# mmigas/LiverRenderer

Hardware: AMD Instinct MI355X
Metric: Msamples/s (higher is better)
Workload: dtype f32; 1 GPU; C3 Liver-SingleMesh volpath 1920x1080 512 spp max_depth 12 (homogeneous medium, isotropic phase, envmap); width=1920, height=1080, spp=512, parallelism=1 GPU

## Files before the change

liverrenderer_amd/csrc/device.hip:

```cpp
#include "host_scene.h"
#include "device_scene.h"
#include "kernels_prb.h"
#include "kernels_vae.h"
#include "kernels_aov.h"
#include "kernels_denoise.h"
#include "kernels_moment.h"
#include <functional>
#include "scene_prep.h"
#include <cmath>
#include <array>
#include <cstring>
#include <algorithm>
#include <stdexcept>
#include <string>
#include <cstdio>
#include <cstdlib>
#include <thread>
#include <chrono>
#include <exception>
#include <dlfcn.h>
#include <rccl/rccl.h>

namespace lrt {

// ... 85 lines not shown
        for (auto e : ev_pool) (void) hipEventDestroy(e);
        if (h_counters) (void) hipHostFree(h_counters);
        if (h_launch) (void) hipHostFree(h_launch);
        if (stream) (void) hipStreamDestroy(stream);
    }
};

void device_scene_destroy(DeviceScene *d) { delete d; }

static_assert(PREP_F_DELTA == F_DELTA && PREP_F_SMOOTH == F_SMOOTH && PREP_F_NULL == F_NULL, "scene_prep.h restates the BSDF leaf flags of dshade.h");

__global__ void k_bio_prepare(DBioMedium *bio, uint32_t n) {
    const uint32_t i = blockIdx.x * blockDim.x + threadIdx.x;
    if (i < n) bio[i].log10_hep = m_log2(bio[i].hepatocity + 1.f) / m_log2(10.f);
}

__global__ void k_medium_prepare(DMedium *media, uint32_t n) {
    const uint32_t i = blockIdx.x * blockDim.x + threadIdx.x;
    if (i >= n) return;
    DMedium &M = media[i];
    const V3 st(M.sigma_t[0], M.sigma_t[1], M.sigma_t[2]), ss = st * V3(M.albedo[0], M.albedo[1], M.albedo[2]);
    const V3 ws = ss / mean3(st / st), wp = ss / st;
    M.w_spec[0] = ws.x; M.w_spec[1] = ws.y; M.w_spec[2] = ws.z; M.w_plain[0] = wp.x; M.w_plain[1] = wp.y; M.w_plain[2] = wp.z;
}

static void upload_media(DeviceScene *D, const lrt_scene_desc &d) {
    prepare_media(d, D->sc.env.bsphere_r, D->h_media, D->h_bio, D->h_het);
    for (size_t i = 0; i < D->h_het.size(); ++i) D->h_het[i].data = D->het_data[i];
    HIP_CHECK(hipMemcpyAsync(D->d_bio, D->h_bio.data(), D->h_bio.size() * sizeof(DBioMedium), hipMemcpyHostToDevice, D->stream));
    k_bio_prepare<<<1, 64, 0, D->stream>>>(D->d_bio, (uint32_t) std::min<size_t>(D->h_bio.size(), 64));
    HIP_CHECK(hipGetLastError());
    HIP_CHECK(hipMemcpyAsync(D->d_het, D->h_het.data(), D->h_het.size() * sizeof(DHetMedium), hipMemcpyHostToDevice, D->stream));
    HIP_CHECK(hipMemcpyAsync(D->d_media, D->h_media.data(), D->h_media.size() * sizeof(DMedium), hipMemcpyHostToDevice, D->stream));
    k_medium_prepare<<<1, 64, 0, D->stream>>>(D->d_media, (uint32_t) std::min<size_t>(D->h_media.size(), 64));
    HIP_CHECK(hipGetLastError());
}

typedef void (*RenderFn)(ScenePtr, LaunchPtr);
struct RenderRow { int mode; bool lds, ld, compact, ext; uint32_t block, record_bytes; RenderFn fn; };

template <int MODE, int BLOCK, bool LDS, bool LD, bool COMPACT = false, bool EXT = false> static void add_row(std::vector<RenderRow> &t) {
    static_assert(record_form_exists(record_layout(MODE), COMPACT), "this layout has no such form (record_layout.h, kRecordForms)");
    t.push_back({ MODE, LDS, LD, COMPACT, EXT, BLOCK, record_bytes(record_layout(MODE), COMPACT), k_render<MODE, BLOCK, LDS, LD, COMPACT, EXT> });
}
template <int MODE, int LDS_BLOCK> static void add_mode(std::vector<RenderRow> &t) {
    add_row<MODE, LDS_BLOCK, true, false>(t); add_row<MODE, LDS_BLOCK, true, true>(t);
    add_row<MODE, LDS_BLOCK, true, false, false, true>(t); add_row<MODE, LDS_BLOCK, true, true, false, true>(t);
    add_row<MODE, LRT_BLOCK, false, false>(t); add_row<MODE, LRT_BLOCK, false, true>(t);
    add_row<MODE, LRT_BLOCK, false, false, false, true>(t); add_row<MODE, LRT_BLOCK, false, true, false, true>(t);
}
template <int MODE> static void add_compact(std::vector<RenderRow> &t) { add_row<MODE, 1024, true, false, true>(t); add_row<MODE, 1024, true, true, true>(t); }

struct KernelTable { std::vector<RenderRow> render; RenderFn prb[2][2][2][2] = {}, prb_grid[2][2] = {}; };
template <bool LDS, bool LD> static void add_prb(KernelTable &t) {
    constexpr int BLOCK = LDS ? 1024 : LRT_BLOCK;
    t.prb[0][LDS][LD][0] = k_render_prb<false, BLOCK, LDS, LD, false>; t.prb[0][LDS][LD][1] = k_render_prb<false, BLOCK, LDS, LD, true>;
    t.prb[1][LDS][LD][0] = k_render_prb<true, BLOCK, LDS, LD, false>; t.prb[1][LDS][LD][1] = k_render_prb<true, BLOCK, LDS, LD, true>;
    t.prb_grid[LDS][LD] = k_render_prb_grid<BLOCK, LDS, LD>;
}
static const KernelTable &kernels() {
    static const KernelTable table = [] {
        KernelTable t; std::vector<RenderRow> &r = t.render;
#ifdef LRT_DEV_VOLPATH_ONLY
#ifndef LRT_DEV_INTEGRATOR
#define LRT_DEV_INTEGRATOR LRT_INTEGRATOR_VOLPATH
#endif
#ifndef LRT_DEV_LD
#define LRT_DEV_LD false
#endif
#ifndef LRT_DEV_BLOCK
#define LRT_DEV_BLOCK 1024
#endif
#define LRT_DEV_CLOSED (LRT_DEV_INTEGRATOR == LRT_INTEGRATOR_VOLPATH ? LRT_INTEGRATOR_VOLPATH_CLOSED : LRT_DEV_INTEGRATOR)
        add_row<LRT_DEV_INTEGRATOR, LRT_DEV_BLOCK, true, LRT_DEV_LD>(r);
        if constexpr (record_form_exists(record_layout(LRT_DEV_INTEGRATOR), true)) {
            add_row<LRT_DEV_INTEGRATOR, LRT_DEV_BLOCK, true, LRT_DEV_LD, true>(r); add_row<LRT_DEV_CLOSED, LRT_DEV_BLOCK, true, LRT_DEV_LD, true>(r);
        }
#else
        add_mode<LRT_INTEGRATOR_PATH, 1024>(r); add_mode<LRT_INTEGRATOR_VOLPATH, 1024>(r); add_mode<LRT_INTEGRATOR_BIOVOLPATH, 1024>(r); add_mode<LRT_INTEGRATOR_BIOVOLPATH06, 1024>(r);
        add_mode<LRT_INTEGRATOR_VOLPATH_HET, LRT_WIDE_BLOCK>(r); add_mode<LRT_INTEGRATOR_VOLPATHMIS, LRT_WIDE_BLOCK>(r); add_mode<LRT_INTEGRATOR_VOLPATHMIS_PLAIN, LRT_WIDE_BLOCK>(r);
        add_compact<LRT_INTEGRATOR_PATH>(r); add_compact<LRT_INTEGRATOR_VOLPATH>(r); add_compact<LRT_INTEGRATOR_BIOVOLPATH>(r); add_compact<LRT_INTEGRATOR_BIOVOLPATH06>(r);
        add_compact<LRT_INTEGRATOR_VOLPATH_CLOSED>(r);
        add_prb<false, false>(t); add_prb<false, true>(t); add_prb<true, false>(t); add_prb<true, true>(t);
#endif
        return t;
    }();
    return table;
}

typedef void (*AovFn)(ScenePtr, LaunchPtr, AovSpecPtr);
static AovFn aov_kernel(bool lds, bool ld, bool ext) {
    static const AovFn t[2][2][2] = { { { k_aov<false, false, false>, k_aov<false, false, true> }, { k_aov<false, true, false>, k_aov<false, true, true> } },
                                      { { k_aov<true, false, false>, k_aov<true, false, true> }, { k_aov<true, true, false>, k_aov<true, true, true> } } };
    return t[lds][ld][ext];
}
typedef decltype(&k_trace<false, false>) TraceFn;
typedef decltype(&k_trace_lds<false, false>) TraceLdsFn;
static TraceFn trace_kernel(bool any_hit, bool ext) {
    static const TraceFn t[2][2] = { { k_trace<false, false>, k_trace<false, true> }, { k_trace<true, false>, k_trace<true, true> } };
    return t[any_hit][ext];
}
static TraceLdsFn trace_lds_kernel(bool any_hit, bool ext) {
    static const TraceLdsFn t[2][2] = { { k_trace_lds<false, false>, k_trace_lds<false, true> }, { k_trace_lds<true, false>, k_trace_lds<true, true> } };
    return t[any_hit][ext];
}
static RenderFn moment_splat_kernel(bool wide, bool alpha) {
    static const RenderFn t[2][2] = { { k_moment_splat<false, false>, k_moment_splat<false, true> }, { k_moment_splat<true, false>, k_moment_splat<true, true> } };
    return t[wide][alpha];
}

DeviceScene *device_scene_create(const lrt_scene_desc &d, int device) {
    select_device(device);
    std::unique_ptr<DeviceScene> D(new DeviceScene());
    D->device = device;
    HIP_CHECK(hipStreamCreateWithFlags(&D->stream, hipStreamNonBlocking));
    hipStream_t st = D->stream;
    PrepOptions opt = PrepOptions::from_env();
    hipDeviceProp_t prop; HIP_CHECK(hipGetDeviceProperties(&prop, device)); opt.n_cus = prop.multiProcessorCount > 0 ? prop.multiProcessorCount : 256;
    int optin = 0; if (hipDeviceGetAttribute(&optin, hipDeviceAttributeSharedMemPerBlockOptin, device) != hipSuccess || optin <= 0) optin = (int) prop.sharedMemPerBlock;
    (void) hipGetLastError();
    opt.lds_limit = std::min<size_t>((size_t) std::max(optin, 0), 160 * 1024) - 512;
    PreparedScene P; DScene &sc = P.sc;
    prepare_geometry(d, opt, P);
    D->n_cus = opt.n_cus; D->bvh_leaf = P.bvh_leaf; D->ext = P.ext;
    auto up = [&](const auto &v) { return D->track(dev_upload(v.data(), v.size(), st)); };
    sc.spheres = P.spheres.empty() ? nullptr : up(P.spheres);
    sc.nodes = (const float4 *) up(P.bvh.nodes);
    sc.tris = (const float4 *) up(P.bvh.tris);
    if (P.use_lds) {
        D->lds = P.lds; D->lds.blob = (const uint4 *) up(P.lds_blob);
        const size_t lds_limit = opt.lds_limit;
        auto raise_lds = [&](const void *k) { if (k) HIP_CHECK(hipFuncSetAttribute(k, hipFuncAttributeMaxDynamicSharedMemorySize, (int) lds_limit)); };
        const KernelTable &K = kernels();
        for (const RenderRow &r : K.render) if (r.lds && (!r.ext || D->ext)) raise_lds((const void *) r.fn);
        for (const auto &adjoint : K.prb) for (const auto &ld : adjoint[1]) for (RenderFn fn : ld) raise_lds((const void *) fn);
        for (RenderFn fn : K.prb_grid[1]) raise_lds((const void *) fn);
        for (int i = 0; i < 2; ++i) for (int ext = 0; ext <= (D->ext ? 1 : 0); ++ext) {
            raise_lds((const void *) aov_kernel(true, i, ext)); raise_lds((const void *) trace_lds_kernel(i, ext));
        }
        D->use_lds = true;
    }
    if (sc.grid.enabled) {
        const size_t n_cells = (size_t) sc.grid.n[0] * sc.grid.n[1] * sc.grid.n[2];
        uint16_t *buf = nullptr; HIP_CHECK(hipMalloc((void **) &buf, n_cells * sizeof(uint16_t))); D->track(buf);
        k_build_dist_grid<<<(uint32_t) ((n_cells + LRT_BLOCK - 1) / LRT_BLOCK), LRT_BLOCK, 0, st>>>(sc.tris, d.n_faces ? (uint32_t) (P.bvh.tris.size() / 12) : 0u, sc.grid, buf, P.grid_abs_margin,
                                                                                             sc.spheres, sc.n_spheres);
        HIP_CHECK(hipGetLastError());
        sc.grid.d = buf;
    }
    prepare_shading(d, opt, P);
    D->has_area_emitter = P.has_area_emitter; D->has_het = P.has_het; D->has_non_bio = P.has_non_bio; D->prb_null = P.prb_null;
    sc.positions = D->track(dev_upload(d.positions, 3 * (size_t) d.n_vertices, st));
    sc.vattr = (const float4 *) up(P.vattr);
    sc.faces = D->track(dev_upload(d.faces, 3 * (size_t) d.n_faces, st));
    sc.face_shape = D->track(dev_upload(d.face_shape, d.n_faces, st));
    sc.shapes = up(P.shapes);
    sc.textures = up(P.textures);
    sc.tex_data = up(P.tex_data);
    sc.bsdfs = up(P.bsdfs);
    HIP_CHECK(hipMalloc((void **) &D->d_media, std::max<uint32_t>(d.n_media, 1) * sizeof(DMedium))); D->track(D->d_media);
    HIP_CHECK(hipMalloc((void **) &D->d_bio, std::max<uint32_t>(d.n_media, 1) * sizeof(DBioMedium))); D->track(D->d_bio);
    HIP_CHECK(hipMalloc((void **) &D->d_het, std::max<uint32_t>(d.n_media, 1) * sizeof(DHetMedium))); D->track(D->d_het);
    D->het_data.assign(std::max<uint32_t>(d.n_media, 1), nullptr);
    for (uint32_t i = 0; i < d.n_media; ++i) {
        const lrt_medium_desc &M = d.media[i];
        if (M.type == LRT_MEDIUM_HETEROGENEOUS) D->het_data[i] = D->track(dev_upload(M.grid_data, (size_t) M.grid_res[0] * M.grid_res[1] * M.grid_res[2], st));
    }
    D->sc = sc;
    upload_media(D.get(), d); sc.media = D->d_media; sc.bio = D->d_bio; sc.het = D->d_het;
    sc.emitters = up(P.emitters);
    sc.mesh_emitters = up(P.mesh_emitters);
    sc.mesh_emitter_tab = up(P.mesh_emitter_tab);
    sc.env_data = (const float4 *) up(P.env_data);
    sc.env_hier = up(P.env_hier);
    HIP_CHECK(hipMalloc((void **) &D->d_sc, sizeof(DScene))); D->track(D->d_sc);
    D->sc = sc;
    HIP_CHECK(hipMemcpyAsync(D->d_sc, &D->sc, sizeof(DScene), hipMemcpyHostToDevice, st));
    HIP_CHECK(hipMalloc((void **) &D->d_launch, LRT_LAUNCH_SLOTS * sizeof(DLaunch))); D->track(D->d_launch);
    HIP_CHECK(hipHostMalloc((void **) &D->h_launch, LRT_LAUNCH_SLOTS * sizeof(DLaunch)));
    HIP_CHECK(hipMalloc((void **) &D->counters, sizeof(DCounters))); D->track(D->counters);
    HIP_CHECK(hipHostMalloc((void **) &D->h_counters, sizeof(DCounters)));
    HIP_CHECK(hipStreamSynchronize(st));
    return D.release();
}

void device_scene_update_params(DeviceScene *D, const lrt_scene_desc &d, bool grids) {
    HIP_CHECK(hipSetDevice(D->device));
    if (grids) for (uint32_t i = 0; i < d.n_media; ++i) {
        const lrt_medium_desc &M = d.media[i];
        if (M.type == LRT_MEDIUM_HETEROGENEOUS && D->het_data[i])
            HIP_CHECK(hipMemcpyAsync(D->het_data[i], M.grid_data, (size_t) M.grid_res[0] * M.grid_res[1] * M.grid_res[2] * sizeof(float), hipMemcpyHostToDevice, D->stream));
    }
    upload_media(D, d);
    HIP_CHECK(hipStreamSynchronize(D->stream));
}

static void ensure_workspace(DeviceScene *D, uint32_t capacity) {
    const uint32_t layouts = workspace_layouts(D->has_het, D->need_mis);
    if (D->capacity >= capacity && D->ws_layouts == layouts) return;
    HIP_CHECK(hipStreamSynchronize(D->stream));
    D->capacity = 0;
    auto get = [](const DPathStreams *q, const RecordStream &r) { void *p; memcpy(&p, (const char *) q + r.member, sizeof p); return p; };
    auto set = [](DPathStreams *q, const RecordStream &r, void *p) { memcpy((char *) q + r.member, &p, sizeof p); };
    for (DPathStreams *q : { &D->q[0], &D->q[1] })
        for (const RecordStream &r : kRecordStreams) if (r.member != kNoMember) { D->release(get(q, r)); set(q, r, nullptr); }
    for (DPathStreams *q : { &D->q[0], &D->q[1] })
        for (size_t k = 0; k < std::size(kRecordStreams); ++k) if (const uint32_t bytes = workspace_stream_bytes(k, layouts)) {
            void *p = nullptr; HIP_CHECK(hipMalloc(&p, (size_t) capacity * bytes)); D->track(p); set(q, kRecordStreams[k], p);
        }
    D->capacity = capacity; D->ws_layouts = layouts;
}

static hipEvent_t get_event(DeviceScene *D, size_t i) {
    while (D->ev_pool.size() <= i) { hipEvent_t e; HIP_CHECK(hipEventCreate(&e)); D->ev_pool.push_back(e); }
    return D->ev_pool[i];
}

static void ensure_pixel_list(DeviceScene *D, const ResolvedOpts &O) {
    const DFilm &F = D->sc.film;
    if (O.tile_count == 1) { D->n_owned_pixels = (uint32_t) F.width * F.height; return; }
    if (D->pixel_list && D->pixel_list_rank == O.tile_rank && D->pixel_list_count == O.tile_count) return;
    const TilePixels T = tile_pixel_list(F, O.tile_rank, O.tile_count);
    D->release(D->pixel_list); D->release(D->pixel_slot); D->pixel_list = nullptr; D->pixel_slot = nullptr;
    D->pixel_list = D->track(dev_upload(T.list.data(), T.list.size(), D->stream));
    D->pixel_slot = D->track(dev_upload(T.slot.data(), T.slot.size(), D->stream));
    D->pixel_list_rank = O.tile_rank; D->pixel_list_count = O.tile_count; D->n_owned_pixels = (uint32_t) T.list.size();
}

static void ensure_halo_list(DeviceScene *D, const ResolvedOpts &O, uint32_t halo) {
    const DFilm &F = D->sc.film;
    if (D->halo_list && D->halo_rank == O.tile_rank && D->halo_count == O.tile_count && D->halo_width == halo) return;
    const std::vector<uint32_t> px = halo_pixel_list(F, O.tile_rank, O.tile_count, halo);
    D->release(D->halo_list); D->halo_list = nullptr;
    D->halo_list = D->track(dev_upload(px.data(), px.size(), D->stream));
    D->halo_rank = O.tile_rank; D->halo_count = O.tile_count; D->halo_width = halo; D->n_halo_pixels = (uint32_t) px.size();
}

static void ensure_prb_workspace(DeviceScene *D, uint32_t records, uint64_t l_buf_lanes) {
    for (int k = 0; k < 2; ++k) D->grow(D->dl[k], D->dl_records[k], records);
    D->grow(D->L_buf, D->l_buf_lanes, l_buf_lanes);
    if (!D->d_grads) { HIP_CHECK(hipMalloc((void **) &D->d_grads, 7 * sizeof(double))); D->track(D->d_grads); }
}

static DRenderParams make_params(const lrt_scene_desc &d, const ResolvedOpts &O, uint64_t n_lanes) {
    DRenderParams rp{};
    rp.integrator = O.integrator; rp.max_depth = O.max_depth; rp.rr_depth = O.rr_depth; rp.hide_emitters = O.hide_emitters;
    rp.spp = O.spp; rp.log2_spp = ((O.spp & (O.spp - 1)) == 0) ? (uint32_t) __builtin_ctz(O.spp) : 0xffffffffu;
    rp.profile = getenv("LRT_DEBUG_LAUNCH") ? 1u : 0u;
#ifdef LRT_EXPERIMENT
    if (getenv("LRT_EXP")) rp.profile |= (uint32_t) atoi(getenv("LRT_EXP"));
    if (getenv("LRT_PRB_DEBUG_LANE")) rp.pad1 = (uint32_t) atoi(getenv("LRT_PRB_DEBUG_LANE")) + 1u;
#endif
    rp.seed_value = d.sampler_seed + O.seed; rp.base_seed = d.sampler_seed; rp.seed = O.seed;
    rp.ld_count = d.sampler_type == LRT_SAMPLER_LD ? O.spp_total : 0u; rp.pass_index = O.pass; rp.spp_total = O.spp_total; rp.tile_rank = O.tile_rank; rp.tile_count = O.tile_count; rp.n_lanes = n_lanes;
    return rp;
}

struct LaunchLog { std::vector<std::pair<hipEvent_t, hipEvent_t>> launches; std::vector<uint32_t> sizes; unsigned long long n_records = 0; size_t ev = 0; uint64_t n_iter = 0; };

static void finish_stats(DeviceScene *D, LaunchLog &log, hipEvent_t e_begin, hipEvent_t e_end, uint64_t n_lanes, lrt_render_stats &stats) {
    hipStream_t st = D->stream;
    HIP_CHECK(hipEventRecord(e_end, st));
    HIP_CHECK(hipMemcpyAsync(D->h_counters, D->counters, sizeof(DCounters), hipMemcpyDeviceToHost, st));
    HIP_CHECK(hipStreamSynchronize(st));
    HIP_CHECK(hipGetLastError());
    stats.n_samples = n_lanes; stats.n_iter = log.n_iter; stats.n_shadow = D->h_counters->n_shadow; stats.n_launches = log.launches.size();
    stats.n_records = log.n_records; if (!log.n_records) for (uint32_t n : log.sizes) stats.n_records += n;
    float ms = 0.f; double ksum = 0.0;
    for (size_t i = 0; i < log.launches.size(); ++i) {
        HIP_CHECK(hipEventElapsedTime(&ms, log.launches[i].first, log.launches[i].second)); ksum += ms;
        if (getenv("LRT_DEBUG_LAUNCH") && i < 40) {
            fprintf(stderr, "[lrt] launch %zu: %.3f ms\n", i, ms);
        }
    }
    stats.kernel_ms = ksum; stats.lds_resident = D->use_lds ? 1 : 0;
    if (getenv("LRT_DEBUG_LAUNCH")) for (int r = 0; r < 4; ++r) {
        fprintf(stderr, "[lrt] tile kind %d (0 proven-free, 1 query, 2 surface, 3 fresh): %llu tiles, %.1f ticks/tile (100 MHz wall clock)\n", r, D->h_counters->prof_tiles[r], D->h_counters->prof_tiles[r] ? (double) D->h_counters->prof_cycles[r] / D->h_counters->prof_tiles[r] : 0.0);
    }
    if (getenv("LRT_DEBUG_LAUNCH") && D->h_counters->prof_wg[1]) {
        const unsigned long long *w = D->h_counters->prof_wg; const double n_wg = D->use_lds ? D->n_cus : 4.0 * D->n_cus, first = (double) ~w[2];
        fprintf(stderr, "[lrt] workgroups (last launch; us): first start 0, last start %.1f, last end %.1f, mean run time %.1f, mean LDS-image copy %.1f, mean barrier wait per wave %.1f\n",
                ((double) w[5] - first) / 100.0, ((double) w[1] - first) / 100.0, (double) w[3] / n_wg / 100.0, (double) w[0] / n_wg / 100.0, (double) w[4] / (n_wg * (D->use_lds ? 16.0 : 4.0)) / 100.0);
    }
    HIP_CHECK(hipEventElapsedTime(&ms, e_begin, e_end)); stats.total_ms = ms;
}

struct PoolGeometry { uint32_t n_wg, P; size_t smem; };
static PoolGeometry pool_geometry(DeviceScene *D, uint64_t n_lanes) {
    PoolGeometry g;
    g.n_wg = D->use_lds ? (uint32_t) D->n_cus : 4u * (uint32_t) D->n_cus;
    const uint32_t pool_max = getenv("LRT_POOL") ? std::max(64, atoi(getenv("LRT_POOL"))) : (D->use_lds ? 32768u : 8192u);
    g.P = (uint32_t) std::min<uint64_t>(pool_max, std::max<uint64_t>(64, ((n_lanes + g.n_wg - 1) / g.n_wg + 63) / 64 * 64));
    if (!getenv("LRT_POOL") && D->use_lds) {
        const uint64_t per_wg = (n_lanes + g.n_wg - 1) / g.n_wg, want = (per_wg / 48 + 63) / 64 * 64;
        if (want < g.P) g.P = (uint32_t) std::max<uint64_t>(want, std::min<uint64_t>(g.P, 8192));
    }
    g.smem = D->use_lds ? D->lds.total_bytes : (size_t) LRT_STACK * LRT_BLOCK * sizeof(int);
    return g;
}

static LaunchPtr push_launch(DeviceScene *D, const DLaunch &a) {
    const uint32_t slot = D->launch_next++ % LRT_LAUNCH_SLOTS;
    if (slot == 0 && D->launch_next > 1) HIP_CHECK(hipStreamSynchronize(D->stream));
    D->h_launch[slot] = a;
    HIP_CHECK(hipMemcpyAsync(&D->d_launch[slot], &D->h_launch[slot], sizeof(DLaunch), hipMemcpyHostToDevice, D->stream));
    return (LaunchPtr) &D->d_launch[slot];
}

template <bool ADJOINT>
static void launch_prb(DeviceScene *D, const DRenderParams &rp, const PoolGeometry &g, const uint32_t *pixel_list, uint64_t lane_begin,
                       float4 *L_buf, const float *grad_image, double *grads, float *film, float *sample_out, float *dgrid = nullptr) {
    hipStream_t st = D->stream;
    HIP_CHECK(hipMemsetAsync(&D->counters->next_lane, 0, sizeof(unsigned long long), st));
    DLaunch a{}; a.rp = rp; a.li = D->lds; a.q0 = D->q[0]; a.q1 = D->q[1]; a.dl0 = D->dl[0]; a.dl1 = D->dl[1]; a.P = g.P; a.cnt = D->counters;
    a.pixel_list = pixel_list; a.lane_begin = lane_begin; a.n = rp.n_lanes; a.L_buf = L_buf; a.grad_image = grad_image; a.wfilm = D->wfilm; a.grads = grads;
    a.film = film; a.sample_out = sample_out; a.sample_base = lane_begin; a.dgrid = dgrid;
    const LaunchPtr lp = push_launch(D, a);
    const bool ld = rp.ld_count != 0;
    const RenderFn fn = (ADJOINT && dgrid) ? kernels().prb_grid[D->use_lds][ld] : kernels().prb[ADJOINT][D->use_lds][ld][D->prb_null];
    if (!fn) throw std::runtime_error("developer build: volpath only");
    fn<<<g.n_wg, D->use_lds ? 1024 : LRT_BLOCK, g.smem, st>>>((ScenePtr) D->d_sc, lp);
    HIP_CHECK(hipGetLastError());
}

static void check_integrator_media(DeviceScene *D, int integrator) {
    if ((integrator == LRT_INTEGRATOR_BIOVOLPATH || integrator == LRT_INTEGRATOR_BIOVOLPATH06) && D->has_non_bio)
        throw std::runtime_error("NotImplementedError: sample_interaction (the bio integrators need liver / parenchyma / glissonCapsule media)");
    if (integrator == LRT_INTEGRATOR_PRBVOLPATH && D->ext)
        throw std::runtime_error("unsupported: prbvolpath on a scene with sphere shapes, point emitters or area emitters on meshes (its adjoint is built for triangles and rectangle / infinite emitters)");
    if (integrator == LRT_INTEGRATOR_VOLPATHMIS) D->need_mis = true;
}

static const RenderRow &select_render_kernel(int integrator, bool has_het, bool spectral_mis, bool lds, bool ld, bool ext, bool compact, bool closed) {
    int mode;
    switch (integrator) {
        case LRT_INTEGRATOR_PATH: case LRT_INTEGRATOR_BIOVOLPATH: case LRT_INTEGRATOR_BIOVOLPATH06: mode = integrator; break;
        case LRT_INTEGRATOR_VOLPATHMIS: mode = spectral_mis ? LRT_INTEGRATOR_VOLPATHMIS : LRT_INTEGRATOR_VOLPATHMIS_PLAIN; break;
        default: mode = closed ? LRT_INTEGRATOR_VOLPATH_CLOSED : (has_het ? LRT_INTEGRATOR_VOLPATH_HET : LRT_INTEGRATOR_VOLPATH);
    }
    for (const RenderRow &r : kernels().render) if (r.mode == mode && r.lds == lds && r.ld == ld && r.compact == compact && r.ext == ext) return r;
    throw std::runtime_error("no render-kernel instance for mode " + std::to_string(mode) + (lds ? ", LDS BVH" : ", global BVH") + (ld ? ", ld sampler" : ", independent sampler") +
                             (compact ? ", compact records" : ", wide records") + (ext ? ", EXT" : ""));
}

static void run_wavefront(DeviceScene *D, const lrt_scene_desc &d, const ResolvedOpts &O, uint64_t lane_begin, uint64_t n_lanes,
                          const uint32_t *pixel_list, float *film, float *sample_out, lrt_render_stats &stats) {
    hipStream_t st = D->stream;
    DRenderParams rp = make_params(d, O, n_lanes);
    rp.pixel_slot = pixel_list ? D->pixel_slot : nullptr;
    rp.pass_in = D->cur_pass_in; rp.pass_out = D->cur_pass_out;
    const bool prb = O.integrator == LRT_INTEGRATOR_PRBVOLPATH;
    check_integrator_media(D, O.integrator);
    PoolGeometry g = pool_geometry(D, n_lanes);
    const uint32_t records = (uint32_t) std::min<uint64_t>((uint64_t) g.n_wg * 2u * g.P, 0xffffffffull);
    ensure_workspace(D, records);
    if (prb) ensure_prb_workspace(D, records, 0);
    HIP_CHECK(hipMemsetAsync(D->counters, 0, sizeof(DCounters), st));
    LaunchLog log;
    hipEvent_t e_begin = get_event(D, log.ev++), e_end = get_event(D, log.ev++);
    HIP_CHECK(hipEventRecord(e_begin, st));
    const bool count_iter = !(O.integrator == LRT_INTEGRATOR_PATH && O.max_depth == 0);
    hipEvent_t a = get_event(D, log.ev++), b = get_event(D, log.ev++);
    HIP_CHECK(hipEventRecord(a, st));
    if (prb) { stats.record_bytes = 0; launch_prb<false>(D, rp, g, pixel_list, lane_begin, nullptr, nullptr, nullptr, film, sample_out); }
    else {
        DLaunch a{}; a.rp = rp; a.li = D->lds; a.q0 = D->q[0]; a.q1 = D->q[1]; a.P = g.P; a.cnt = D->counters; a.pixel_list = pixel_list;
        a.lane_begin = lane_begin; a.n = n_lanes; a.film = film; a.sample_out = sample_out; a.sample_base = lane_begin;
        const bool compact = D->use_lds && !D->has_area_emitter && !D->ext && !getenv("LRT_WIDE_RECORDS") && O.integrator != LRT_INTEGRATOR_VOLPATHMIS && !(O.integrator == LRT_INTEGRATOR_VOLPATH && D->has_het);
        const bool closed = compact && O.integrator == LRT_INTEGRATOR_VOLPATH && closed_records(d, D->sc.cam.medium) && !getenv("LRT_NO_CLOSED_RECORDS");
#ifdef LRT_DEV_VOLPATH_ONLY
        if (D->ext) throw std::runtime_error("developer build: no EXT instances (spheres / point emitters)");
        if (!(D->use_lds && (O.integrator == LRT_DEV_INTEGRATOR || (LRT_DEV_INTEGRATOR == LRT_INTEGRATOR_VOLPATH_HET && D->has_het)) && (rp.ld_count != 0) == LRT_DEV_LD)) throw std::runtime_error("developer build: one integrator / sampler / LDS BVH only");
#endif
        const RenderRow &row = select_render_kernel(O.integrator, D->has_het, d.use_spectral_mis != 0, D->use_lds, rp.ld_count != 0, D->ext, compact, closed);
        stats.record_bytes = row.record_bytes;
        const LaunchPtr lp = push_launch(D, a);
        row.fn<<<g.n_wg, row.block, g.smem, st>>>((ScenePtr) D->d_sc, lp);
        HIP_CHECK(hipGetLastError());
    }
    HIP_CHECK(hipEventRecord(b, st));
    log.launches.emplace_back(a, b); log.sizes.push_back(0);
    HIP_CHECK(hipMemcpyAsync(D->h_counters, D->counters, sizeof(DCounters), hipMemcpyDeviceToHost, st));
    HIP_CHECK(hipStreamSynchronize(st));
    log.n_iter = count_iter ? D->h_counters->n_iter : 0;
    log.n_records = D->h_counters->n_records;
    finish_stats(D, log, e_begin, e_end, n_lanes, stats);
    stats.n_closed_guard = D->h_counters->n_closed_guard;
    if (stats.n_closed_guard)
        throw std::runtime_error("64-byte path records: " + std::to_string(stats.n_closed_guard) + " trips broke the premise of the layout (radiance before a path's last trip, "
                                 "or an emitter hit that needs its MIS weight); the scene test in closed_records() is wrong for this scene: LRT_NO_CLOSED_RECORDS=1 renders it with 80-byte records");
}

static void render_passes(DeviceScene *D, const lrt_scene_desc &d, const lrt_render_opts *opts, float *film_raw, float *image, lrt_render_stats &stats,
                          const std::function<void(const ResolvedOpts &)> &after_pass, bool moment = false);

void device_render(DeviceScene *D, const lrt_scene_desc &d, const lrt_render_opts *opts, float *film_raw, float *image, lrt_render_stats &stats) {
    render_passes(D, d, opts, film_raw, image, stats, nullptr);
}

static void develop_and_download(DeviceScene *D, const float *film, float *film_raw, float *image, size_t film_floats, size_t image_floats, bool on_device, bool moment = false) {
    const DFilm &F = D->sc.film; const size_t np = (size_t) F.width * F.height;
// ... 614 lines not shown
```

liverrenderer_amd/csrc/device_types.h:

```cpp
#pragma once
#include <stdint.h>
#include <hip/hip_vector_types.h>

namespace lrt {

struct DShape {
    int32_t bsdf, emitter, interior_medium, exterior_medium;
    int32_t has_normals, has_texcoords, flip_normals, kind;
};

struct DBsdf {
    int32_t type, reflectance, nested, texture;
    float eta, scale; int32_t flags, pad;
};

struct DTexture {
    int32_t type, width, height, channels;
    float color0[3]; float color1[3];
    float to_uv[6];
    uint32_t data_offset;
    uint32_t pad;
};

struct DMedium {
    float sigma_t[3]; float albedo[3];
    int32_t has_spectral_extinction, sample_emitters, phase; float g;
    float scale; int32_t het;
    float w_spec[3], w_plain[3];
    float nee_vmin[3];
    float pad2[3];
};

struct DBioMedium {
    int32_t type, has_spectral_extinction;
    float layer_limit[4];
    float collagen[4][3], elastin[4][3];
    float blood[3], bile[3], lipid_water[3];
    float hepatocity, log10_hep;
    float sigmat[3];
    float pad;
};

struct DHetMedium {
    const float *data;
    int32_t res[3]; float max_density;
    float to_local[12];
    float bbox_min[3], bbox_max[3];
    float scale, pad;
};

struct DEmitter {
    int32_t type, shape; float radiance[3]; float scale;
    float n[3]; float inv_area;
    float to_world[12];
};

struct DSphere {
    float center[3], radius;
    float to_world[9];
    float to_object[12];
    uint32_t shape; int32_t flip_normals;
    float pad[2];
};

struct DMeshEmitter {
    uint32_t first_face, n_faces, pmf_offset, cdf_offset;
    float sum, normalization;
    int32_t has_normals, flip_normals;
    int32_t mesh, pad[3];
};

#define LRT_MAX_HIER_LEVELS 16

struct DCamera {
    float s2c[16];
    float to_world[12];
    float near_clip, far_clip;
    int32_t medium, pad;
    float ppo_x, ppo_y;
};

struct DFilm {
    int32_t width, height;
    int32_t crop_offset_x, crop_offset_y;
    float scale_x, scale_y, offset_x, offset_y;
    int32_t channels, has_alpha, rfilter, fcount;
    float rf_radius, rf_inv_radius; int32_t fn, pad;
    float rf_coeff[10];
    int32_t pad2[2];
};

struct DEnv {
    int32_t type;
    int32_t emitter;
    uint32_t w, h;
    float scale;
    float bsphere_c[3]; float bsphere_r;
    float to_world[9];
    float to_local[9];
    float patch_size[2], inv_patch_size[2];
    uint32_t max_patch[2];
    int32_t n_levels;
    uint32_t level_offset[LRT_MAX_HIER_LEVELS];
    uint32_t level_width[LRT_MAX_HIER_LEVELS];
    float radiance[3];
};

struct DDistGrid {
    const uint16_t *d;
    float lo[3]; float cell, inv_cell;
    int32_t n[3]; int32_t enabled;
};

struct DScene {
    const float4 *nodes;
    const float4 *tris;
    const float *positions;
    const float4 *vattr;
    const uint32_t *faces, *face_shape;
    const DShape *shapes; const DBsdf *bsdfs; const DTexture *textures; const DMedium *media; const DBioMedium *bio; const DHetMedium *het; const DEmitter *emitters;
    const float *tex_data;
    const float4 *env_data;
    const float *env_hier;
    uint32_t n_faces, n_emitters;
    int32_t root_is_leaf, has_null_bsdf;
    int32_t nee_fast_reject;
    int32_t one_shape;
    uint32_t root_leaf_first, root_leaf_count;
    DCamera cam; DFilm film; DEnv env;
    DDistGrid grid;
    const DSphere *spheres;
    uint32_t n_spheres, pad_sph;
    const DMeshEmitter *mesh_emitters;
    const float *mesh_emitter_tab;
};

#define LRT_CONST __attribute__((address_space(4)))
typedef const LRT_CONST DScene &SceneRef;
typedef const LRT_CONST DFilm &FilmRef;
typedef const LRT_CONST DEnv &EnvRef;
typedef const LRT_CONST DDistGrid &GridRef;
typedef const LRT_CONST DScene *ScenePtr;

struct DRenderParams {
    int32_t integrator, max_depth, rr_depth, hide_emitters;
    uint32_t spp, log2_spp;
    uint32_t seed_value;
    uint32_t base_seed, seed;
    uint32_t ld_count, pad1;
    uint32_t tile_rank, tile_count;
    int32_t grad_medium;
    uint32_t tiles_x, tiles_y, profile;
    uint32_t pad2;
    uint64_t n_lanes;
    const uint32_t *pixel_slot;
    uint32_t pass_index, spp_total;
    const unsigned long long *pass_in;
    unsigned long long *pass_out;
};

struct DPathStreams {
    float4 *o_maxt;
    float4 *d_eta;
    float4 *tp_pdf;
    float4 *res_flags;
    float4 *lp_lane;
    uint2  *rng;
    float2 *tdepth;
    float4 *hit;
    float4 *w1, *w2, *w3, *w4;
};

#define LRT_INTEGRATOR_VOLPATHMIS_PLAIN 102
#define LRT_INTEGRATOR_VOLPATH_HET 101
#define LRT_INTEGRATOR_VOLPATH_CLOSED 103

#define PF_DEPTH_MASK   0x0000ffffu
#define PF_MEDIUM_SHIFT 16
#define PF_MEDIUM_MASK  0x00ff0000u
#define PF_CHANNEL_SHIFT 24
#define PF_SPECULAR     (1u << 26)
#define PF_VALID        (1u << 27)
#define PF_NOHIT        (1u << 28)
#define PF_BIO_SCATTERED (1u << 29)
#define PF_LONG_QUERY   (1u << 29)
#define PF_HAVE_SI      (1u << 29)
#define PF_LAST_NULL    (1u << 30)
#define PF_BIO_EMIT     (1u << 30)
#define PF_BIO_FULL     (1u << 31)

struct DCounters {
    uint32_t pad[4];
    unsigned long long n_shadow;
    unsigned long long n_iter;
    unsigned long long next_lane;
    unsigned long long n_records;
    unsigned long long prof_cycles[4], prof_tiles[4];
    unsigned long long prof_wg[6];
    unsigned long long n_closed_guard;
};

struct DLdsInfo {
    const uint4 *blob;
    uint32_t blob_bytes, nodes_off, verts_off, tris_off, stack_off, total_bytes;
};

struct DLaunch {
    DRenderParams rp; DLdsInfo li; DPathStreams q0, q1;
    float4 *dl0, *dl1;
    uint32_t P, pad; DCounters *cnt; const uint32_t *pixel_list; uint64_t lane_begin, n;
    float4 *L_buf; const float *grad_image; const float *wfilm; double *grads;
    float *film; float *sample_out; uint64_t sample_base;
    float *dgrid;
};
typedef const LRT_CONST DRenderParams &RpRef;
typedef const LRT_CONST DLaunch *LaunchPtr;

}
```

liverrenderer_amd/csrc/dshade.h:

```cpp
#pragma once
#include "device_types.h"
#include "dmath.h"
#include "../../include/liverrt.h"

namespace lrt {

#define LRT_BLOCK 256
#define LRT_STACK 32

template <class T> DEV T tab(const T *table, uint32_t i, bool worth_a_look = true) {
    if (!worth_a_look) return table[i];
    const uint32_t i0 = (uint32_t) __builtin_amdgcn_readfirstlane((int) i);
    if (__builtin_amdgcn_ballot_w64(true) != 0ull && __builtin_amdgcn_ballot_w64(i != i0) == 0ull)
    { T out; __builtin_memcpy(&out, reinterpret_cast<const LRT_CONST T *>((uintptr_t) table) + i0, sizeof(T)); return out; }
    return table[i];
}

struct Ray { V3 o, d; float maxt; };
struct Hit { float t, u, v; uint32_t prim; uint32_t slot = 0xffffffffu; };
struct SI { bool valid; float t; V3 p, n; Frame sh; V2 uv; V3 dp_du, dp_dv, wi; uint32_t prim, shape; };

DEV float slab_rcp(float x) { return fmin_(fmax_(__builtin_amdgcn_rcpf(x), -1e20f), 1e20f); }
DEV void test_tri(const float4 *__restrict__ tris, uint32_t slot, V3 o, V3 d, float maxt, Hit &best) {
    float4 a = tris[3 * slot], b = tris[3 * slot + 1], c = tris[3 * slot + 2];
    V3 p0(a.x, a.y, a.z), e1(b.x, b.y, b.z), e2(c.x, c.y, c.z);
    uint32_t f = f2u(a.w);
    V3 pvec = cross(d, e2);
    float inv_det = rcp(dot(e1, pvec));
    V3 tvec = o - p0;
    float u = dot(tvec, pvec) * inv_det;
    if (!(u >= 0.f && u <= 1.f)) return;
    V3 qvec = cross(tvec, e1);
    float v = dot(d, qvec) * inv_det;
    if (!(v >= 0.f && u + v <= 1.f)) return;
    float t = dot(e2, qvec) * inv_det;
    if (!(t >= 0.f && t <= maxt)) return;
    if (t < best.t || (t == best.t && f < best.prim)) { best.t = t; best.u = u; best.v = v; best.prim = f; }
}

template <bool ANY_HIT>
DEV Hit trace(SceneRef sc, const Ray &r, int *__restrict__ stack ) {
    Hit best; best.t = kInf; best.u = best.v = 0.f; best.prim = 0xffffffffu;
    if (sc.n_faces == 0) return best;
    const V3 o = r.o, d = r.d;
    if (sc.root_is_leaf) {
        for (uint32_t i = 0; i < sc.root_leaf_count; ++i) test_tri(sc.tris, sc.root_leaf_first + i, o, d, r.maxt, best);
        return best;
    }
    const float ix = slab_rcp(d.x), iy = slab_rcp(d.y), iz = slab_rcp(d.z);
    const float ox = -o.x * ix, oy = -o.y * iy, oz = -o.z * iz;
    const f32x2 vix = { ix, ix }, viy = { iy, iy }, viz = { iz, iz }, vox = { ox, ox }, voy = { oy, oy }, voz = { oz, oz };
    const uint32_t DONE = 0x7fffffffu;
    int sp = 0; uint32_t cur = 0;
    for (;;) {
        while (cur < DONE) {
            const float4 *nd = sc.nodes + 4 * (size_t) cur;
            float4 n0 = nd[0], n1 = nd[1], n2 = nd[2], n3 = nd[3];
            float limit = fmin_(best.t, r.maxt);
            const f32x2 vax = pk_fma(f32x2{ n0.x, n0.y }, vix, vox), vay = pk_fma(f32x2{ n0.z, n0.w }, viy, voy), vaz = pk_fma(f32x2{ n2.x, n2.y }, viz, voz);
            const f32x2 vbx = pk_fma(f32x2{ n1.x, n1.y }, vix, vox), vby = pk_fma(f32x2{ n1.z, n1.w }, viy, voy), vbz = pk_fma(f32x2{ n2.z, n2.w }, viz, voz);
            const float ax0 = vax.x, ax1 = vax.y, ay0 = vay.x, ay1 = vay.y, az0 = vaz.x, az1 = vaz.y;
            const float bx0 = vbx.x, bx1 = vbx.y, by0 = vby.x, by1 = vby.y, bz0 = vbz.x, bz1 = vbz.y;
            float tmin0 = fmax_(fmax_(fmin_(ax0, ax1), fmin_(ay0, ay1)), fmax_(fmin_(az0, az1), 0.f));
            float tmax0 = fmin_(fmin_(fmax_(ax0, ax1), fmax_(ay0, ay1)), fmin_(fmax_(az0, az1), limit));
            float tmin1 = fmax_(fmax_(fmin_(bx0, bx1), fmin_(by0, by1)), fmax_(fmin_(bz0, bz1), 0.f));
            float tmax1 = fmin_(fmin_(fmax_(bx0, bx1), fmax_(by0, by1)), fmin_(fmax_(bz0, bz1), limit));
            bool h0 = tmin0 <= tmax0 * 1.000002f, h1 = tmin1 <= tmax1 * 1.000002f;
            int r0 = (int) f2u(n3.x), r1 = (int) f2u(n3.y);
            uint32_t c0 = r0 < 0 ? (0x80000000u | (uint32_t) ~r0) : (uint32_t) r0;
            uint32_t c1 = r1 < 0 ? (0x80000000u | (uint32_t) ~r1) : (uint32_t) r1;
            if (h0 && h1) {
                bool swap = tmin1 < tmin0;
                stack[sp * LRT_BLOCK] = (int) (swap ? c0 : c1); ++sp;
                cur = swap ? c1 : c0;
            } else if (h0 || h1) cur = h0 ? c0 : c1;
            else if (sp == 0) cur = DONE;
            else { --sp; cur = (uint32_t) stack[sp * LRT_BLOCK]; }
        }
        if (cur == DONE) break;
        uint32_t slot = cur & 0x7fffffffu; bool last;
        do { last = sc.tris[3 * slot + 1].w != 0.f; test_tri(sc.tris, slot, o, d, r.maxt, best); ++slot; } while (!last);
        if (ANY_HIT && best.prim != 0xffffffffu) return best;
        if (sp == 0) break;
        --sp; cur = (uint32_t) stack[sp * LRT_BLOCK];
    }
    return best;
}

struct GlobalTracer {
    static constexpr bool kExt = false;
    SceneRef sc; int *stack;
    DEV Hit closest(const Ray &r) const { return trace<false>(sc, r, stack); }
    DEV Hit any(const Ray &r) const { return trace<true>(sc, r, stack); }
    DEV SI surface(SceneRef s, const Ray &r, const Hit &h) const;
};

struct LdsScene {
    const float4 *nodes; const float4 *verts; const uint2 *tris;
    uint32_t n_faces, root_is_leaf, root_first, root_count;
};
#define LRT_LDS_BLOCK_MAX 1024

DEV void test_tri_lds(const LdsScene &L, uint2 ix, uint32_t slot, V3 o, V3 d, float maxt, Hit &best) {
    float4 a = L.verts[ix.x & 0xffffu], b = L.verts[ix.x >> 16], c = L.verts[ix.y & 0xffffu];
    V3 p0(a.x, a.y, a.z), e1(b.x - a.x, b.y - a.y, b.z - a.z), e2(c.x - a.x, c.y - a.y, c.z - a.z);
    V3 pvec = cross(d, e2);
    float inv_det = rcp(dot(e1, pvec));
    V3 tvec = o - p0;
    float u = dot(tvec, pvec) * inv_det;
    if (!(u >= 0.f && u <= 1.f)) return;
    V3 qvec = cross(tvec, e1);
    float v = dot(d, qvec) * inv_det;
    if (!(v >= 0.f && u + v <= 1.f)) return;
    float t = dot(e2, qvec) * inv_det;
    if (!(t >= 0.f && t <= maxt)) return;
    if (t > best.t) return;
    uint32_t f = ix.y >> 17;
    if (t < best.t || f < (best.prim & 0x7fffu)) { best.t = t; best.u = u; best.v = v; best.prim = f | (slot << 16); }
}

#ifdef LRT_TRAV_STATS
__device__ unsigned long long g_trav[8];
#define LRT_TRAV_COUNT(k) { const unsigned long long m_ = __ballot(true); if ((threadIdx.x & 63u) == (uint32_t) (__ffsll((long long) m_) - 1)) { atomicAdd(&g_trav[(ANY_HIT ? 4 : 0) + k], 1ull); atomicAdd(&g_trav[(ANY_HIT ? 4 : 0) + k + 1], (unsigned long long) __popcll(m_)); } }
#else
#define LRT_TRAV_COUNT(k)
#endif
template <bool ANY_HIT, int STRIDE>
DEV Hit trace_lds(const LdsScene &L, const Ray &r, uint16_t *__restrict__ stack ) {
    Hit best; best.t = kInf; best.u = best.v = 0.f; best.prim = 0xffffffffu;
    if (L.n_faces == 0) return best;
    const V3 o = r.o, d = r.d;
    if (L.root_is_leaf) {
        for (uint32_t i = 0; i < L.root_count; ++i) test_tri_lds(L, L.tris[L.root_first + i], L.root_first + i, o, d, r.maxt, best);
        if (best.prim != 0xffffffffu) { best.slot = best.prim >> 16; best.prim &= 0x7fffu; }
        return best;
    }
    const float ix = slab_rcp(d.x), iy = slab_rcp(d.y), iz = slab_rcp(d.z);
    const float ox = -o.x * ix, oy = -o.y * iy, oz = -o.z * iz;
    const f32x2 vix = { ix, ix }, viy = { iy, iy }, viz = { iz, iz }, vox = { ox, ox }, voy = { oy, oy }, voz = { oz, oz };
    const uint32_t DONE = 0x10000u;
    int sp = 0; uint32_t cur = 0;
    for (;;) {
        while (cur < 0x8000u) {
            LRT_TRAV_COUNT(0)
            const float4 *nd = L.nodes + 4 * cur;
            float4 n0 = nd[0], n1 = nd[1], n2 = nd[2], n3 = nd[3];
            float limit = fmin_(best.t, r.maxt);
            const f32x2 vax = pk_fma(f32x2{ n0.x, n0.y }, vix, vox), vay = pk_fma(f32x2{ n0.z, n0.w }, viy, voy), vaz = pk_fma(f32x2{ n2.x, n2.y }, viz, voz);
            const f32x2 vbx = pk_fma(f32x2{ n1.x, n1.y }, vix, vox), vby = pk_fma(f32x2{ n1.z, n1.w }, viy, voy), vbz = pk_fma(f32x2{ n2.z, n2.w }, viz, voz);
            const float ax0 = vax.x, ax1 = vax.y, ay0 = vay.x, ay1 = vay.y, az0 = vaz.x, az1 = vaz.y;
            const float bx0 = vbx.x, bx1 = vbx.y, by0 = vby.x, by1 = vby.y, bz0 = vbz.x, bz1 = vbz.y;
            float tmin0 = fmax_(fmax_(fmin_(ax0, ax1), fmin_(ay0, ay1)), fmax_(fmin_(az0, az1), 0.f));
            float tmax0 = fmin_(fmin_(fmax_(ax0, ax1), fmax_(ay0, ay1)), fmin_(fmax_(az0, az1), limit));
            float tmin1 = fmax_(fmax_(fmin_(bx0, bx1), fmin_(by0, by1)), fmax_(fmin_(bz0, bz1), 0.f));
            float tmax1 = fmin_(fmin_(fmax_(bx0, bx1), fmax_(by0, by1)), fmin_(fmax_(bz0, bz1), limit));
            bool h0 = tmin0 <= tmax0 * 1.000002f, h1 = tmin1 <= tmax1 * 1.000002f;
            const uint32_t c0 = f2u(n3.x), c1 = f2u(n3.y);
            if (h0 && h1) {
                bool swap = tmin1 < tmin0;
                stack[sp * STRIDE] = (uint16_t) (swap ? c0 : c1); ++sp;
                cur = swap ? c1 : c0;
            } else if (h0 || h1) cur = h0 ? c0 : c1;
            else if (sp == 0) cur = DONE;
            else { --sp; cur = stack[sp * STRIDE]; }
        }
        if (cur == DONE) break;
        uint32_t slot = cur & 0x7fffu, last;
        do {
            LRT_TRAV_COUNT(2)
            const uint2 ix = L.tris[slot];
            last = (ix.y >> 16) & 1u;
            test_tri_lds(L, ix, slot, o, d, r.maxt, best);
            ++slot;
        } while (!last);
        if (ANY_HIT && best.prim != 0xffffffffu) return best;
        if (sp == 0) break;
        --sp; cur = stack[sp * STRIDE];
    }
    if (best.prim != 0xffffffffu) { best.slot = best.prim >> 16; best.prim &= 0x7fffu; }
    return best;
}

template <int STRIDE>
struct LdsTracer {
    static constexpr bool kExt = false;
    const LdsScene &L; uint16_t *stack;
    DEV Hit closest(const Ray &r) const { return trace_lds<false, STRIDE>(L, r, stack); }
    DEV Hit any(const Ray &r) const { return trace_lds<true, STRIDE>(L, r, stack); }
    DEV SI surface(SceneRef s, const Ray &r, const Hit &h) const;
};

DEV float dist_grid_lower_bound(GridRef g, V3 p) {
    float fx = (p.x - g.lo[0]) * g.inv_cell, fy = (p.y - g.lo[1]) * g.inv_cell, fz = (p.z - g.lo[2]) * g.inv_cell;
    int ix = min(max((int) fx, 0), g.n[0] - 1), iy = min(max((int) fy, 0), g.n[1] - 1), iz = min(max((int) fz, 0), g.n[2] - 1);
    union { uint16_t u; _Float16 h; } cv; cv.u = g.d[(uint32_t) ((iz * g.n[1] + iy) * g.n[0] + ix)];
    float D = (float) cv.h;
    float cx = fx - ((float) ix + .5f), cy = fy - ((float) iy + .5f), cz = fz - ((float) iz + .5f);
    return D - __builtin_amdgcn_sqrtf(cx * cx + cy * cy + cz * cz) * (g.cell * 1.001f);
}

#ifndef LRT_GRID_STEPS
#define LRT_GRID_STEPS 3
#endif
template <int STEPS = LRT_GRID_STEPS>
DEV bool segment_proven_empty(GridRef g, V3 o, V3 d, float maxt) {
    if (!g.enabled || !(maxt < 1e30f)) return false;
    float len = __builtin_amdgcn_sqrtf(dot(d, d));
    float remaining = maxt * len * 1.01f, inv_len = __builtin_amdgcn_rcpf(len);
    V3 p = o;
    for (int k = 0; k < STEPS; ++k) {
        float lb = dist_grid_lower_bound(g, p);
        if (remaining < lb) return true;
        if (!(lb > .5f * g.cell)) return false;
        float adv = lb * .99f;
        p = p + d * (adv * inv_len);
        remaining -= adv * .995f;
    }
    return false;
}

template <int K>
DEV bool segment_covered_by_balls(GridRef g, V3 o, V3 d, float maxt) {
    if (!g.enabled || !(maxt < 1e30f)) return false;
    const float len = __builtin_amdgcn_sqrtf(dot(d, d));
    const float L = maxt * len * 1.01f;
#define LRT_FRAC(k) (((float) (k) + .5f) / (float) K)
    float lb[K];
#pragma unroll
    for (int k = 0; k < K; ++k) lb[k] = dist_grid_lower_bound(g, fma3(d, maxt * LRT_FRAC(k), o)) * .995f;
    float covered = 0.f; bool ok = true;
#pragma unroll
    for (int k = 0; k < K; ++k) {
        const float c = L * LRT_FRAC(k);
        ok = ok && (lb[k] > 0.f) && (c - lb[k] <= covered);
        covered = fmax_(covered, c + lb[k]);
    }
    return ok && covered >= L;
#undef LRT_FRAC
}

DEV bool segment_free_of_surfaces(GridRef g, V3 o, V3 d, float maxt) {
#ifdef LRT_SPHERE_TRACE
    return segment_proven_empty(g, o, d, maxt);
#else
    return segment_covered_by_balls<2>(g, o, d, maxt);
#endif
}

DEV SI compute_si(SceneRef sc, const Ray &r, const Hit &h, const LdsScene *L = nullptr) {
    const bool valid = h.prim != 0xffffffffu;
    float t = kInf; V3 p(0.f), n(0.f), shn(0.f), shs(0.f), sht(0.f), dp_du(0.f), dp_dv(0.f), wi = -r.d;
    V2 uv = { 0.f, 0.f }; uint32_t f = 0xffffffffu, shp = 0xffffffffu;
    if (valid) {
        f = h.prim; shp = 0u; if (!sc.one_shape) shp = sc.face_shape[f];
        const DShape sd = tab(sc.shapes, shp, sc.one_shape);
        uint32_t i0, i1, i2; V3 p0, p1, p2;
        if (L && h.slot != 0xffffffffu) {
            const uint2 ix = L->tris[h.slot];
            i0 = ix.x & 0xffffu; i1 = ix.x >> 16; i2 = ix.y & 0xffffu;
            const float4 a = L->verts[i0], b = L->verts[i1], c = L->verts[i2];
            p0 = V3(a.x, a.y, a.z); p1 = V3(b.x, b.y, b.z); p2 = V3(c.x, c.y, c.z);
        } else {
            i0 = sc.faces[3 * f]; i1 = sc.faces[3 * f + 1]; i2 = sc.faces[3 * f + 2];
            p0 = V3(sc.positions[3 * i0], sc.positions[3 * i0 + 1], sc.positions[3 * i0 + 2]);
            p1 = V3(sc.positions[3 * i1], sc.positions[3 * i1 + 1], sc.positions[3 * i1 + 2]);
            p2 = V3(sc.positions[3 * i2], sc.positions[3 * i2 + 1], sc.positions[3 * i2 + 2]);
        }
        float b1 = h.u, b2 = h.v, b0 = 1.f - b1 - b2;
        t = h.t;
        p = V3(fma_(p0.x, b0, fma_(p1.x, b1, p2.x * b2)), fma_(p0.y, b0, fma_(p1.y, b1, p2.y * b2)), fma_(p0.z, b0, fma_(p1.z, b1, p2.z * b2)));
        V3 dp0 = p1 - p0, dp1 = p2 - p0;
        n = normalize(cross(dp0, dp1));
        uv = { b1, b2 };
        Basis bs = coordinate_system(n);
        dp_du = bs.s; dp_dv = bs.t;
        if (sd.has_texcoords) {
            const float2 t0 = *reinterpret_cast<const float2 *>(sc.vattr + 2 * (size_t) i0 + 1), t1 = *reinterpret_cast<const float2 *>(sc.vattr + 2 * (size_t) i1 + 1),
                         t2 = *reinterpret_cast<const float2 *>(sc.vattr + 2 * (size_t) i2 + 1);
            V2 uv0 = { t0.x, t0.y }, uv1 = { t1.x, t1.y }, uv2 = { t2.x, t2.y };
            uv = { fma_(uv2.x, b2, fma_(uv1.x, b1, uv0.x * b0)), fma_(uv2.y, b2, fma_(uv1.y, b1, uv0.y * b0)) };
            V2 duv0 = { uv1.x - uv0.x, uv1.y - uv0.y }, duv1 = { uv2.x - uv0.x, uv2.y - uv0.y };
            float det = fma_(duv0.x, duv1.y, -(duv0.y * duv1.x)), inv_det = rcp(det);
            if (det != 0.f) {
                dp_du = V3(fma_(duv1.y, dp0.x, -(duv0.y * dp1.x)), fma_(duv1.y, dp0.y, -(duv0.y * dp1.y)), fma_(duv1.y, dp0.z, -(duv0.y * dp1.z))) * inv_det;
                dp_dv = V3(fma_(-duv1.x, dp0.x, duv0.x * dp1.x), fma_(-duv1.x, dp0.y, duv0.x * dp1.y), fma_(-duv1.x, dp0.z, duv0.x * dp1.z)) * inv_det;
            }
        }
        if (sd.has_normals) {
            const float4 a0 = sc.vattr[2 * (size_t) i0], a1 = sc.vattr[2 * (size_t) i1], a2 = sc.vattr[2 * (size_t) i2];
            V3 n0(a0.x, a0.y, a0.z), n1(a1.x, a1.y, a1.z), n2(a2.x, a2.y, a2.z);
            V3 ni(fma_(n2.x, b2, fma_(n1.x, b1, n0.x * b0)), fma_(n2.y, b2, fma_(n1.y, b1, n0.y * b0)), fma_(n2.z, b2, fma_(n1.z, b1, n0.z * b0)));
            float il = rsqrt_(squared_norm(ni));
            shn = ni * il;
        } else shn = n;
        if (sd.flip_normals) { n = V3(-n.x, -n.y, -n.z); shn = V3(-shn.x, -shn.y, -shn.z); }
        shs = normalize(fma3(shn, -dot(shn, dp_du), dp_du));
        if (dp_du.x == 0.f && dp_du.y == 0.f && dp_du.z == 0.f) shs = coordinate_system(shn).s;
        sht = cross(shn, shs);
        V3 md(-r.d.x, -r.d.y, -r.d.z);
        wi = V3(dot(md, shs), dot(md, sht), dot(md, shn));
    }
    SI si;
    si.valid = valid; si.t = t; si.p = p; si.n = n; si.sh.s = shs; si.sh.t = sht; si.sh.n = shn; si.uv = uv;
    si.dp_du = dp_du; si.dp_dv = dp_dv; si.wi = wi; si.prim = f; si.shape = shp;
    return si;
}

DEV SI GlobalTracer::surface(SceneRef s, const Ray &r, const Hit &h) const { return compute_si(s, r, h); }
template <int STRIDE> DEV SI LdsTracer<STRIDE>::surface(SceneRef s, const Ray &r, const Hit &h) const { return compute_si(s, r, h, &L); }


DEV bool solve_quadratic(float a, float b, float c, float &x0, float &x1) {
    const bool linear_case = a == 0.f, valid_linear = linear_case && b != 0.f;
    x0 = x1 = -c / b;
    const float discrim = fma_(b, b, -(4.f * a * c));
    const bool valid_quadratic = !linear_case && discrim >= 0.f;
    const float sqrt_discrim = __builtin_sqrtf(discrim);
    const float temp = -0.5f * (b + __builtin_copysignf(sqrt_discrim, b));
    const float x0p = temp / a, x1p = c / temp;
    const float x0m = fmin_(x0p, x1p), x1m = fmax_(x0p, x1p);
    if (!linear_case) { x0 = x0m; x1 = x1m; }
    return valid_linear || valid_quadratic;
}
DEV float sphere_intersect(V3 center, float radius, const Ray &r) {
    const V3 l = r.o - center, d = r.d;
    const float plane_t = dot(-l, d) / norm(d);
    const V3 o = fma3(d, plane_t, r.o) - center;
    const float A = squared_norm(d), B = 2.f * dot(o, d), C = squared_norm(o) - sqr(radius);
    float near_t, far_t;
    const bool found = solve_quadratic(A, B, C, near_t, far_t);
    near_t += plane_t; far_t += plane_t;
    const bool out_bounds = !(near_t <= r.maxt && far_t >= 0.f);
    const bool in_bounds = near_t < 0.f && far_t > r.maxt;
    const float t = near_t < 0.f ? far_t : near_t;
    return (found && !out_bounds && !in_bounds) ? t : kInf;
}
DEV bool sphere_test(V3 center, float radius, const Ray &r) {
    const V3 o = r.o - center, d = r.d;
    const float A = squared_norm(d), B = 2.f * dot(o, d), C = squared_norm(o) - sqr(radius);
    float near_t, far_t;
    const bool found = solve_quadratic(A, B, C, near_t, far_t);
    const bool out_bounds = !(near_t <= r.maxt && far_t >= 0.f);
    const bool in_bounds = near_t < 0.f && far_t > r.maxt;
    return found && !out_bounds && !in_bounds;
}
DEV const LRT_CONST DSphere &sphere_ref(SceneRef sc, uint32_t k) { return reinterpret_cast<const LRT_CONST DSphere *>((uintptr_t) sc.spheres)[k]; }
DEV Hit spheres_closest(SceneRef sc, const Ray &r) {
    Hit best; best.t = kInf; best.u = best.v = 0.f; best.prim = 0xffffffffu;
    const uint32_t ns = sc.n_spheres;
    for (uint32_t k = 0; k < ns; ++k) {
        const LRT_CONST DSphere &S = sphere_ref(sc, k);
        const float t = sphere_intersect(V3(S.center[0], S.center[1], S.center[2]), S.radius, r);
        if (t < best.t) { best.t = t; best.prim = sc.n_faces + k; }
    }
    return best;
}
DEV bool spheres_any(SceneRef sc, const Ray &r) {
    const uint32_t ns = sc.n_spheres;
    bool hit = false;
    for (uint32_t k = 0; k < ns; ++k) {
        const LRT_CONST DSphere &S = sphere_ref(sc, k);
        hit = hit || sphere_test(V3(S.center[0], S.center[1], S.center[2]), S.radius, r);
    }
    return hit;
}
template <bool ANY_HIT, class WALK> DEV Hit trace_ext(SceneRef sc, const Ray &r, const WALK &walk) {
    if (ANY_HIT) {
        if (spheres_any(sc, r)) { Hit h; h.t = 0.f; h.u = h.v = 0.f; h.prim = sc.n_faces; return h; }
        return walk(r);
    }
    const Hit s = spheres_closest(sc, r);
    Ray r2 = r; r2.maxt = fmin_(r.maxt, s.t);
    const Hit h = walk(r2);
    return h.prim != 0xffffffffu ? h : s;
}

DEV float unit_angle_z(V3 v) {
    const float temp = 2.f * m_asin(.5f * norm(V3(v.x, v.y, v.z - signf_(v.z))));
    return v.z >= 0.f ? temp : kPi - temp;
}
DEV SI compute_si_sphere(SceneRef sc, const Ray &r, const Hit &h) {
    const uint32_t k = h.prim - sc.n_faces;
    const DSphere S = tab(reinterpret_cast<const DSphere *>(sc.spheres), k);
    const V3 c(S.center[0], S.center[1], S.center[2]);
    SI si;
    si.valid = true; si.t = h.t;
    si.p = fma3(r.d, h.t, r.o);
    V3 n = normalize(si.p - c);
    const V3 local = xform_point12(S.to_object, si.p);
    const float theta = unit_angle_z(local);
    float phi = m_atan2(local.y, local.x);
    if (phi < 0.f) phi += 2.f * kPi;
    si.uv = { phi * kInvTwoPi, theta * kInvPi };
    V3 dp_du(-local.y, local.x, 0.f);
    const float rd = __builtin_sqrtf(sqr(local.x) + sqr(local.y)), inv_rd = rcp(rd);
    const float cos_phi = local.x * inv_rd, sin_phi = local.y * inv_rd;
    V3 dp_dv(local.z * cos_phi, local.z * sin_phi, -rd);
    if (rd == 0.f) dp_dv = V3(1.f, 0.f, 0.f);
    si.dp_du = xform_vec9(S.to_world, dp_du) * (2.f * kPi);
    si.dp_dv = xform_vec9(S.to_world, dp_dv) * kPi;
    if (S.flip_normals) n = V3(-n.x, -n.y, -n.z);
    si.n = n; si.sh.n = n;
    V3 shs = normalize(fma3(n, -dot(n, si.dp_du), si.dp_du));
    if (si.dp_du.x == 0.f && si.dp_du.y == 0.f && si.dp_du.z == 0.f) shs = coordinate_system(n).s;
    si.sh.s = shs; si.sh.t = cross(n, shs);
    const V3 md(-r.d.x, -r.d.y, -r.d.z);
    si.wi = V3(dot(md, si.sh.s), dot(md, si.sh.t), dot(md, si.sh.n));
    si.prim = h.prim; si.shape = S.shape;
    return si;
}

template <class BASE> struct ExtTracer {
    static constexpr bool kExt = true;
    const BASE &base; SceneRef sc;
    DEV Hit closest(const Ray &r) const { return trace_ext<false>(sc, r, [&](const Ray &rr) { return base.closest(rr); }); }
    DEV Hit any(const Ray &r) const { return trace_ext<true>(sc, r, [&](const Ray &rr) { return base.any(rr); }); }
    DEV SI surface(SceneRef s, const Ray &r, const Hit &h) const {
        if (h.prim != 0xffffffffu && h.prim >= s.n_faces) return compute_si_sphere(s, r, h);
        return base.surface(s, r, h);
    }
};
template <bool SECOND, class A, class B> DEV const auto &pick(const A &a, const B &b) { if constexpr (SECOND) return b; else return a; }
template <class TR> DEV SI surface_of(const TR &, SceneRef sc, const Ray &r, const Hit &h) { return compute_si(sc, r, h); }
template <class B> DEV SI surface_of(const ExtTracer<B> &tr, SceneRef sc, const Ray &r, const Hit &h) { return tr.surface(sc, r, h); }
template <class TR> DEV bool hit_on_emitter(const TR &, SceneRef sc, const Hit &h) {
    return h.prim != 0xffffffffu && tab(sc.shapes, sc.face_shape[h.prim], sc.one_shape).emitter >= 0;
}
template <class B> DEV bool hit_on_emitter(const ExtTracer<B> &, SceneRef sc, const Hit &h) {
    return h.prim != 0xffffffffu && h.prim < sc.n_faces && tab(sc.shapes, sc.face_shape[h.prim], sc.one_shape).emitter >= 0;
}

DEV V3 offset_p(V3 p, V3 n, V3 d) {
    float mag = (1.f + max3(abs3(p))) * kRayEpsilon;
    mag = mulsign(mag, dot(n, d));
    return fma3(n, mag, p);
}
DEV Ray spawn_ray(V3 p, V3 n, V3 d) { Ray r; r.o = offset_p(p, n, d); r.d = d; r.maxt = kLargest; return r; }
DEV Ray spawn_ray_to(V3 p, V3 n, V3 t) {
    Ray r; r.o = offset_p(p, n, t - p);
    V3 d = t - r.o; float dist = norm(d);
    r.d = d / dist; r.maxt = dist * (1.f - kShadowEpsilon);
    return r;
}

DEV V2 square_to_uniform_disk_concentric(float sx, float sy) {
    float x = fma_(2.f, sx, -1.f), y = fma_(2.f, sy, -1.f);
    bool is_zero = (x == 0.f) && (y == 0.f), q13 = __builtin_fabsf(x) < __builtin_fabsf(y);
    float r = q13 ? y : x, rp = q13 ? x : y;
    float phi = 0.25f * kPi * rp / r;
    if (q13) phi = 0.5f * kPi - phi;
    if (is_zero) phi = 0.f;
    float s, c; m_sincos(phi, &s, &c);
    return { r * c, r * s };
}
DEV V3 square_to_cosine_hemisphere(float sx, float sy) {
    V2 p = square_to_uniform_disk_concentric(sx, sy);
    float z = safe_sqrt(1.f - fma_(p.x, p.x, p.y * p.y));
    return V3(p.x, p.y, z);
}
DEV V3 square_to_uniform_sphere(float sx, float sy) {
    float z = fma_(-2.f, sy, 1.f), r = safe_sqrt(fma_(-z, z, 1.f));
    float s, c; m_sincos(2.f * kPi * sx, &s, &c);
    return V3(r * c, r * s, z);
}

DEV V3 tex_eval(SceneRef sc, int tex, const SI &si) {
    const DTexture &T = sc.textures[tex];
    if (T.type == LRT_TEX_CHECKERBOARD) {
        float u = fma_(T.to_uv[1], si.uv.y, fma_(T.to_uv[0], si.uv.x, T.to_uv[2]));
        float v = fma_(T.to_uv[4], si.uv.y, fma_(T.to_uv[3], si.uv.x, T.to_uv[5]));
        bool mx = u - __builtin_floorf(u) > .5f, my = v - __builtin_floorf(v) > .5f;
        return (mx == my) ? V3(T.color0[0], T.color0[1], T.color0[2]) : V3(T.color1[0], T.color1[1], T.color1[2]);
    }
    if (T.type == LRT_TEX_RGB) return V3(T.color0[0], T.color0[1], T.color0[2]);
    return V3(0.f);
}

DEV V2 tex_eval_1_grad(SceneRef sc, int tex, const SI &si) {
    const DTexture &T = sc.textures[tex];
    if (T.type != LRT_TEX_BITMAP) return { 0.f, 0.f };
    float u = fma_(T.to_uv[1], si.uv.y, fma_(T.to_uv[0], si.uv.x, T.to_uv[2]));
    float v = fma_(T.to_uv[4], si.uv.y, fma_(T.to_uv[3], si.uv.x, T.to_uv[5]));
    int w = T.width, h = T.height;
    float fx = fma_(u, (float) w, -0.5f), fy = fma_(v, (float) h, -0.5f);
    int ix = (int) __builtin_floorf(fx), iy = (int) __builtin_floorf(fy);
    float w1x = fx - (float) ix, w1y = fy - (float) iy, w0x = 1.f - w1x, w0y = 1.f - w1y;
    int x0 = ix % w; if (x0 < 0) x0 += w; int x1 = (ix + 1) % w; if (x1 < 0) x1 += w;
    int y0 = iy % h; if (y0 < 0) y0 += h; int y1 = (iy + 1) % h; if (y1 < 0) y1 += h;
    const float *d = sc.tex_data + T.data_offset;
    float f00 = d[y0 * w + x0], f10 = d[y0 * w + x1], f01 = d[y1 * w + x0], f11 = d[y1 * w + x1];
    float dx = fma_(w0y, f10 - f00, w1y * (f11 - f01)), dy = fma_(w0x, f01 - f00, w1x * (f11 - f10));
    float du = T.to_uv[0] * dx + T.to_uv[3] * dy, dv = T.to_uv[1] * dx + T.to_uv[4] * dy;
    return { (float) w * du, (float) h * dv };
}

enum { F_DELTA = 1, F_SMOOTH = 2, F_NULL = 4 };
struct BSDFSample { V3 wo; float pdf, eta; int type; V3 weight; };

DEV void fresnel(float cos_theta_i, float eta, float *r, float *cos_theta_t, float *eta_it, float *eta_ti) {
    bool outside = cos_theta_i >= 0.f;
    float rcp_eta = rcp(eta);
    *eta_it = outside ? eta : rcp_eta; *eta_ti = outside ? rcp_eta : eta;
    float cos_theta_t_sqr = fma_(-fma_(-cos_theta_i, cos_theta_i, 1.f), *eta_ti * *eta_ti, 1.f);
    float cti = __builtin_fabsf(cos_theta_i), ctt = safe_sqrt(cos_theta_t_sqr);
    bool index_matched = eta == 1.f, special = index_matched || cti == 0.f;
    float r_sc = index_matched ? 0.f : 1.f;
    float a_s = fma_(-*eta_it, ctt, cti) / fma_(*eta_it, ctt, cti);
    float a_p = fma_(-*eta_it, cti, ctt) / fma_(*eta_it, cti, ctt);
    float rr = 0.5f * (sqr(a_s) + sqr(a_p));
    if (special) rr = r_sc;
    *r = rr; *cos_theta_t = mulsign_neg(ctt, cos_theta_i);
}

DEV Frame bump_frame(SceneRef sc, const DBsdf &B, const SI &si) {
    V2 g = tex_eval_1_grad(sc, B.texture, si);
    float gx = B.scale * g.x, gy = B.scale * g.y;
    V3 dp_du = fma3(si.sh.n, gx - dot(si.sh.n, si.dp_du), si.dp_du);
    V3 dp_dv = fma3(si.sh.n, gy - dot(si.sh.n, si.dp_dv), si.dp_dv);
    Frame r;
    r.n = normalize(cross(dp_du, dp_dv));
    if (dot(si.n, r.n) < 0.f) r.n = r.n * -1.f;
    r.n = si.sh.to_local(r.n);
    if (si.wi.z * dot(si.wi, r.n) <= 0.f) r.n = V3(-r.n.x, -r.n.y, r.n.z);
    r.s = normalize(fma3(r.n, -dot(r.n, si.dp_du), si.dp_du));
    r.t = cross(r.n, r.s);
    return r;
}
DEV float tan_theta_2(V3 v) { float t = fma_(-v.z, v.z, 1.f); return fmax_(t, 0.f) / sqr(v.z); }
DEV float shadow_terminator(V3 pn, V3 wo) {
    float alpha2 = fmin_(0.125f * tan_theta_2(pn), 1.f);
    return 2.f / (1.f + __builtin_sqrtf(1.f + alpha2 * tan_theta_2(wo)));
}

template <bool DIELECTRIC = false>
DEV BSDFSample leaf_sample(SceneRef sc, const DBsdf &B, const SI &si, V3 wi, float s1, float s2x, float s2y) {
    BSDFSample bs;
    bs.wo = V3(0.f); bs.pdf = 0.f; bs.eta = 0.f; bs.type = 0; bs.weight = V3(0.f);
    if (!DIELECTRIC && B.type == LRT_BSDF_DIFFUSE) {
        if (wi.z > 0.f) {
            bs.wo = square_to_cosine_hemisphere(s2x, s2y);
            bs.pdf = kInvPi * bs.wo.z; bs.eta = 1.f; bs.type = F_SMOOTH;
            if (bs.pdf > 0.f) bs.weight = tex_eval(sc, B.reflectance, si);
        }
    } else if (DIELECTRIC || B.type == LRT_BSDF_DIELECTRIC) {
        float r_i, ctt, eta_it, eta_ti;
        fresnel(wi.z, B.eta, &r_i, &ctt, &eta_it, &eta_ti);
        float t_i = 1.f - r_i;
        bool sel_r = s1 <= r_i;
        bs.pdf = sel_r ? r_i : t_i;
        bs.type = F_DELTA;
        bs.wo = sel_r ? V3(-wi.x, -wi.y, wi.z) : V3(-eta_ti * wi.x, -eta_ti * wi.y, ctt);
        bs.eta = sel_r ? 1.f : eta_it;
        bs.weight = V3(1.f);
        if (!sel_r) bs.weight = bs.weight * sqr(eta_ti);
    } else {
        float nx = -wi.x, ny = -wi.y, nz = -wi.z;
        asm volatile("" : "+v"(nx), "+v"(ny), "+v"(nz));
        bs.wo = V3(nx, ny, nz); bs.type = F_NULL; bs.eta = 1.f; bs.pdf = 1.f; bs.weight = V3(1.f);
    }
    return bs;
}
DEV V3 leaf_eval(SceneRef sc, const DBsdf &B, const SI &si, V3 wi, V3 wo) {
    if (B.type == LRT_BSDF_DIFFUSE) {
        if (!(wi.z > 0.f && wo.z > 0.f)) return V3(0.f);
        return tex_eval(sc, B.reflectance, si) * kInvPi * wo.z;
    }
    return V3(0.f);
}
DEV float leaf_pdf(const DBsdf &B, V3 wi, V3 wo) {
    if (B.type == LRT_BSDF_DIFFUSE) return (wi.z > 0.f && wo.z > 0.f) ? kInvPi * wo.z : 0.f;
    return 0.f;
}

template <bool DIELECTRIC = false>
DEV BSDFSample bsdf_sample(SceneRef sc, int b, const SI &si, float s1, float s2x, float s2y) {
    const DBsdf B = tab(sc.bsdfs, b, sc.one_shape);
    if (B.type == LRT_BSDF_BUMPMAP) {
        Frame pf = bump_frame(sc, B, si);
        V3 pwi = pf.to_local(si.wi);
        BSDFSample bs = leaf_sample<DIELECTRIC>(sc, tab(sc.bsdfs, B.nested, sc.one_shape), si, pwi, s1, s2x, s2y);
        bool active = any_nonzero(bs.weight);
        V3 pwo = pf.to_world(bs.wo);
        active = active && (bs.wo.z * pwo.z > 0.f);
        bs.wo = pwo;
        V3 w = bs.weight * shadow_terminator(pf.n, bs.wo);
        bs.weight = active ? w : V3(0.f);
        return bs;
    }
    return leaf_sample<DIELECTRIC>(sc, B, si, si.wi, s1, s2x, s2y);
}
DEV V3 bsdf_eval(SceneRef sc, int b, const SI &si, V3 wo) {
    const DBsdf B = tab(sc.bsdfs, b, sc.one_shape);
    if (B.type == LRT_BSDF_BUMPMAP) {
        Frame pf = bump_frame(sc, B, si);
        V3 pwi = pf.to_local(si.wi), pwo = pf.to_local(wo);
        if (!(wo.z * pwo.z > 0.f)) return V3(0.f);
        return leaf_eval(sc, tab(sc.bsdfs, B.nested, sc.one_shape), si, pwi, pwo) * shadow_terminator(pf.n, wo);
    }
    return leaf_eval(sc, B, si, si.wi, wo);
}
DEV float bsdf_pdf(SceneRef sc, int b, const SI &si, V3 wo) {
    const DBsdf B = tab(sc.bsdfs, b, sc.one_shape);
    if (B.type == LRT_BSDF_BUMPMAP) {
        Frame pf = bump_frame(sc, B, si);
        V3 pwi = pf.to_local(si.wi), pwo = pf.to_local(wo);
        if (!(wo.z * pwo.z > 0.f)) return 0.f;
        return leaf_pdf(tab(sc.bsdfs, B.nested, sc.one_shape), pwi, pwo);
    }
    return leaf_pdf(B, si.wi, wo);
}
DEV float bsdf_null_transmission(SceneRef sc, int b) { return tab(sc.bsdfs, b, sc.one_shape).type == LRT_BSDF_NULL ? 1.f : 0.f; }

struct DirSample { V3 p, n, d; float pdf, dist; bool delta; int emitter; };

DEV float interval_to_linear(float v0, float v1, float sample) {
    if (__builtin_fabsf(v0 - v1) > 1e-4f * (v0 + v1))
        return (v0 - safe_sqrt(lerpf(sqr(v0), sqr(v1), sample))) / (v0 - v1);
    return sample;
}
DEV void hier_sample(SceneRef sc, float sx, float sy, float *ox, float *oy, float *pdf) {
    EnvRef E = sc.env;
    sx = clampf(sx, 0.f, 1.f); sy = clampf(sy, 0.f, 1.f);
    uint32_t offx = 0, offy = 0;
    for (int l = E.n_levels - 2; l > 0; --l) {
        offx <<= 1; offy <<= 1;
        uint32_t width = E.level_width[l];
        uint32_t oi = ((offx & 1u) | (((offx & ~1u) | (offy & 1u)) << 1)) + ((offy & ~1u) * width);
        const float4 q = *reinterpret_cast<const float4 *>(sc.env_hier + E.level_offset[l] + oi);
        float v00 = q.x, v10 = q.y, v01 = q.z, v11 = q.w;
        sx = clampf(sx, 0.f, 1.f); sy = clampf(sy, 0.f, 1.f);
        float r0 = v00 + v10, r1 = v01 + v11;
        sy *= r0 + r1;
        bool mask = sy > r0;
        if (mask) { offy += 1; sy -= r0; }
        sy /= mask ? r1 : r0;
        float c0 = mask ? v01 : v00, c1 = mask ? v11 : v10;
        sx *= c0 + c1;
        mask = sx > c0;
        if (mask) sx -= c0;
        sx /= mask ? c1 : c0;
        if (mask) offx += 1;
    }
    uint32_t w0 = E.level_width[0];
    const float *l0 = sc.env_hier + E.level_offset[0];
    uint32_t oi = offx + offy * w0;
    float v00 = l0[oi], v10 = l0[oi + 1], v01 = l0[oi + w0], v11 = l0[oi + w0 + 1];
    float r0 = v00 + v10, r1 = v01 + v11;
    sy = interval_to_linear(r0, r1, sy);
    float c0 = lerpf(v00, v01, sy), c1 = lerpf(v10, v11, sy);
    sx = interval_to_linear(c0, c1, sx);
    *pdf = lerpf(c0, c1, sx);
    *ox = ((float) (int) offx + sx) * E.patch_size[0];
    *oy = ((float) (int) offy + sy) * E.patch_size[1];
}
DEV float hier_eval(SceneRef sc, float px, float py) {
    EnvRef E = sc.env;
    px = clampf(px, 0.f, 1.f); py = clampf(py, 0.f, 1.f);
    px *= E.inv_patch_size[0]; py *= E.inv_patch_size[1];
    uint32_t ox = min((uint32_t) (int) px, E.max_patch[0]), oy = min((uint32_t) (int) py, E.max_patch[1]);
    px -= (float) (int) ox; py -= (float) (int) oy;
    uint32_t w0 = E.level_width[0];
    const float *l0 = sc.env_hier + E.level_offset[0];
    uint32_t oi = ox + oy * w0;
    float v00 = l0[oi], v10 = l0[oi + 1], v01 = l0[oi + w0], v11 = l0[oi + w0 + 1];
    return lerpf(lerpf(v00, v10, px), lerpf(v01, v11, px), py);
}

DEV V3 env_eval_uv(SceneRef sc, float u, float v) {
    EnvRef E = sc.env;
    uint32_t rx = E.w, ry = E.h;
    u -= .5f / (float) (rx - 1u);
    u -= __builtin_floorf(u); v -= __builtin_floorf(v);
    u *= (float) (rx - 1u); v *= (float) (ry - 1u);
    uint32_t px = min((uint32_t) u, rx - 2u), py = min((uint32_t) v, ry - 2u);
    float w1x = u - (float) px, w1y = v - (float) py, w0x = 1.f - w1x, w0y = 1.f - w1y;
    uint32_t idx = py * rx + px;
    float4 a = sc.env_data[idx], b = sc.env_data[idx + 1], c = sc.env_data[idx + rx], d = sc.env_data[idx + rx + 1];
    V3 v00(a.x, a.y, a.z), v10(b.x, b.y, b.z), v01(c.x, c.y, c.z), v11(d.x, d.y, d.z);
    V3 t0 = v10 * w1x, t1 = v11 * w1x;
    V3 v0(fma_(w0x, v00.x, t0.x), fma_(w0x, v00.y, t0.y), fma_(w0x, v00.z, t0.z));
    V3 v1(fma_(w0x, v01.x, t1.x), fma_(w0x, v01.y, t1.y), fma_(w0x, v01.z, t1.z));
    V3 t2 = v1 * w1y;
    V3 vv(fma_(w0y, v0.x, t2.x), fma_(w0y, v0.y, t2.y), fma_(w0y, v0.z, t2.z));
    return vv * E.scale;
}
DEV V3 emitter_eval_env(SceneRef sc, V3 dir_world) {
    EnvRef E = sc.env;
    if (E.type == LRT_EMITTER_CONSTANT) return V3(E.radiance[0], E.radiance[1], E.radiance[2]);
    V3 v = xform_vec9(E.to_local, dir_world);
    float uu = m_atan2(v.x, -v.z) * kInvTwoPi, vv = safe_acos(v.y) * kInvPi;
    return env_eval_uv(sc, uu, vv);
}

DEV uint32_t mesh_emitter_search(const float *__restrict__ cdf, uint32_t n, float sum, float value) {
    const float s = value * sum;
    uint32_t start = 0u, end = n - 1u;
    const uint32_t trips = n > 1u ? 32u - (uint32_t) __builtin_clz(n - 1u) : 0u;
    for (uint32_t i = 0; i < trips; ++i) {
        const uint32_t middle = (start + end) >> 1;
        const float c = cdf[middle];
        const bool pred = (c < s || c == 0.f) && c != sum;
        start = pred ? min(middle + 1u, end) : start;
        end = pred ? end : middle;
    }
    return start;
}
DEV void mesh_emitter_position(SceneRef sc, const DMeshEmitter &M, float sx, float sy, V3 *p_out, V3 *n_out) {
    const float *tab_f = sc.mesh_emitter_tab;
    const uint32_t idx = mesh_emitter_search(tab_f + M.cdf_offset, M.n_faces, M.sum, sy);
    const float pmf = tab_f[M.pmf_offset + idx] * M.normalization;
    const float cdf = idx > 0u ? tab_f[M.cdf_offset + idx - 1u] * M.normalization : 0.f;
    sy = (sy - cdf) / pmf;
    const uint32_t f = M.first_face + idx;
    const uint32_t i0 = sc.faces[3 * f], i1 = sc.faces[3 * f + 1], i2 = sc.faces[3 * f + 2];
    const V3 p0(sc.positions[3 * i0], sc.positions[3 * i0 + 1], sc.positions[3 * i0 + 2]);
    const V3 p1(sc.positions[3 * i1], sc.positions[3 * i1 + 1], sc.positions[3 * i1 + 2]);
    const V3 p2(sc.positions[3 * i2], sc.positions[3 * i2 + 1], sc.positions[3 * i2 + 2]);
    const V3 e0 = p1 - p0, e1 = p2 - p0;
    const float t = safe_sqrt(1.f - sx), bx = 1.f - t, by = t * sy;
    *p_out = V3(fma_(e0.x, bx, fma_(e1.x, by, p0.x)), fma_(e0.y, bx, fma_(e1.y, by, p0.y)), fma_(e0.z, bx, fma_(e1.z, by, p0.z)));
    V3 n;
    if (M.has_normals) {
        const float4 a0 = sc.vattr[2 * (size_t) i0], a1 = sc.vattr[2 * (size_t) i1], a2 = sc.vattr[2 * (size_t) i2];
        const float b0 = 1.f - bx - by;
        n = V3(fma_(a0.x, b0, fma_(a1.x, bx, a2.x * by)), fma_(a0.y, b0, fma_(a1.y, bx, a2.y * by)), fma_(a0.z, b0, fma_(a1.z, bx, a2.z * by)));
    } else n = cross(e0, e1);
    n = normalize(n);
    *n_out = M.flip_normals ? -n : n;
}

template <bool EXT = false>
DEV V3 sample_emitter_direction(SceneRef sc, V3 ref_p, float sx, float sy, DirSample *ds) {
    uint32_t ne = sc.n_emitters;
    ds->p = V3(0.f); ds->n = V3(0.f); ds->d = V3(0.f); ds->pdf = 0.f; ds->dist = 0.f; ds->delta = false; ds->emitter = -1;
    if (ne == 0) return V3(0.f);
    uint32_t index = 0; float emitter_weight = 1.f, pmf = 1.f;
    if (ne > 1) {
        float scaled = sx * (float) ne;
        index = min((uint32_t) scaled, ne - 1u);
        emitter_weight = (float) ne; sx = scaled - (float) index; pmf = 1.f / (float) ne;
    }
    const DEmitter &E = sc.emitters[index];
    ds->emitter = (int) index;
    V3 spec(0.f);
    if (E.type == LRT_EMITTER_AREA) {
        const DMeshEmitter M = EXT ? tab(sc.mesh_emitters, index) : DMeshEmitter{};
        if (EXT && M.mesh) {
            mesh_emitter_position(sc, M, sx, sy, &ds->p, &ds->n);
            ds->pdf = M.normalization;
        } else {
            ds->p = xform_point12(E.to_world, V3(fma_(sx, 2.f, -1.f), fma_(sy, 2.f, -1.f), 0.f));
            ds->n = V3(E.n[0], E.n[1], E.n[2]);
            ds->pdf = E.inv_area;
        }
        ds->d = ds->p - ref_p;
        float dist2 = squared_norm(ds->d);
        ds->dist = __builtin_sqrtf(dist2);
// ... 215 lines not shown
```

liverrenderer_amd/csrc/film.h:

```cpp

template <typename FP> DEV float estrin10(float x, FP c) {
    float x2 = x * x, x4 = x2 * x2, x8 = x4 * x4;
    float a0 = fma_(x, c[1], c[0]), a1 = fma_(x, c[3], c[2]), a2 = fma_(x, c[5], c[4]), a3 = fma_(x, c[7], c[6]), a4 = fma_(x, c[9], c[8]);
    float b0 = fma_(x2, a1, a0), b1 = fma_(x2, a3, a2);
    float c0 = fma_(x4, b1, b0);
    return fma_(x8, a4, c0);
}
DEV float rfilter_eval(FilmRef F, float x) {
    if (F.rfilter == LRT_RFILTER_GAUSSIAN) return fmax_(estrin10(sqr(x), F.rf_coeff), 0.f);
    if (F.rfilter == LRT_RFILTER_TENT) return fmax_(0.f, 1.f - __builtin_fabsf(x * F.rf_inv_radius));
    return (__builtin_fabsf(x) <= 0.5f) ? 1.f : 0.f;
}

DEV size_t film_pixel_index(FilmRef F, int px, int py) {
    return (size_t) (py - F.crop_offset_y) * F.width + (px - F.crop_offset_x);
}

struct FilmFootprint {
    int pix, piy; float relx, rely;
    DEV uint32_t key() const { return (uint32_t) (piy + 0x4000) << 16 | (uint32_t) (pix + 0x4000); }
};
DEV FilmFootprint film_footprint(FilmRef F, int px, int py, float jx, float jy) {
    const float spx = (float) px + jx, spy = (float) py + jy;
    FilmFootprint f;
    f.pix = (int) __builtin_floorf(spx) - F.fn; f.piy = (int) __builtin_floorf(spy) - F.fn;
    f.relx = (float) f.pix + .5f - spx; f.rely = (float) f.piy + .5f - spy;
    return f;
}

DEV void finish_path(SceneRef sc, RpRef rp, float *__restrict__ film, float *__restrict__ sample_out,
                     uint64_t sample_base, uint32_t lane, V3 L, bool valid) {
    if (rp.integrator == LRT_INTEGRATOR_PATH && !valid) L = V3(0.f);
    if (sample_out) {
        const uint64_t j = lane_local_index(rp, lane);
        float4 *o = reinterpret_cast<float4 *>(sample_out) + (j - sample_base);
        *o = make_float4(L.x, L.y, L.z, valid ? 1.f : 0.f);
        return;
    }
    FilmRef F = sc.film;
    int px, py; lane_to_pixel(sc, rp, lane, &px, &py);
    const int C = F.channels;
    const float alpha = valid ? 1.f : 0.f;
    auto splat = [&](float *p, float w) {
        atomicAdd(p + 0, L.x * w); atomicAdd(p + 1, L.y * w); atomicAdd(p + 2, L.z * w);
        if (F.has_alpha) { atomicAdd(p + 3, alpha * w); atomicAdd(p + 4, 1.f * w); } else atomicAdd(p + 3, 1.f * w);
    };
    if (F.rfilter == LRT_RFILTER_BOX) {
        int x = px - F.crop_offset_x, y = py - F.crop_offset_y;
        float *p = film + ((size_t) y * F.width + x) * C;
        atomicAdd(p + 0, L.x); atomicAdd(p + 1, L.y); atomicAdd(p + 2, L.z);
        if (F.has_alpha) { atomicAdd(p + 3, alpha); atomicAdd(p + 4, 1.f); } else atomicAdd(p + 3, 1.f);
        return;
    }
    float jx, jy; lane_jitter(rp, lane, lane_local_index(rp, lane), jx, jy);
    const FilmFootprint fp = film_footprint(F, px, py, jx, jy);
    int count = F.fcount;
    for (int ys = 0; ys < count; ++ys) {
        int y = fp.piy - F.crop_offset_y + ys;
        float wy = rfilter_eval(F, fp.rely + (float) ys);
        if (y < 0 || y >= F.height || (wy == 0.f && finite3(L))) continue;
        for (int xs = 0; xs < count; ++xs) {
            int x = fp.pix - F.crop_offset_x + xs;
            if (x < 0 || x >= F.width) continue;
            float w = wy * rfilter_eval(F, fp.relx + (float) xs);
            if (w == 0.f && finite3(L)) continue;
            splat(film + ((size_t) y * F.width + x) * C, w);
        }
    }
}

struct FilmRun { uint32_t pixel; bool head, tail; };
DEV FilmRun film_run(FilmRef F, bool have, int px, int py) {
    FilmRun r;
    r.pixel = have ? (uint32_t) film_pixel_index(F, px, py) : 0xffffffffu;
    const uint32_t prev = wave_prev(r.pixel, 0xfffffffeu), next = wave_next(r.pixel, 0xfffffffeu);
    r.head = r.pixel != prev || !have; r.tail = have && r.pixel != next;
    return r;
}

DEV void finish_paths_wave(SceneRef sc, RpRef rp, float *__restrict__ film, float *__restrict__ sample_out,
                           uint64_t sample_base, bool finishing, uint32_t lane, V3 L, bool valid) {
    FilmRef F = sc.film;
    if (sample_out || F.rfilter != LRT_RFILTER_BOX) {
        if (finishing) finish_path(sc, rp, film, sample_out, sample_base, lane, L, valid);
        return;
    }
    if (rp.integrator == LRT_INTEGRATOR_PATH && !valid) L = V3(0.f);
    uint32_t pixel = 0xffffffffu;
    if (finishing) { int px, py; lane_to_pixel(sc, rp, lane, &px, &py); pixel = (uint32_t) (py - F.crop_offset_y) * (uint32_t) F.width + (uint32_t) (px - F.crop_offset_x); }
    if (__ballot(finishing) == 0ull) return;
    const uint32_t prev = wave_prev(pixel, 0xfffffffeu), next = wave_next(pixel, 0xfffffffeu);
    float v[5] = { finishing ? L.x : 0.f, finishing ? L.y : 0.f, finishing ? L.z : 0.f, finishing ? 1.f : 0.f, (finishing && valid) ? 1.f : 0.f };
    wave_segmented_sums(v, pixel != prev || !finishing);
    if (finishing && pixel != next) {
        float *p = film + (size_t) pixel * F.channels;
        atomicAdd(p + 0, v[0]); atomicAdd(p + 1, v[1]); atomicAdd(p + 2, v[2]);
        if (F.has_alpha) { atomicAdd(p + 3, v[4]); atomicAdd(p + 4, v[3]); } else atomicAdd(p + 3, v[3]);
    }
}

template <int NC, int WI, typename Live, typename Flush>
DEV void film_walk(FilmRef F, bool have, const FilmFootprint &fp, const float (&v)[NC], Live live, Flush flush) {
    const uint32_t me = threadIdx.x & 63u, key = fp.key();
    const int count = F.fcount, n_cells = count * count;
    unsigned long long todo = __ballot(have);
    while (todo) {
        const int leader = __ffsll((long long) todo) - 1;
        const bool mine = have && key == (uint32_t) __shfl((int) key, leader);
        const int gx = __shfl(fp.pix, leader), gy = __shfl(fp.piy, leader);
        float t[NC];
#pragma unroll
        for (int k = 0; k < NC; ++k) t[k] = 0.f;
        for (int ys = 0, ci = 0; ys < count; ++ys) {
            const float wy = mine ? rfilter_eval(F, fp.rely + (float) ys) : 0.f;
            for (int xs = 0; xs < count; ++xs, ++ci) {
                const float w = mine ? wy * rfilter_eval(F, fp.relx + (float) xs) : 0.f;
                const bool keep = (int) me == (ci & 63);
#pragma unroll
                for (int k = 0; k < NC; ++k) {
                    if (!live(k)) continue;
                    const float s = wave_sum(mine ? v[k] * w : 0.f);
                    if (keep) t[k] = s;
                }
                if ((ci & 63) != 63 && ci != n_cells - 1) continue;
                const int cell = (ci & ~63) + (int) me;
                bool add = false;
#pragma unroll
                for (int k = 0; k < NC; ++k) add = add || ((WI < 0 || k == WI) ? t[k] != 0.f : t[k] != t[k]);
                if (cell <= ci && add) {
                    const int cy = cell / count, cx = cell - cy * count;
                    const int x = gx - F.crop_offset_x + cx, y = gy - F.crop_offset_y + cy;
                    if (x >= 0 && x < F.width && y >= 0 && y < F.height) flush(x, y, t);
                }
#pragma unroll
                for (int k = 0; k < NC; ++k) t[k] = 0.f;
            }
        }
        todo &= ~__ballot(mine);
    }
}
```

liverrenderer_amd/csrc/kernels.h:

```cpp
#pragma once
#include "dshade.h"
#include "record.h"

namespace lrt {

#ifndef LRT_STAMP_KIND
#define LRT_STAMP_KIND 0
#endif
struct StampClock {
    unsigned long long *acc; unsigned long long t; bool on;
    DEV void start(unsigned long long *a, bool enable) { acc = a; on = enable; t = on ? __builtin_amdgcn_s_memtime() : 0ull; }
    DEV void at(int k) { if (on) { const unsigned long long now = __builtin_amdgcn_s_memtime(); if ((threadIdx.x & 63u) == 0) atomicAdd(&acc[k], now - t); t = now; } }
};

template <bool LD>
DEV uint64_t lane_rng_inc(RpRef rp, uint32_t lane) {
    if (LD) {
        const uint32_t pixel = (rp.log2_spp != 0xffffffffu) ? (lane >> rp.log2_spp) : (lane / rp.spp);
        uint32_t v0, v1; tea32(rp.base_seed, rp.spp * pixel + rp.seed, &v0, &v1);
        return (uint64_t) v0 | ((uint64_t) (rp.pass_index * rp.spp + (lane - pixel * rp.spp)) << 32);
    }
    uint32_t v0, v1; tea32(rp.seed_value, lane, &v0, &v1);
    return ((uint64_t) v1 << 1) | 1u;
}
// ... 54 lines not shown
    for (int i = 0; i < 4; ++i) r[i] = fma_(m[4 * i + 2], p.z, fma_(m[4 * i + 1], p.y, fma_(m[4 * i + 0], p.x, m[4 * i + 3])));
    V3 near_p(r[0] / r[3], r[1] / r[3], r[2] / r[3]);
    V3 d = normalize(near_p);
    Ray ray;
    ray.o = V3(sc.cam.to_world[3], sc.cam.to_world[7], sc.cam.to_world[11]);
    ray.d = xform_vec12(sc.cam.to_world, d);
    float inv_z = rcp(d.z), near_t = sc.cam.near_clip * inv_z, far_t = sc.cam.far_clip * inv_z;
    ray.o = ray.o + ray.d * near_t;
    ray.maxt = far_t - near_t;
    return ray;
}

template <bool LD>
DEV PathState generate_camera_path(SceneRef sc, RpRef rp, const uint32_t *__restrict__ pixel_list, uint64_t j) {
    uint32_t lane;
    if (pixel_list) { uint32_t pj = (rp.log2_spp != 0xffffffffu) ? (uint32_t) (j >> rp.log2_spp) : (uint32_t) (j / rp.spp); lane = pixel_list[pj] * rp.spp + (uint32_t) (j - (uint64_t) pj * rp.spp); }
    else lane = (uint32_t) j;
    SamplerT<LD> rng = lane_rng_pass_start<LD>(rp, lane, j);
    int px, py; lane_to_pixel(sc, rp, lane, &px, &py);
    float jx, jy; rng.next2(jx, jy);
    float spx = (float) px + jx, spy = (float) py + jy;
    Ray ray = camera_ray(sc, fma_(spx, sc.film.scale_x, sc.film.offset_x), fma_(spy, sc.film.scale_y, sc.film.offset_y));
    PathState s;
    s.o = ray.o; s.d = ray.d; s.maxt = ray.maxt; s.eta = 1.f; s.tp = V3(1.f); s.res = V3(0.f); s.lp = V3(0.f); s.last_pdf = 1.f; s.lane = lane;
    s.tdepth = 0.f; s.si_t = kInf; s.ff_t = u2f(0x7fc00000u); s.bio_dist = u2f(0x7fc00000u); s.bio_hep = false; s.hit = make_float4(0.f, 0.f, 0.f, 0.f);
    for (int a = 0; a < 2; ++a) for (int i = 0; i < 3; ++i) for (int j = 0; j < 3; ++j) s.W[a][i][j] = 1.f;
    bool env_visible = !rp.hide_emitters && sc.env.type >= 0;
    uint32_t flags = env_visible ? PF_VALID : 0u;
    if (rp.integrator == LRT_INTEGRATOR_PATH) flags |= PF_SPECULAR;
    else {
        if (!rp.hide_emitters) flags |= PF_SPECULAR;
        uint32_t channel = min((uint32_t) (rng.next() * 3.f), 2u);
        flags |= channel << PF_CHANNEL_SHIFT;
        flags |= (uint32_t) (sc.cam.medium + 1) << PF_MEDIUM_SHIFT;
        if (rp.integrator == LRT_INTEGRATOR_BIOVOLPATH06) flags |= PF_BIO_EMIT | PF_BIO_FULL;
    }
    s.flags = flags; s.rng_state = rng.state; s.rng_word = lane_rng_word<LD>(rng);
    return s;
}

#include "film.h"

template <bool HET, typename SMP, typename TR, typename CNT>
DEV V3 volpath_sample_emitter(SceneRef sc, SMP &rng, V3 ref_p, V3 ref_n, bool ref_is_surface, uint32_t ref_shape, V3 ref_geo_n,
                              int medium, uint32_t channel, DirSample *ds_out, const TR &tr, CNT &n_shadow) {
    V3 transmittance(1.f);
    float sx, sy; rng.next2(sx, sy);
    DirSample ds; V3 emitter_val = sample_emitter_direction<TR::kExt>(sc, ref_p, sx, sy, &ds);
    *ds_out = ds;
    if (ds.pdf == 0.f) return V3(0.f);
    Ray ray = spawn_ray_to(ref_p, ref_n, ds.p);
    float max_dist = ray.maxt;
    if (ref_is_surface) { const DShape sd = tab(sc.shapes, ref_shape, sc.one_shape); if (is_medium_transition(sd)) medium = target_medium(sd, ray.d, ref_geo_n); }
    float total_dist = 0.f;
    SI si; si.valid = false; si.t = 0.f; si.shape = 0; si.p = V3(0.f); si.n = V3(0.f);
    bool needs_intersection = true, active = true;
    while (active) {
        float remaining_dist = max_dist - total_dist;
        ray.maxt = remaining_dist;
        if (!(remaining_dist > 0.f)) { rng.skip(1); break; }
        bool escaped_medium = false, active_medium = medium >= 0, active_surface = !active_medium;
        if (!active_medium) rng.skip(1);
        if (active_medium) {
            const DMedium M = tab(sc.media, medium);
            const bool het = HET && M.het;
            MI mei = het ? het_sample_interaction(M, tab(sc.het, medium), ray, rng.next()) : medium_sample_interaction(M, ray, rng.next(), channel);
            if (mei.valid() && !het) ray.maxt = fmin_(mei.t, remaining_dist);
            if (needs_intersection) {
                bool elide = mei.valid() && !sc.has_null_bsdf && !het;
                if (!elide) { n_shadow++; Hit h = tr.closest(ray); si = tr.surface(sc, ray, h); }
                else { si.valid = false; si.t = kInf; }
            }
            if (si.t < mei.t) mei.t = kInf;
            needs_intersection = false;
            bool spectral = M.has_spectral_extinction;
            if (spectral) {
                float t = fmin_(remaining_dist, fmin_(mei.t, si.t)) - mei.mint;
                V3 tr = exp_neg(t, mei.combined);
                V3 ffp = (si.t < mei.t || mei.t > remaining_dist) ? tr : tr * mei.combined;
                float tr_pdf = idx3(ffp, channel);
                transmittance = transmittance * ((tr_pdf > 0.f) ? div_uniform(tr, tr_pdf) : V3(0.f));
            }
            if ((mei.t > remaining_dist) && mei.valid()) total_dist = ds.dist;
            if (mei.t > remaining_dist) mei.t = kInf;
            escaped_medium = !mei.valid();
            active_medium = mei.valid();
            if (active_medium) {
                total_dist += mei.t;
                ray.o = mei.p;
                si.t = si.t - mei.t;
                if (spectral) transmittance = transmittance * mei.sigma_n;
                else transmittance = transmittance * (mei.sigma_n / mei.combined);
            }
        }
        bool intersect = active_surface && needs_intersection;
        if (intersect) { n_shadow++; Hit h = tr.closest(ray); si = tr.surface(sc, ray, h); needs_intersection = false; }
        active_surface = active_surface || escaped_medium;
        if (active_surface) total_dist += si.t;
        active_surface = active_surface && si.valid && !active_medium;
        if (active_surface) {
            transmittance = transmittance * bsdf_null_transmission(sc, tab(sc.shapes, si.shape, sc.one_shape).bsdf);
            ray = spawn_ray(si.p, si.n, ray.d);
        }
        ray.maxt = remaining_dist;
        needs_intersection = needs_intersection || active_surface;
        active = (active_medium || active_surface) && any_nonzero(transmittance);
        if (active_surface) { const DShape sd = tab(sc.shapes, si.shape, sc.one_shape); if (is_medium_transition(sd)) medium = target_medium(sd, ray.d, si.n); }
    }
    return transmittance * emitter_val;
}

struct WaveCount {
    unsigned long long *c;
    DEV void operator++(int) {
        const unsigned long long m = __ballot(true);
        if ((threadIdx.x & 63u) == (uint32_t) (__ffsll((long long) m) - 1)) atomicAdd(c, (unsigned long long) __popcll(m));
    }
};

template <bool HET, bool CLOSED = false, typename SMP, typename TR, typename CNT>
DEV bool volpath_iteration(SceneRef sc, RpRef rp, PathState &s, SMP &rng, const TR &tr, CNT &n_shadow, CNT &n_extra, bool fresh = false, StampClock *clk = nullptr,
                           unsigned long long *guard = nullptr) {
    constexpr bool PRE = !HET;
    uint32_t depth = s.flags & PF_DEPTH_MASK;
    bool proven_empty = (s.flags & PF_NOHIT) != 0;
    float ff_t = s.ff_t;
    const bool needs_intersection = !(HET && (s.flags & PF_HAVE_SI));
    bool act_null_scatter = false;
    Hit hkeep; hkeep.t = s.hit.x; hkeep.u = s.hit.y; hkeep.v = s.hit.z; hkeep.prim = f2u(s.hit.w);
    if (PRE) { hkeep.t = kInf; hkeep.u = hkeep.v = 0.f; hkeep.prim = 0xffffffffu; }
    int medium = (int) ((s.flags & PF_MEDIUM_MASK) >> PF_MEDIUM_SHIFT) - 1;
    const uint32_t channel = (s.flags >> PF_CHANNEL_SHIFT) & 3u;
    bool specular_chain = (s.flags & PF_SPECULAR) != 0, valid_ray = (s.flags & PF_VALID) != 0;
    const uint32_t max_depth = (uint32_t) rp.max_depth;
    V3 throughput = s.tp, result = CLOSED ? V3(0.f) : s.res;
    bool broken = false;
    float eta = s.eta;
    Ray ray; ray.o = s.o; ray.d = s.d; ray.maxt = s.maxt;
    auto commit = [&]() {
        s.tp = throughput; s.res = result; s.eta = eta; s.o = ray.o; s.d = ray.d; s.maxt = ray.maxt;
        s.flags = (depth & PF_DEPTH_MASK) | ((uint32_t) (medium + 1) << PF_MEDIUM_SHIFT) | (channel << PF_CHANNEL_SHIFT) |
                  (specular_chain ? PF_SPECULAR : 0u) | (valid_ray ? PF_VALID : 0u);
    };
    auto termination_stage = [&]() -> bool {
        bool a = any_nonzero(throughput);
        const float q = fmin_(max3(throughput) * sqr(eta), .95f);
        const bool perform_rr = depth > (uint32_t) rp.rr_depth;
        if (a) { const float u = rng.next(); a = (u < q) || !perform_rr; }
        if (perform_rr) throughput = throughput * rcp(q);
        return a && depth < max_depth;
    };
    uint32_t nohit = 0;
    float cache_t = u2f(0x7fc00000u);
    auto free_flight_stage = [&]() {
        if (medium < 0) return;
        const DMedium M = tab(sc.media, medium);
        cache_t = medium_sampled_t(M, rng.next(), channel);
        if (sc.grid.enabled) { const MI m2 = medium_interaction_at(M, ray, cache_t); if (m2.valid() && segment_free_of_surfaces(sc.grid, ray.o, ray.d, m2.t)) nohit = PF_NOHIT; }
    };
    bool active = true;
    if (!PRE) active = termination_stage();
    else if (fresh) { active = termination_stage(); if (active) { free_flight_stage(); ff_t = cache_t; proven_empty = nohit != 0; nohit = 0; cache_t = u2f(0x7fc00000u); } }
    if (!active) { commit(); return false; }

    bool active_medium = medium >= 0, active_surface = !active_medium;
    bool act_medium_scatter = false, escaped_medium = false;
    MI mei; mei.t = kInf;
    SI si; si.valid = false; si.t = kInf;
    if (!active_medium) rng.skip(2);
    if (active_medium) {
        const DMedium M = tab(sc.media, medium);
        const bool het = HET && M.het;
        if (PRE) mei = medium_interaction_at(M, ray, ff_t);
        else { const float sample = rng.next(); mei = het ? het_sample_interaction(M, tab(sc.het, medium), ray, sample) : medium_sample_interaction(M, ray, sample, channel); }
        if (mei.valid() && !het) ray.maxt = mei.t;
        if (!needs_intersection) si = surface_of(tr, sc, ray, hkeep);
        else if (!proven_empty) {
            hkeep = tr.closest(ray);
            if (PRE) { si.valid = hkeep.prim != 0xffffffffu; si.t = si.valid ? hkeep.t : kInf; }
            else si = tr.surface(sc, ray, hkeep);
        }
        if (si.t < mei.t) mei.t = kInf;
        if (M.has_spectral_extinction) {
            float t = fmin_(mei.t, si.t) - mei.mint;
            V3 tr = exp_neg(t, mei.combined);
            V3 pdf = (si.t < mei.t) ? tr : tr * mei.combined;
            float tr_pdf = idx3(pdf, channel);
            throughput = throughput * ((tr_pdf > 0.f) ? div_uniform(tr, tr_pdf) : V3(0.f));
        }
        escaped_medium = !mei.valid();
        active_medium = mei.valid();
        if (!active_medium) rng.skip(1);
        if (active_medium) {
            const float u_null = rng.next();
            if (HET) {
                const float null_scatter_prob = mean3(mei.sigma_n / mei.combined);
                act_null_scatter = u_null < null_scatter_prob;
                if (M.has_spectral_extinction && act_null_scatter) throughput = throughput * (mei.sigma_n / null_scatter_prob);
            }
            act_medium_scatter = !act_null_scatter;
            if (act_medium_scatter) { depth += 1; s.lp = mei.p; }
        }
    }
    active = active && depth < max_depth;
    act_medium_scatter = act_medium_scatter && active;
    if (HET && act_null_scatter) { ray.o = mei.p; hkeep.t = si.t - mei.t; }
    if (clk) clk->at(2);
    if (!act_medium_scatter) rng.skip(3);
    if (act_medium_scatter) {
        const DMedium M = tab(sc.media, medium);
        if (HET && M.het) {
            if (M.has_spectral_extinction) throughput = throughput * (mei.sigma_s / mean3(mei.sigma_t / mei.combined));
            else throughput = throughput * (mei.sigma_s / mei.sigma_t);
        } else if (M.has_spectral_extinction) throughput = throughput * V3(M.w_spec[0], M.w_spec[1], M.w_spec[2]);
        else throughput = throughput * V3(M.w_plain[0], M.w_plain[1], M.w_plain[2]);
        bool sample_emitters = M.sample_emitters != 0;
        valid_ray = true;
        specular_chain = !sample_emitters;
        if (!sample_emitters) rng.skip(1);
        if (sample_emitters) {
            bool rejected = false;
            if (sc.nee_fast_reject) {
                SMP saved = rng;
                float sx, sy; rng.next2(sx, sy);
                float u3 = rng.next();
                const float lo = 9.5367431640625e-7f, hi = 1.f - 9.5367431640625e-7f;
                bool interior = sc.env.type == LRT_EMITTER_CONSTANT || (sx > lo && sx < hi && sy > lo && sy < hi);
                rejected = interior;
                if (!(1.f - u3 >= idx3(V3(M.nee_vmin[0], M.nee_vmin[1], M.nee_vmin[2]), channel))) {
                    float sampled_t = 0.f + (-m_log(1.f - u3) / idx3(V3(M.sigma_t[0], M.sigma_t[1], M.sigma_t[2]), channel));
                    V3 cc(sc.env.bsphere_c[0], sc.env.bsphere_c[1], sc.env.bsphere_c[2]);
                    float dist = 2.f * fmax_(sc.env.bsphere_r, norm(mei.p - cc));
                    rejected = interior && sampled_t <= dist * 0.998f - 1e-3f;
                }
                if (!rejected) rng = saved;
            }
            if (!rejected && CLOSED) {
                float sx, sy; rng.next2(sx, sy);
                DirSample ds; (void) sample_emitter_direction<TR::kExt>(sc, mei.p, sx, sy, &ds);
                if (ds.pdf != 0.f) {
                    const Ray r2 = spawn_ray_to(mei.p, V3(0.f), ds.p);
                    if (!(r2.maxt > 0.f)) rng.skip(1);
                    else { const MI m2 = medium_sample_interaction(M, r2, rng.next(), channel); if (!m2.valid()) n_shadow++; }
                }
            } else if (!rejected) {
                DirSample ds;
                V3 emitted = volpath_sample_emitter<HET>(sc, rng, mei.p, V3(0.f), false, 0, V3(0.f), medium, channel, &ds, tr, n_shadow);
                float phase_val = phase_eval(M, mei.wi, ds.d);
                V3 c = throughput * phase_val * emitted * mis_weight(ds.pdf, ds.delta ? 0.f : phase_val);
                result = result + c;
            }
        }
        (void) rng.next();
        float s2x, s2y; rng.next2(s2x, s2y);
        V3 wo; float phase_pdf; phase_sample(M, mei.wi, s2x, s2y, &wo, &phase_pdf);
        if (phase_pdf > 0.f) {
            ray = spawn_ray(mei.p, V3(0.f), wo);
            s.last_pdf = phase_pdf;
        }
    }
    active_surface = active_surface || escaped_medium;
    bool intersect = active_surface && !escaped_medium;
    if (PRE) {
        Hit h = hkeep;
        if (intersect) h = tr.closest(ray);
        if (active_surface) si = tr.surface(sc, ray, h);
    } else if (intersect) { Hit h = tr.closest(ray); si = tr.surface(sc, ray, h); }
    if (active_surface) {
        if (!CLOSED && rp.hide_emitters && depth == 0 && intersect) {
            bool skip = si.valid && tab(sc.shapes, si.shape, sc.one_shape).emitter >= 0;
            if (skip) {
                Ray r2 = spawn_ray(si.p, si.n, ray.d);
                bool a = true; Hit h; h.prim = 0xffffffffu; h.t = kInf; h.u = h.v = 0.f;
                while (a) {
                    h = tr.closest(r2);
                    a = hit_on_emitter(tr, sc, h);
                    if (a) { SI s2 = surface_of(tr, sc, r2, h); r2 = spawn_ray(s2.p, s2.n, r2.d); }
                }
                si = surface_of(tr, sc, r2, h);
            }
        }
        bool count_direct = (depth == 0) || specular_chain;
        int emitter = CLOSED ? (si.valid ? -1 : sc.env.emitter) : si_emitter(sc, si);
        bool active_e = emitter >= 0 && !(depth == 0 && rp.hide_emitters);
        if (active_e) {
            if (CLOSED) { broken = broken || !count_direct; result = result + throughput * emitter_eval_env(sc, -si.wi); }
            else {
                float emitter_pdf = 1.f;
                if (!count_direct) emitter_pdf = pdf_emitter_direction<TR::kExt>(sc, s.lp, si, emitter);
                V3 emitted = emitter_eval(sc, emitter, si);
                V3 contrib = count_direct ? throughput * emitted : throughput * mis_weight(s.last_pdf, emitter_pdf) * emitted;
                result = result + contrib;
            }
        }
    }
    active_surface = active_surface && si.valid;
    if (!active_surface) rng.skip(3);
    if (active_surface) {
        const DShape sd = tab(sc.shapes, si.shape, sc.one_shape);
        int b = sd.bsdf;
        int flags = tab(sc.bsdfs, b, sc.one_shape).flags;
        bool active_e = !CLOSED && (flags & F_SMOOTH) && (depth + 1 < max_depth);
        if (!active_e) rng.skip(1);
        if (active_e) {
            DirSample ds;
            V3 emitted = volpath_sample_emitter<HET>(sc, rng, si.p, si.n, true, si.shape, si.n, medium, channel, &ds, tr, n_shadow);
            V3 wo = si.sh.to_local(ds.d);
            V3 bsdf_val = bsdf_eval(sc, b, si, wo);
            float bpdf = bsdf_pdf(sc, b, si, wo);
            V3 c = throughput * bsdf_val * mis_weight(ds.pdf, ds.delta ? 0.f : bpdf) * emitted;
            result = result + c;
        }
        float s1 = rng.next(), s2x, s2y; rng.next2(s2x, s2y);
        const BSDFSample bs = bsdf_sample<CLOSED>(sc, b, si, s1, s2x, s2y);
        throughput = throughput * bs.weight;
        eta *= bs.eta;
        ray = spawn_ray(si.p, si.n, si.sh.to_world(bs.wo));
        bool non_null = !(bs.type & F_NULL);
        if (non_null) { depth += 1; s.lp = si.p; s.last_pdf = bs.pdf; valid_ray = true; }
        specular_chain = specular_chain || (non_null && (bs.type & F_DELTA));
        specular_chain = specular_chain && !(bs.type & F_SMOOTH);
        if (is_medium_transition(sd)) medium = target_medium(sd, ray.d, si.n);
    }
    active = active && (active_surface || active_medium);
    if (clk) clk->at(3);
    if (PRE) {
        if (active) { if (!termination_stage()) { active = false; n_extra++; } else free_flight_stage(); }
        if (clk) clk->at(4);
    } else if (active) {
        SMP pk = rng;
        bool a2 = any_nonzero(throughput);
        float q2 = fmin_(max3(throughput) * sqr(eta), .95f);
        if (a2) { float u = pk.next(); a2 = (u < q2) || !(depth > (uint32_t) rp.rr_depth); }
        a2 = a2 && depth < max_depth;
        if (!a2) { active = false; n_extra++; rng = pk; }
        else if (medium >= 0 && sc.grid.enabled && !(HET && act_null_scatter)) {
            const DMedium M = tab(sc.media, medium);
            if (!(HET && M.het)) {
                const float t2 = medium_sampled_t(M, pk.next(), channel);
                const MI m2 = medium_interaction_at(M, ray, t2);
                if (m2.valid() && segment_free_of_surfaces(sc.grid, ray.o, ray.d, m2.t)) nohit = PF_NOHIT;
            }
        }
    }
    commit();
    s.flags |= nohit; s.ff_t = cache_t;
#ifndef LRT_CLOSED_NO_GUARD
    if (CLOSED && (broken || (active && !(result.x == 0.f && result.y == 0.f && result.z == 0.f)))) atomicAdd(guard, 1ull);
#endif
    if (HET && act_null_scatter && active) { s.flags |= PF_HAVE_SI; s.hit = make_float4(hkeep.t, hkeep.u, hkeep.v, u2f(hkeep.prim)); }
    return active;
}

template <typename SMP, typename TR>
DEV bool path_iteration(SceneRef sc, RpRef rp, PathState &s, SMP &rng, const TR &tr, uint32_t &n_shadow) {
    uint32_t depth = s.flags & PF_DEPTH_MASK;
    bool prev_bsdf_delta = (s.flags & PF_SPECULAR) != 0, valid_ray = (s.flags & PF_VALID) != 0;
    const uint32_t max_depth = (uint32_t) rp.max_depth;
    V3 throughput = s.tp, result = s.res;
    float eta = s.eta;
    Ray ray; ray.o = s.o; ray.d = s.d; ray.maxt = s.maxt;
    auto commit = [&]() {
        s.tp = throughput; s.res = result; s.eta = eta; s.o = ray.o; s.d = ray.d; s.maxt = ray.maxt;
        s.flags = (depth & PF_DEPTH_MASK) | (prev_bsdf_delta ? PF_SPECULAR : 0u) | (valid_ray ? PF_VALID : 0u);
    };
    if (max_depth == 0) { commit(); return false; }
    Hit pi = tr.closest(ray);
    if (rp.hide_emitters && depth == 0) {
        bool skip = hit_on_emitter(tr, sc, pi);
        if (skip) {
            SI s0 = surface_of(tr, sc, ray, pi);
            Ray r2 = spawn_ray(s0.p, s0.n, ray.d);
            bool a = true; Hit h; h.prim = 0xffffffffu; h.t = kInf; h.u = h.v = 0.f;
            while (a) {
                h = tr.closest(r2);
                a = hit_on_emitter(tr, sc, h);
                if (a) { SI s2 = surface_of(tr, sc, r2, h); r2 = spawn_ray(s2.p, s2.n, r2.d); }
            }
            pi = h; ray = r2;
        }
    }
    SI si = surface_of(tr, sc, ray, pi);
    int emitter = si_emitter(sc, si);
    if (emitter >= 0) {
        float em_pdf = 0.f;
        if (!prev_bsdf_delta) em_pdf = pdf_emitter_direction<TR::kExt>(sc, s.lp, si, emitter);
        float mis_bsdf = mis_weight(s.last_pdf, em_pdf);
        V3 em = (s.last_pdf > 0.f) ? emitter_eval(sc, emitter, si) : V3(0.f);
        em = em * mis_bsdf;
        result = V3(fma_(throughput.x, em.x, result.x), fma_(throughput.y, em.y, result.y), fma_(throughput.z, em.z, result.z));
    }
    bool active_next = (depth + 1 < max_depth) && si.valid;
    if (!active_next) {
        float a0, a1; rng.next2(a0, a1); (void) rng.next(); rng.next2(a0, a1); (void) rng.next();
        if (si.valid && !(tab(sc.bsdfs, tab(sc.shapes, si.shape, sc.one_shape).bsdf, sc.one_shape).flags & F_NULL)) valid_ray = true;
        commit(); return false;
    }
    const DShape sd = tab(sc.shapes, si.shape, sc.one_shape);
    int b = sd.bsdf;
    bool active_em = (tab(sc.bsdfs, b, sc.one_shape).flags & F_SMOOTH) != 0;
    DirSample ds; ds.pdf = 0.f; ds.delta = false; ds.d = V3(0.f);
    V3 em_weight(0.f), wo(0.f);
    float sx, sy; rng.next2(sx, sy);
    if (active_em) {
        em_weight = sample_emitter_direction<TR::kExt>(sc, si.p, sx, sy, &ds);
        if (ds.pdf != 0.f) {
            Ray sr = spawn_ray_to(si.p, si.n, ds.p);
            n_shadow++;
            Hit h = tr.any(sr);
            if (h.prim != 0xffffffffu) { em_weight = V3(0.f); ds.pdf = 0.f; }
        }
        active_em = ds.pdf != 0.f;
        wo = si.sh.to_local(ds.d);
    }
    float s1 = rng.next(), s2x, s2y; rng.next2(s2x, s2y);
    V3 bsdf_val = bsdf_eval(sc, b, si, wo);
    float bpdf = bsdf_pdf(sc, b, si, wo);
    const BSDFSample bs = bsdf_sample(sc, b, si, s1, s2x, s2y);
    const V3 bsdf_weight = bs.weight;
    if (active_em) {
        float mis_em = ds.delta ? 1.f : mis_weight(ds.pdf, bpdf);
        V3 c = bsdf_val * em_weight * mis_em;
        result = V3(fma_(throughput.x, c.x, result.x), fma_(throughput.y, c.y, result.y), fma_(throughput.z, c.z, result.z));
    }
    ray = spawn_ray(si.p, si.n, si.sh.to_world(bs.wo));
    throughput = throughput * bsdf_weight;
    eta *= bs.eta;
    valid_ray = valid_ray || !(bs.type & F_NULL);
    s.lp = si.p; s.last_pdf = bs.pdf; prev_bsdf_delta = (bs.type & F_DELTA) != 0;
    depth += 1;
    float tmax = max3(throughput);
    float rr_prob = fmin_(tmax * sqr(eta), .95f);
    bool rr_active = depth >= (uint32_t) rp.rr_depth, rr_continue = rng.next() < rr_prob;
    if (rr_active) throughput = throughput * rcp(rr_prob);
    bool active = active_next && (!rr_active || rr_continue) && (tmax != 0.f);
    commit();
    return active;
}

}
#include "kernels_bio.h"
#include "kernels_mis.h"
namespace lrt {

template <RecordLayout LAYOUT = RecordLayout::Wide, bool READLANE = true, bool COMPACT = false, bool LONGQ = false>
DEV void retire_and_compact_wave(SceneRef sc, RpRef rp, bool had_path, bool alive, const PathState &s,
                                 float *__restrict__ film, float *__restrict__ sample_out, uint64_t sample_base,
                                 const LRT_CONST DPathStreams &qout, size_t pool, uint32_t P, uint32_t *s_out , StampClock *clk = nullptr) {
    const uint32_t lane_in_wave = threadIdx.x & 63u;
    const int region = !(s.flags & PF_MEDIUM_MASK) ? 2 : ((s.flags & PF_NOHIT) ? 0 : ((LONGQ && (s.flags & PF_LONG_QUERY)) ? 3 : 1));
    const unsigned long long m0 = __ballot(alive && region == 0), m1 = __ballot(alive && region == 1), m2 = __ballot(alive && region == 2);
    const unsigned long long m3 = LONGQ ? __ballot(alive && region == 3) : 0ull;
    uint32_t base = 0;
    if (lane_in_wave < (LONGQ ? 4u : 3u)) {
        const uint32_t c = (uint32_t) __popcll(lane_in_wave == 0 ? m0 : (lane_in_wave == 1 ? m1 : ((!LONGQ || lane_in_wave == 2) ? m2 : m3)));
        if (c) base = atomicAdd(&s_out[lane_in_wave], c);
    }
    uint32_t b;
    if (READLANE) {
        const uint32_t b0 = (uint32_t) __builtin_amdgcn_readlane((int) base, 0), b1 = (uint32_t) __builtin_amdgcn_readlane((int) base, 1), b2 = (uint32_t) __builtin_amdgcn_readlane((int) base, 2);
        b = region == 0 ? b0 : (region == 1 ? b1 : b2);
        if (LONGQ) { const uint32_t b3 = (uint32_t) __builtin_amdgcn_readlane((int) base, 3); if (region == 3) b = b3; }
    } else b = __shfl(base, region);
    if (clk) clk->at(5);
    if (alive) {
        const unsigned long long mine = region == 0 ? m0 : (region == 1 ? m1 : ((!LONGQ || region == 2) ? m2 : m3));
        const uint32_t slot = b + (uint32_t) __popcll(mine & ((1ull << lane_in_wave) - 1ull));
        store_state<LAYOUT, COMPACT>(qout, pool + (region == 0 ? slot : (region == 1 ? P + slot : ((!LONGQ || region == 2) ? 2u * P - 1u - slot : P - 1u - slot))), s);
    }
    if (clk) clk->at(6);
    if (rp.pass_out && had_path && !alive) rp.pass_out[lane_local_index(rp, s.lane)] = s.rng_state;
    finish_paths_wave(sc, rp, film, sample_out, sample_base, had_path && !alive, s.lane, s.res, (s.flags & PF_VALID) != 0);
}

template <int INTEGRATOR, int BLOCK, bool LDS_BVH, bool LD, bool COMPACT = false, bool EXT = false>
__global__ void __launch_bounds__(BLOCK, BLOCK == 512 ? 2 : (BLOCK == 768 ? 3 : 4))
k_render(ScenePtr scp, LaunchPtr lp) {
    SceneRef sc = *scp;
    const LRT_CONST DLaunch &A = *lp;
    RpRef rp = A.rp;
// ... 399 lines not shown
```

liverrenderer_amd/csrc/kernels_prb.h:

```cpp
#pragma once
#include "kernels.h"

namespace lrt {

struct PrbGrads { float sigma_t[3], albedo[3], g; };

DEV float hg_dlog_dg(float g, float c) {
    float temp = 1.f + sqr(g) + 2.f * g * c;
    return -2.f * g / (1.f - sqr(g)) - 1.5f * (2.f * g + 2.f * c) / temp;
}

DEV float het_null_dlog_dscale(const DMedium &M, float sigma_t, float sigma_n) { return sigma_n > 0.f ? -(sigma_t / sigma_n) / M.scale : 0.f; }

template <bool HET, bool SCATTER = false, typename SMP, typename TR>
DEV V3 prb_sample_emitter(SceneRef sc, SMP &rng, V3 ref_p, V3 ref_n, bool ref_is_surface, uint32_t ref_shape, V3 ref_geo_n,
                          int medium, uint32_t channel, DirSample *ds_out, const TR &tr, uint32_t &n_shadow, V3 *seg_sum, int grad_medium,
                          V3 coef = V3(0.f), float *__restrict__ dgrid = nullptr) {
    float sx, sy; rng.next2(sx, sy);
    DirSample ds; V3 emitter_val = sample_emitter_direction(sc, ref_p, sx, sy, &ds);
    *ds_out = ds;
    bool active = ds.pdf != 0.f;
    if (!active) { emitter_val = V3(0.f); medium = -1; }
    if (ref_is_surface) { const DShape sd = tab(sc.shapes, ref_shape, sc.one_shape); if (is_medium_transition(sd)) medium = target_medium(sd, ds.d, ref_geo_n); }
    Ray ray = spawn_ray_to(ref_p, ref_n, ds.p);
    float max_dist = ray.maxt, total_dist = 0.f;
    SI si; si.valid = false; si.t = 0.f; si.shape = 0; si.p = V3(0.f); si.n = V3(0.f);
    bool needs_intersection = true;
    V3 transmittance(1.f), sum(0.f);
    while (active) {
        float remaining_dist = max_dist - total_dist;
        ray.maxt = remaining_dist;
        active = active && remaining_dist > 0.f;
        needs_intersection = needs_intersection && active;
        if (needs_intersection) { n_shadow++; Hit h = tr.closest(ray); si = tr.surface(sc, ray, h); }
        needs_intersection = false;
        bool active_medium = active && medium >= 0, active_surface = active && !active_medium;
        V3 tr_multiplier(1.f);
        float seg_t = 0.f, scale_t = 0.f, mei_t = kInf; bool escaped_medium = false;
        V3 null_dlog(0.f);
        if (!active_medium) rng.skip(1);
        if (active_medium) {
            const DMedium M = tab(sc.media, medium);
            const bool graded = grad_medium < 0 || medium == grad_medium;
            if (HET && M.het) {
                MI mei = het_sample_interaction(M, tab(sc.het, medium), ray, rng.next());
                if (si.t < mei.t) mei.t = kInf;
                escaped_medium = !mei.valid(); active_medium = mei.valid();
                if (active_medium) {
                    ray.o = mei.p; si.t = si.t - mei.t; mei_t = mei.t;
                    tr_multiplier = mei.sigma_n / mei.combined;
                    if (graded) null_dlog = V3(het_null_dlog_dscale(M, mei.sigma_t.x, mei.sigma_n.x), het_null_dlog_dscale(M, mei.sigma_t.x, mei.sigma_n.y), het_null_dlog_dscale(M, mei.sigma_t.x, mei.sigma_n.z));
                    if (SCATTER && graded) {
                        const float a = (tr_multiplier.x > 0.f ? -coef.x / mei.sigma_n.x : 0.f) + (tr_multiplier.y > 0.f ? -coef.y / mei.sigma_n.y : 0.f) +
                                        (tr_multiplier.z > 0.f ? -coef.z / mei.sigma_n.z : 0.f);
                        const DHetMedium H = tab(sc.het, medium);
                        if (a != 0.f) grid_scatter(H, dgrid, xform_point12(H.to_local, mei.p), a);
                    }
                }
            } else {
                (void) rng.next();
                float t = fmin_(remaining_dist, si.t);
                seg_t = fmin_(t, si.t) - 0.f;
                tr_multiplier = V3(m_exp(-seg_t * M.sigma_t[0]), m_exp(-seg_t * M.sigma_t[1]), m_exp(-seg_t * M.sigma_t[2]));
                scale_t = graded ? -seg_t * M.scale : 0.f;
                escaped_medium = true; active_medium = false;
            }
        }
        active_surface = (active_surface || escaped_medium) && si.valid && !active_medium;
        if (active_surface) tr_multiplier = tr_multiplier * bsdf_null_transmission(sc, tab(sc.shapes, si.shape, sc.one_shape).bsdf);
        if (escaped_medium && active_surface) {
            if (tr_multiplier.x > 0.f) sum.x += scale_t;
            if (tr_multiplier.y > 0.f) sum.y += scale_t;
            if (tr_multiplier.z > 0.f) sum.z += scale_t;
        }
        if (HET && active_medium) {
            if (tr_multiplier.x > 0.f) sum.x += null_dlog.x;
            if (tr_multiplier.y > 0.f) sum.y += null_dlog.y;
            if (tr_multiplier.z > 0.f) sum.z += null_dlog.z;
        }
        transmittance = transmittance * tr_multiplier;
        if (active_surface) ray = spawn_ray(si.p, si.n, ray.d);
        ray.maxt = remaining_dist;
        needs_intersection = needs_intersection || active_surface;
        active = active && (active_medium || active_surface) && any_nonzero(transmittance);
        if (active) total_dist += (HET && active_medium) ? mei_t : si.t;
        if (active_surface) { const DShape sd = tab(sc.shapes, si.shape, sc.one_shape); if (is_medium_transition(sd)) medium = target_medium(sd, ray.d, si.n); }
    }
    *seg_sum = sum;
    return emitter_val * transmittance;
}

template <bool ADJOINT, bool HET, bool GRID = false, typename SMP, typename TR>
DEV bool prb_iteration(SceneRef sc, RpRef rp, PathState &s, SMP &rng, const TR &tr, uint32_t &n_shadow,
                       V3 delta_L, PrbGrads &G, float *__restrict__ dgrid = nullptr) {
    uint32_t depth = s.flags & PF_DEPTH_MASK;
    const bool proven_empty = (s.flags & PF_NOHIT) != 0;
    const bool needs_intersection = !(HET && (s.flags & PF_HAVE_SI));
    Hit hkeep; hkeep.t = s.hit.x; hkeep.u = s.hit.y; hkeep.v = s.hit.z; hkeep.prim = f2u(s.hit.w);
    int medium = (int) ((s.flags & PF_MEDIUM_MASK) >> PF_MEDIUM_SHIFT) - 1;
    const uint32_t channel = (s.flags >> PF_CHANNEL_SHIFT) & 3u;
    bool specular_chain = (s.flags & PF_SPECULAR) != 0, valid_ray = (s.flags & PF_VALID) != 0;
    const uint32_t max_depth = (uint32_t) rp.max_depth;
    V3 throughput = s.tp, L = s.res;
    float eta = s.eta;
    Ray ray; ray.o = s.o; ray.d = s.d; ray.maxt = s.maxt;
    auto commit = [&]() {
        s.tp = throughput; s.res = L; s.eta = eta; s.o = ray.o; s.d = ray.d; s.maxt = ray.maxt;
        s.flags = (depth & PF_DEPTH_MASK) | ((uint32_t) (medium + 1) << PF_MEDIUM_SHIFT) | (channel << PF_CHANNEL_SHIFT) |
                  (specular_chain ? PF_SPECULAR : 0u) | (valid_ray ? PF_VALID : 0u);
    };
    bool active = any_nonzero(throughput);
    float q = fmin_(max3(throughput) * sqr(eta), 0.99f);
    bool perform_rr = depth > (uint32_t) rp.rr_depth;
    if (active) { float u = rng.next(); active = (u < q) || !perform_rr; }
    if (perform_rr) throughput = throughput * rcp(q);
    bool active_medium = active && medium >= 0, active_surface = active && !active_medium;
    bool escaped_medium = false, act_medium_scatter = false, act_null_scatter = false, in_medium_segment = false, het = false;
    MI mei; mei.t = kInf; mei.wi = -ray.d; mei.p = V3(0.f); mei.sigma_t = V3(0.f); mei.sigma_n = V3(0.f); mei.combined = V3(1.f);
    SI si; si.valid = false; si.t = kInf;
    V3 weight(1.f);
    float seg_t = 0.f, scatter_prob = 1.f;
    if (!active_medium) rng.skip(1);
    if (active_medium) {
        const DMedium M = tab(sc.media, medium);
        het = HET && M.het;
        mei = het ? het_sample_interaction(M, tab(sc.het, medium), ray, rng.next()) : medium_sample_interaction(M, ray, rng.next(), channel);
        if (mei.valid() && !het) ray.maxt = mei.t;
        if (!needs_intersection) si = compute_si(sc, ray, hkeep);
        else if (!proven_empty) { hkeep = tr.closest(ray); si = tr.surface(sc, ray, hkeep); }
        if (si.t < mei.t) mei.t = kInf;
        seg_t = fmin_(mei.t, si.t) - mei.mint;
        V3 tr(m_exp(-seg_t * mei.combined.x), m_exp(-seg_t * mei.combined.y), m_exp(-seg_t * mei.combined.z));
        V3 pdf = (si.t < mei.t) ? tr : tr * mei.combined;
        float tr_pdf = idx3(pdf, channel);
        weight = (tr_pdf > 0.f) ? tr / tr_pdf : V3(0.f);
        escaped_medium = !mei.valid();
        active_medium = mei.valid();
        in_medium_segment = true;
    }
    if (HET) {
        if (!active_medium) rng.skip(1);
        else {
            scatter_prob = mean3(mei.sigma_t / mei.combined);
            act_null_scatter = rng.next() >= scatter_prob;
            if (act_null_scatter) weight = weight * (mei.sigma_n / (1.f - scatter_prob));
        }
    }
    if (active_medium && !act_null_scatter) { act_medium_scatter = true; depth += 1; s.lp = mei.p; }
    active = active && depth < max_depth;
    act_medium_scatter = act_medium_scatter && active;
    if (HET && act_null_scatter) { ray.o = mei.p; hkeep.t = si.t - mei.t; }
    if (act_medium_scatter) weight = weight * (HET ? mei.sigma_s / scatter_prob : mei.sigma_s);
    throughput = throughput * weight;
    const int gm = rp.grad_medium;
    if (ADJOINT && in_medium_segment && (gm < 0 || medium == gm)) {
        const DMedium M = tab(sc.media, medium);
        auto term = [&](float w, float l, float dl, float st, float al, float sn, float &gs, float &ga) {
            float Lo = l / fmax_(1e-8f, w);
            if (het) {
                const float dlog = act_medium_scatter ? 1.f / M.scale : (act_null_scatter ? het_null_dlog_dscale(M, mei.sigma_t.x, sn) : 0.f);
                gs += dl * Lo * (w * dlog);
                if (act_medium_scatter && al > 0.f) ga += dl * Lo * (w / al);
                return;
            }
            float dws = w * (-seg_t) + (act_medium_scatter && st > 0.f ? w / st : 0.f);
            if (!(seg_t < kInf)) dws = 0.f;
            gs += dl * Lo * dws * M.scale;
            if (act_medium_scatter && al > 0.f) ga += dl * Lo * (w / al);
        };
#ifdef LRT_EXPERIMENT
        if (rp.pad1 && s.lane == rp.pad1 - 1u) printf("  [dev] medium term: depth %u seg_t %.9g w %.9g %.9g %.9g L %.9g %.9g %.9g dl %.9g scatter %d\n", depth, seg_t, weight.x, weight.y, weight.z, L.x, L.y, L.z, delta_L.x, (int) act_medium_scatter);
#endif
        term(weight.x, L.x, delta_L.x, M.sigma_t[0], M.albedo[0], mei.sigma_n.x, G.sigma_t[0], G.albedo[0]);
        term(weight.y, L.y, delta_L.y, M.sigma_t[1], M.albedo[1], mei.sigma_n.y, G.sigma_t[1], G.albedo[1]);
        term(weight.z, L.z, delta_L.z, M.sigma_t[2], M.albedo[2], mei.sigma_n.z, G.sigma_t[2], G.albedo[2]);
        if (GRID && het && (act_medium_scatter || act_null_scatter)) {
            auto coef = [&](float w, float l, float dl, float sn) {
                const float c = dl * (l / fmax_(1e-8f, w)) * w;
                if (act_medium_scatter) return mei.sigma_t.x > 0.f ? c / mei.sigma_t.x : 0.f;
                return sn > 0.f ? -c / sn : 0.f;
            };
            const float a = coef(weight.x, L.x, delta_L.x, mei.sigma_n.x) + coef(weight.y, L.y, delta_L.y, mei.sigma_n.y) + coef(weight.z, L.z, delta_L.z, mei.sigma_n.z);
            const DHetMedium H = tab(sc.het, medium);
            if (a != 0.f) grid_scatter(H, dgrid, xform_point12(H.to_local, mei.p), a);
        }
    }
    active_surface = active_surface || escaped_medium;
    bool intersect = active_surface && !escaped_medium;
    if (intersect) { Hit h = tr.closest(ray); si = tr.surface(sc, ray, h); }
    if (rp.hide_emitters && intersect && depth == 0 && si.valid && tab(sc.shapes, si.shape, sc.one_shape).emitter >= 0) {
        Ray r2 = spawn_ray(si.p, si.n, ray.d);
        bool a = true; Hit h; h.prim = 0xffffffffu; h.t = kInf; h.u = h.v = 0.f;
        while (a) {
            h = tr.closest(r2);
            a = h.prim != 0xffffffffu && tab(sc.shapes, sc.face_shape[h.prim], sc.one_shape).emitter >= 0;
            if (a) { SI s2 = compute_si(sc, r2, h); r2 = spawn_ray(s2.p, s2.n, r2.d); }
        }
        si = compute_si(sc, r2, h);
    }
    if (active_surface) {
        bool count_direct = (depth == 0) || specular_chain;
        int emitter = si_emitter(sc, si);
        bool active_e = emitter >= 0 && !(depth == 0 && rp.hide_emitters);
        if (active_e) {
            float emitter_pdf = pdf_emitter_direction(sc, s.lp, si, emitter);
            V3 emitted = emitter_eval(sc, emitter, si);
            V3 contrib = count_direct ? throughput * emitted : throughput * mis_weight(s.last_pdf, emitter_pdf) * emitted;
            L = ADJOINT ? L - contrib : L + contrib;
#ifdef LRT_EXPERIMENT
            if (rp.pad1 && s.lane == rp.pad1 - 1u) printf("  [dev] %s emitter hit: depth %u contrib %.9g %.9g %.9g L after %.9g %.9g %.9g\n", ADJOINT ? "adjoint" : "primal", depth, contrib.x, contrib.y, contrib.z, L.x, L.y, L.z);
#endif
        }
    }
    active_surface = active_surface && si.valid;
    int b = active_surface ? tab(sc.shapes, si.shape, sc.one_shape).bsdf : 0;
    bool active_e_surface = active_surface && (tab(sc.bsdfs, b, sc.one_shape).flags & F_SMOOTH) && (depth + 1 < max_depth);
    bool sample_emitters = act_medium_scatter ? (tab(sc.media, medium).sample_emitters != 0) : false;
    if (act_medium_scatter) specular_chain = !sample_emitters;
    bool active_e_medium = act_medium_scatter && sample_emitters;
    if (!(active_e_surface || active_e_medium)) rng.skip(1);
    if (active_e_surface || active_e_medium) {
        DirSample ds; V3 seg_sum;
        V3 rp_ = active_e_medium ? mei.p : si.p, rn = active_e_medium ? V3(0.f) : si.n;
        SMP rng_march = rng;
        V3 emitted = prb_sample_emitter<HET>(sc, rng, rp_, rn, active_e_surface, active_e_surface ? si.shape : 0u, si.n, medium, channel, &ds, tr, n_shadow, &seg_sum, gm);
        V3 nee_weight; float nee_pdf;
        if (active_e_surface) { V3 wo = si.sh.to_local(ds.d); nee_weight = bsdf_eval(sc, b, si, wo); nee_pdf = bsdf_pdf(sc, b, si, wo); }
        else { float pv = phase_eval(tab(sc.media, medium), mei.wi, ds.d); nee_weight = V3(pv); nee_pdf = pv; }
        V3 contrib = throughput * nee_weight * mis_weight(ds.pdf, ds.delta ? 0.f : nee_pdf) * emitted;
        L = ADJOINT ? L - contrib : L + contrib;
#ifdef LRT_EXPERIMENT
        if (rp.pad1 && s.lane == rp.pad1 - 1u) printf("  [dev] %s nee: depth %u surface %d contrib %.9g %.9g %.9g L after %.9g %.9g %.9g seg_sum %.9g %.9g %.9g\n", ADJOINT ? "adjoint" : "primal", depth, (int) active_e_surface, contrib.x, contrib.y, contrib.z, L.x, L.y, L.z, seg_sum.x, seg_sum.y, seg_sum.z);
#endif
        if (ADJOINT) {
            G.sigma_t[0] += delta_L.x * contrib.x * seg_sum.x; G.sigma_t[1] += delta_L.y * contrib.y * seg_sum.y; G.sigma_t[2] += delta_L.z * contrib.z * seg_sum.z;
            if (GRID) {
                const V3 coef = delta_L * contrib;
                if (any_nonzero(coef)) {
                    DirSample ds2; V3 seg2;
                    (void) prb_sample_emitter<HET, true>(sc, rng_march, rp_, rn, active_e_surface, active_e_surface ? si.shape : 0u, si.n, medium, channel, &ds2, tr, n_shadow, &seg2, gm, coef, dgrid);
                }
            }
            if (active_e_medium && tab(sc.media, medium).phase == LRT_PHASE_HG && (gm < 0 || medium == gm))
                G.g += (delta_L.x * contrib.x + delta_L.y * contrib.y + delta_L.z * contrib.z) * hg_dlog_dg(tab(sc.media, medium).g, dot(ds.d, mei.wi));
        }
    }
    if (!act_medium_scatter) rng.skip(2);
    if (act_medium_scatter) {
        valid_ray = true;
        const DMedium M = tab(sc.media, medium);
        (void) rng.next();
        float s2x, s2y; rng.next2(s2x, s2y);
        V3 wo; float phase_pdf; phase_sample(M, mei.wi, s2x, s2y, &wo, &phase_pdf);
        act_medium_scatter = phase_pdf > 0.f;
        if (act_medium_scatter) {
            if (ADJOINT && M.phase == LRT_PHASE_HG && (gm < 0 || medium == gm)) {
                float pe = phase_eval(M, mei.wi, wo), dlg = hg_dlog_dg(M.g, dot(wo, mei.wi));
                G.g += delta_L.x * (pe * (L.x / fmax_(1e-8f, pe))) * dlg;
                G.g += delta_L.y * (pe * (L.y / fmax_(1e-8f, pe))) * dlg;
                G.g += delta_L.z * (pe * (L.z / fmax_(1e-8f, pe))) * dlg;
            }
            ray = spawn_ray(mei.p, V3(0.f), wo);
            s.last_pdf = phase_pdf;
        }
    }
    if (!active_surface) rng.skip(2);
    if (active_surface) {
        const DShape sd = tab(sc.shapes, si.shape, sc.one_shape);
        float s1 = rng.next(), s2x, s2y; rng.next2(s2x, s2y);
        const BSDFSample bs = bsdf_sample(sc, b, si, s1, s2x, s2y);
        active_surface = bs.pdf > 0.f;
        if (active_surface) {
            throughput = throughput * bs.weight;
            eta *= bs.eta;
            ray = spawn_ray(si.p, si.n, si.sh.to_world(bs.wo));
            bool non_null = !(bs.type & F_NULL);
            if (non_null) { depth += 1; s.lp = si.p; s.last_pdf = bs.pdf; valid_ray = true; }
            specular_chain = specular_chain || (non_null && (bs.type & F_DELTA));
            specular_chain = specular_chain && !(bs.type & F_SMOOTH);
            if (is_medium_transition(sd)) medium = target_medium(sd, ray.d, si.n);
        }
    }
    active = active && (active_surface || active_medium);
    uint32_t nohit = 0;
    if (active && medium >= 0 && sc.grid.enabled && !(HET && (act_null_scatter || tab(sc.media, medium).het))) {
        SMP pk = rng;
        bool a2 = any_nonzero(throughput);
        float q2 = fmin_(max3(throughput) * sqr(eta), 0.99f);
        if (a2) { float u = pk.next(); a2 = (u < q2) || !(depth > (uint32_t) rp.rr_depth); }
        if (a2) {
            const DMedium M = tab(sc.media, medium);
            MI m2 = medium_sample_interaction(M, ray, pk.next(), channel);
            if (m2.valid() && segment_free_of_surfaces(sc.grid, ray.o, ray.d, m2.t)) nohit = PF_NOHIT;
        }
    }
    commit();
    s.flags |= nohit;
    if (HET && act_null_scatter && active) { s.flags |= PF_HAVE_SI; s.hit = make_float4(hkeep.t, hkeep.u, hkeep.v, u2f(hkeep.prim)); }
    return active;
}

DEV V3 lane_delta_L(SceneRef sc, RpRef rp, uint32_t lane, const float *__restrict__ grad_image, const float *__restrict__ wfilm) {
    FilmRef F = sc.film;
    const int T = F.has_alpha ? 4 : 3;
    if (F.rfilter == LRT_RFILTER_BOX) {
        int px, py; lane_to_pixel(sc, rp, lane, &px, &py);
        size_t p = film_pixel_index(F, px, py);
        float w = (float) rp.spp;
        return V3(grad_image[p * T] / w, grad_image[p * T + 1] / w, grad_image[p * T + 2] / w);
    }
    int px, py; lane_to_pixel(sc, rp, lane, &px, &py);
    float jx, jy; lane_jitter(rp, lane, lane_local_index(rp, lane), jx, jy);
    const FilmFootprint fp = film_footprint(F, px, py, jx, jy);
    const int count = F.fcount;
    V3 dL(0.f);
    for (int ys = 0; ys < count; ++ys) {
        int y = fp.piy - F.crop_offset_y + ys;
        if (y < 0 || y >= F.height) continue;
        float wy = rfilter_eval(F, fp.rely + (float) ys);
        for (int xs = 0; xs < count; ++xs) {
            int x = fp.pix - F.crop_offset_x + xs;
            if (x < 0 || x >= F.width) continue;
            size_t p = (size_t) y * F.width + x;
            float w = wy * rfilter_eval(F, fp.relx + (float) xs), wp = wfilm[p]; if (wp == 0.f) wp = 1.f;
            float f = w / wp;
            dL = dL + V3(grad_image[p * T] * f, grad_image[p * T + 1] * f, grad_image[p * T + 2] * f);
        }
    }
    return dL;
}

template <bool ADJOINT, int BLOCK, bool LDS_BVH, bool LD, bool HET = false>
__global__ void __launch_bounds__(BLOCK, 4)
k_render_prb(ScenePtr scp, LaunchPtr lp) {
    constexpr bool GRID = false;
#include "kernels_prb_body.h"
}

template <int BLOCK, bool LDS_BVH, bool LD>
__global__ void __launch_bounds__(BLOCK, 4)
k_render_prb_grid(ScenePtr scp, LaunchPtr lp) {
    constexpr bool ADJOINT = true, HET = true, GRID = true;
#include "kernels_prb_body.h"
}

}
```

liverrenderer_amd/csrc/kernels_prb_body.h:

```cpp
    constexpr RecordLayout LAYOUT = record_layout(HET ? LRT_INTEGRATOR_VOLPATH_HET : LRT_INTEGRATOR_PRBVOLPATH);
    SceneRef sc = *scp;
    const LRT_CONST DLaunch &A = *lp;
    RpRef rp = A.rp;
    const LRT_CONST DLdsInfo &li = A.li;
    const uint32_t P = A.P;
    float4 *__restrict__ L_buf = A.L_buf; const float *__restrict__ grad_image = A.grad_image; const float *__restrict__ wfilm = A.wfilm;
    extern __shared__ __align__(16) unsigned char smem[];
    __shared__ uint32_t s_in[3], s_out[3], s_ticket, s_fresh;
    __shared__ unsigned long long s_fresh_base;
    __shared__ double s_grad[7];
    const uint32_t tid = threadIdx.x, lane_in_wave = tid & 63u;
    LdsScene L{};
    if (LDS_BVH) {
        const uint4 *src = li.blob; uint4 *dst = reinterpret_cast<uint4 *>(smem);
        for (uint32_t k = tid; k < li.blob_bytes / 16u; k += BLOCK) dst[k] = src[k];
        L.nodes = reinterpret_cast<const float4 *>(smem + li.nodes_off); L.verts = reinterpret_cast<const float4 *>(smem + li.verts_off);
        L.tris = reinterpret_cast<const uint2 *>(smem + li.tris_off);
        L.n_faces = sc.n_faces; L.root_is_leaf = (uint32_t) sc.root_is_leaf; L.root_first = sc.root_leaf_first; L.root_count = sc.root_leaf_count;
    }
    const LdsTracer<BLOCK> tr_lds{ L, reinterpret_cast<uint16_t *>(smem + li.stack_off) + tid };
    const GlobalTracer tr_glb{ sc, reinterpret_cast<int *>(smem) + tid };
    const size_t pool = (size_t) blockIdx.x * 2u * P;
    uint32_t parity = 0;
    if (tid == 0) { s_in[0] = s_in[1] = s_in[2] = 0; }
    if (tid < 7) s_grad[tid] = 0.0;
    bool lanes_left = true;
    uint32_t n_shadow = 0, n_trips = 0, n_loaded = 0;
    for (;;) {
        if (tid == 0) {
            const uint32_t want = P - (s_in[0] + s_in[1] + s_in[2]);
            uint32_t got = 0; unsigned long long base = 0;
            if (want && lanes_left) {
                base = atomicAdd(&A.cnt->next_lane, (unsigned long long) want);
                if (base < rp.n_lanes) got = (uint32_t) (rp.n_lanes - base < (unsigned long long) want ? rp.n_lanes - base : (unsigned long long) want);
                lanes_left = base + want < rp.n_lanes;
            }
            s_fresh = got; s_fresh_base = base; s_ticket = 0; s_out[0] = s_out[1] = s_out[2] = 0;
        }
        __syncthreads();
        const uint32_t n_a = s_in[0], n_c = s_in[1], n_s = s_in[2], fresh = s_fresh;
        const unsigned long long fresh_base = s_fresh_base;
        if (n_a + n_c + n_s + fresh == 0) break;
        const uint32_t ta = (n_a + 63u) >> 6, tc = (n_c + 63u) >> 6, ts = (n_s + 63u) >> 6, tf = (fresh + 63u) >> 6, tm = ta + tc;
        for (;;) {
            uint32_t t = 0;
            if (lane_in_wave == 0) t = atomicAdd(&s_ticket, 1u);
            t = (uint32_t) __builtin_amdgcn_readfirstlane((int) t);
            if (t >= tm + ts + tf) break;
            bool had_path = false, alive = false;
            PathState s; s.flags = 0; s.lane = 0; s.res = V3(0.f);
            float4 dl = make_float4(0.f, 0.f, 0.f, 0.f);
            if (t < tm + ts) {
                uint32_t i;
                if (t < ta) { i = (t << 6) + lane_in_wave; had_path = i < n_a; }
                else if (t < tm) { i = ((t - ta) << 6) + lane_in_wave; had_path = i < n_c; i += P; }
                else { i = ((t - tm) << 6) + lane_in_wave; had_path = i < n_s; i = 2u * P - 1u - i; }
                if (had_path) { load_state<LAYOUT>(parity ? A.q1 : A.q0, pool + i, s); dl = (parity ? A.dl1 : A.dl0)[pool + i]; n_loaded += 1; }
            } else {
                const uint32_t i = ((t - tm - ts) << 6) + lane_in_wave;
                had_path = i < fresh;
                if (had_path) {
                    const unsigned long long slot = fresh_base + i;
                    s = generate_camera_path<LD>(sc, rp, A.pixel_list, A.lane_begin + slot);
                    s.flags = PF_SPECULAR | (s.flags & (3u << PF_CHANNEL_SHIFT));
                    V3 dL(0.f);
                    if (ADJOINT) { float4 l = L_buf[slot]; s.res = V3(l.x, l.y, l.z); dL = lane_delta_L(sc, rp, s.lane, grad_image, wfilm); }
                    dl = make_float4(dL.x, dL.y, dL.z, u2f((uint32_t) slot));
                }
            }
            PrbGrads G; G.sigma_t[0] = G.sigma_t[1] = G.sigma_t[2] = G.albedo[0] = G.albedo[1] = G.albedo[2] = G.g = 0.f;
            if (had_path) {
                SamplerT<LD> rng = lane_rng_resume<LD>(rp, s.lane, s.rng_state);
                alive = LDS_BVH ? prb_iteration<ADJOINT, HET, GRID>(sc, rp, s, rng, tr_lds, n_shadow, V3(dl.x, dl.y, dl.z), G, GRID ? A.dgrid : nullptr)
                                : prb_iteration<ADJOINT, HET, GRID>(sc, rp, s, rng, tr_glb, n_shadow, V3(dl.x, dl.y, dl.z), G, GRID ? A.dgrid : nullptr);
                s.rng_state = rng.state;
                n_trips += 1;
            }
            if (!ADJOINT) {
                if (L_buf) { if (had_path && !alive) L_buf[f2u(dl.w)] = make_float4(s.res.x, s.res.y, s.res.z, (s.flags & PF_VALID) ? 1.f : 0.f); }
                else finish_paths_wave(sc, rp, A.film, A.sample_out, A.sample_base, had_path && !alive, s.lane, s.res, (s.flags & PF_VALID) != 0);
            } else {
                float g[7] = { G.sigma_t[0], G.sigma_t[1], G.sigma_t[2], G.albedo[0], G.albedo[1], G.albedo[2], G.g };
#pragma unroll
                for (int k = 0; k < 7; ++k) {
                    const float v = wave_sum(g[k]);
                    if (lane_in_wave == 0 && v != 0.f) atomicAdd(&s_grad[k], (double) v);
                }
            }
            const int region = !(s.flags & PF_MEDIUM_MASK) ? 2 : ((s.flags & PF_NOHIT) ? 0 : 1);
            const unsigned long long m0 = __ballot(alive && region == 0), m1 = __ballot(alive && region == 1), m2 = __ballot(alive && region == 2);
            uint32_t base = 0;
            if (lane_in_wave < 3) { const uint32_t c = (uint32_t) __popcll(lane_in_wave == 0 ? m0 : (lane_in_wave == 1 ? m1 : m2)); if (c) base = atomicAdd(&s_out[lane_in_wave], c); }
            const uint32_t b0 = (uint32_t) __builtin_amdgcn_readlane((int) base, 0), b1 = (uint32_t) __builtin_amdgcn_readlane((int) base, 1), b2 = (uint32_t) __builtin_amdgcn_readlane((int) base, 2);
            const uint32_t b = region == 0 ? b0 : (region == 1 ? b1 : b2);
            if (alive) {
                const uint32_t slot = b + (uint32_t) __popcll((region == 0 ? m0 : (region == 1 ? m1 : m2)) & ((1ull << lane_in_wave) - 1ull));
                const uint32_t rec = region == 0 ? slot : (region == 1 ? P + slot : 2u * P - 1u - slot);
                store_state<LAYOUT>(parity ? A.q0 : A.q1, pool + rec, s); (parity ? A.dl0 : A.dl1)[pool + rec] = dl;
            }
        }
        __syncthreads();
        if (tid == 0) { s_in[0] = s_out[0]; s_in[1] = s_out[1]; s_in[2] = s_out[2]; }
        parity ^= 1u;
    }
    if (ADJOINT && tid < 7 && s_grad[tid] != 0.0) atomicAdd(&A.grads[tid], s_grad[tid]);
    for (int off = 32; off > 0; off >>= 1) {
        n_shadow += __shfl_down(n_shadow, off); n_trips += __shfl_down(n_trips, off); n_loaded += __shfl_down(n_loaded, off);
    }
    if (lane_in_wave == 0) {
        if (n_shadow) atomicAdd(&A.cnt->n_shadow, (unsigned long long) n_shadow);
        if (n_trips) atomicAdd(&A.cnt->n_iter, (unsigned long long) n_trips);
        if (n_loaded) atomicAdd(&A.cnt->n_records, (unsigned long long) n_loaded);
    }
```

liverrenderer_amd/csrc/scene_prep.cpp:

```cpp
#include "scene_prep.h"
#include <cmath>
#include <cstring>
#include <cstdlib>
#include <algorithm>
#include <stdexcept>
#include <string>

namespace lrt {

PrepOptions PrepOptions::from_env() {
    PrepOptions o;
    if (getenv("LRT_BVH_LEAF")) o.bvh_leaf = std::max(1, atoi(getenv("LRT_BVH_LEAF")));
    o.no_lds_bvh = getenv("LRT_NO_LDS_BVH") != nullptr;
    o.no_dist_grid = getenv("LRT_NO_DIST_GRID") != nullptr;
    if (getenv("LRT_DIST_GRID_RES")) o.dist_grid_res = std::max(8, std::min(256, atoi(getenv("LRT_DIST_GRID_RES"))));
    o.no_nee_reject = getenv("LRT_NO_NEE_REJECT") != nullptr;
    return o;
}

static void m4_mul(const float *a, const float *b, float *r) {
    for (int i = 0; i < 4; ++i) for (int j = 0; j < 4; ++j) { float s = a[4 * i] * b[j]; for (int k = 1; k < 4; ++k) s = fmaf(a[4 * i + k], b[4 * k + j], s); r[4 * i + j] = s; }
}
static void m4_ident(float *m) { for (int i = 0; i < 16; ++i) m[i] = (i % 5 == 0) ? 1.f : 0.f; }

static void build_camera(const lrt_scene_desc &d, DCamera &cam, DFilm &film) {
    const lrt_film_desc &F = d.film; const lrt_sensor_desc &C = d.sensor;
    float fw = (float) F.width, fh = (float) F.height;
    float rsx = (float) F.crop_width / fw, rsy = (float) F.crop_height / fh, rox = (float) F.crop_offset_x / fw, roy = (float) F.crop_offset_y / fh;
    float aspect = fw / fh, recip = 1.f / (C.far_clip - C.near_clip);
    float tn = (float) tan((double) (C.fov_x * .5f) * (3.14159265358979323846 / 180.0));
    (void) recip;
    float S1i[16], T1i[16], S2i[16], T2i[16], Pit[16], t0[16], t1[16], t2[16], it[16];
    m4_ident(S1i); S1i[0] = 1.f / (1.f / rsx); S1i[5] = 1.f / (1.f / rsy); S1i[10] = 1.f / 1.f;
    m4_ident(T1i); T1i[12] = rox; T1i[13] = roy; T1i[14] = -0.f;
    m4_ident(S2i); S2i[0] = 1.f / -0.5f; S2i[5] = 1.f / (-0.5f * aspect); S2i[10] = 1.f;
    m4_ident(T2i); T2i[12] = 1.f; T2i[13] = 1.f / aspect; T2i[14] = -0.f;
    float Pinv[16]; m4_ident(Pinv); Pinv[0] = tn; Pinv[5] = tn; Pinv[10] = 0.f; Pinv[15] = 1.f / C.near_clip; Pinv[11] = 1.f;
    Pinv[14] = (C.near_clip - C.far_clip) / (C.far_clip * C.near_clip);
    for (int i = 0; i < 4; ++i) for (int j = 0; j < 4; ++j) Pit[4 * i + j] = Pinv[4 * j + i];
    m4_mul(S1i, T1i, t0); m4_mul(t0, S2i, t1); m4_mul(t1, T2i, t2); m4_mul(t2, Pit, it);
    for (int i = 0; i < 4; ++i) for (int j = 0; j < 4; ++j) cam.s2c[4 * i + j] = it[4 * j + i];
    memcpy(cam.to_world, C.to_world, sizeof(float) * 12);
    cam.near_clip = C.near_clip; cam.far_clip = C.far_clip; cam.medium = C.medium;
    cam.ppo_x = fw * C.principal_point_offset_x / (float) F.crop_width; cam.ppo_y = fh * C.principal_point_offset_y / (float) F.crop_height;

    film.width = F.crop_width; film.height = F.crop_height; film.crop_offset_x = F.crop_offset_x; film.crop_offset_y = F.crop_offset_y;
    film.scale_x = 1.f / (float) F.crop_width; film.scale_y = 1.f / (float) F.crop_height;
    film.offset_x = -(float) F.crop_offset_x * film.scale_x; film.offset_y = -(float) F.crop_offset_y * film.scale_y;
    film.has_alpha = F.has_alpha; film.channels = F.has_alpha ? 5 : 4; film.rfilter = F.rfilter;
    film.rf_radius = 0.5f; film.rf_inv_radius = 1.f;
    if (F.rfilter == LRT_RFILTER_GAUSSIAN) {
        float stddev = F.rfilter_param; film.rf_radius = 4.f * stddev;
        static const double coeff[10] = { 9.992604880e-1, -4.977025247e-1, 1.222248550e-1, -1.932406282e-2, 2.136713061e-3,
                                          -1.679873860e-4, 9.202145248e-6, -3.329417433e-7, 7.128382794e-9, -6.821193280e-11 };
        double sc = 1; for (int i = 0; i < 10; ++i) { film.rf_coeff[i] = (float) (coeff[i] * sc); sc /= (double) stddev * (double) stddev; }
        float x = film.rf_radius * film.rf_radius, x2 = x * x, x4 = x2 * x2, x8 = x4 * x4; const float *c = film.rf_coeff;
        float a0 = fmaf(x, c[1], c[0]), a1 = fmaf(x, c[3], c[2]), a2 = fmaf(x, c[5], c[4]), a3 = fmaf(x, c[7], c[6]), a4 = fmaf(x, c[9], c[8]);
        float b0 = fmaf(x2, a1, a0), b1 = fmaf(x2, a3, a2), c0 = fmaf(x4, b1, b0);
        film.rf_coeff[0] -= fmaf(x8, a4, c0);
    } else if (F.rfilter == LRT_RFILTER_TENT) { film.rf_radius = F.rfilter_param; film.rf_inv_radius = 1.f / film.rf_radius; }
    film.fn = (int) ceilf(film.rf_radius - .5f); film.fcount = 2 * film.fn + 1;
}

static void inverse3(const float *m16, float *out9) {
    double m[3][3]; for (int i = 0; i < 3; ++i) for (int j = 0; j < 3; ++j) m[i][j] = m16[4 * i + j];
    double det = m[0][0] * (m[1][1] * m[2][2] - m[1][2] * m[2][1]) - m[0][1] * (m[1][0] * m[2][2] - m[1][2] * m[2][0]) + m[0][2] * (m[1][0] * m[2][1] - m[1][1] * m[2][0]);
    double id = 1.0 / det;
    out9[0] = (float) ((m[1][1] * m[2][2] - m[1][2] * m[2][1]) * id); out9[1] = (float) ((m[0][2] * m[2][1] - m[0][1] * m[2][2]) * id); out9[2] = (float) ((m[0][1] * m[1][2] - m[0][2] * m[1][1]) * id);
    out9[3] = (float) ((m[1][2] * m[2][0] - m[1][0] * m[2][2]) * id); out9[4] = (float) ((m[0][0] * m[2][2] - m[0][2] * m[2][0]) * id); out9[5] = (float) ((m[0][2] * m[1][0] - m[0][0] * m[1][2]) * id);
    out9[6] = (float) ((m[1][0] * m[2][1] - m[1][1] * m[2][0]) * id); out9[7] = (float) ((m[0][1] * m[2][0] - m[0][0] * m[2][1]) * id); out9[8] = (float) ((m[0][0] * m[1][1] - m[0][1] * m[1][0]) * id);
}

static uint32_t log2i_ceil(uint32_t v) { uint32_t r = 0; while ((1u << r) < v) ++r; return r; }

static void build_hierarchy(const std::vector<float> &lum, uint32_t w, uint32_t h, DEnv &E, std::vector<float> &out) {
    uint32_t npx = w - 1, npy = h - 1;
    E.patch_size[0] = 1.f / (float) npx; E.patch_size[1] = 1.f / (float) npy;
    E.inv_patch_size[0] = (float) npx; E.inv_patch_size[1] = (float) npy;
    E.max_patch[0] = npx - 1; E.max_patch[1] = npy - 1;
    uint32_t max_level = log2i_ceil(std::max(npx, npy));
    struct L { uint32_t w, h, off; };
    std::vector<L> lv; uint32_t total = 0;
    auto add = [&](uint32_t lw, uint32_t lh) { lv.push_back({ lw, lh, total }); total += (lw * lh + 3u) & ~3u; };
    add(w, h);
    uint32_t lx = npx, ly = npy;
    for (int level = (int) max_level; level >= 0; --level) { lx += lx & 1u; ly += ly & 1u; add(lx, ly); lx >>= 1; ly >>= 1; }
    if (lv.size() > LRT_MAX_HIER_LEVELS) throw std::runtime_error("environment map too large for the sampling hierarchy");
    out.assign(total, 0.f);
    auto index = [](uint32_t x, uint32_t y, uint32_t width) { return ((x & 1u) | (((x & ~1u) | (y & 1u)) << 1)) + ((y & ~1u) * width); };
    float *l0 = &out[lv[0].off], *l1 = &out[lv[1].off];
    const float *in = lum.data(); double sum = 0.0;
    for (uint32_t y = 0; y < npy; ++y) { for (uint32_t x = 0; x < npx; ++x) { float avg = .25f * (in[0] + in[1] + in[w] + in[w + 1]); sum += (double) avg; l1[index(x, y, lv[1].w)] = avg; ++in; } ++in; }
    float scale = (float) ((double) (npx * npy) / sum);
    for (uint32_t i = 0; i < w * h; ++i) l0[i] = lum[i] * scale;
    for (uint32_t i = 0; i < lv[1].w * lv[1].h; ++i) l1[i] *= scale;
    lx = npx; ly = npy;
    for (uint32_t level = 2; level <= max_level + 1; ++level) {
        const float *a = &out[lv[level - 1].off]; float *b = &out[lv[level].off];
        lx = (lx + 1u) >> 1; ly = (ly + 1u) >> 1;
        for (uint32_t y = 0; y < ly; ++y) for (uint32_t x = 0; x < lx; ++x) { const float *d0 = a + index(x * 2, y * 2, lv[level - 1].w); b[index(x, y, lv[level].w)] = d0[0] + d0[1] + d0[2] + d0[3]; }
    }
    E.n_levels = (int) lv.size();
    for (size_t i = 0; i < lv.size(); ++i) { E.level_offset[i] = lv[i].off; E.level_width[i] = lv[i].w; }
}

struct LdsLayout {
    size_t nodes_b, verts_b, tris_b, stacks_b;
    size_t blob() const { return nodes_b + verts_b + tris_b; }
    size_t total() const { return blob() + stacks_b; }
};
static LdsLayout lds_layout(const HostBVH &b, uint32_t n_vertices) {
    return { b.nodes.size() / 16 * 64, ((size_t) n_vertices * 16 + 15) & ~size_t(15), (b.tris.size() / 12 * 8 + 15) & ~size_t(15), (size_t) 2 * (b.max_depth + 2) * 1024 };
}
size_t lds_image_bytes(const HostBVH &b, uint32_t n_vertices) { return lds_layout(b, n_vertices).total(); }

static bool lds_possible(const lrt_scene_desc &d, const PrepOptions &opt) { return d.n_faces > 0 && d.n_faces <= 32767 && d.n_vertices <= 65535 && !opt.no_lds_bvh; }
bool lds_image_fits(const lrt_scene_desc &d, const HostBVH &b, const PrepOptions &opt) {
    return lds_possible(d, opt) && b.nodes.size() / 16 <= 32767 && b.tris.size() / 12 <= 32767 && lds_image_bytes(b, d.n_vertices) <= opt.lds_limit;
}

static void build_lds_image(const lrt_scene_desc &d, const HostBVH &bvh, PreparedScene &P) {
    const LdsLayout lay = lds_layout(bvh, d.n_vertices);
    const size_t n_nodes = bvh.nodes.size() / 16, n_slots = bvh.tris.size() / 12, n_verts = d.n_vertices;
    const size_t nodes_b = lay.nodes_b, verts_b = lay.verts_b;
    std::vector<unsigned char> &blob = P.lds_blob; blob.assign(lay.blob(), 0);
    memcpy(blob.data(), bvh.nodes.data(), nodes_b);
    float *v = reinterpret_cast<float *>(blob.data() + nodes_b);
    for (size_t i = 0; i < n_verts; ++i) { v[4 * i] = d.positions[3 * i]; v[4 * i + 1] = d.positions[3 * i + 1]; v[4 * i + 2] = d.positions[3 * i + 2]; v[4 * i + 3] = 0.f; }
    uint16_t *t = reinterpret_cast<uint16_t *>(blob.data() + nodes_b + verts_b);
    for (size_t sl = 0; sl < n_slots; ++sl) {
        uint32_t f; memcpy(&f, &bvh.tris[12 * sl + 3], 4);
        for (int k = 0; k < 3; ++k) t[4 * sl + k] = (uint16_t) d.faces[3 * (size_t) f + k];
        t[4 * sl + 3] = (uint16_t) (f << 1);
    }
    for (size_t n = 0; n < n_nodes; ++n) {
        int32_t refs[4]; memcpy(refs, &bvh.nodes[16 * n + 12], 16);
        for (int c = 0; c < 2; ++c) if (refs[c] < 0 && refs[2 + c] > 0) t[4 * ((size_t) (uint32_t) ~refs[c] + (size_t) refs[2 + c] - 1) + 3] |= 1;
        uint32_t enc[2]; for (int c = 0; c < 2; ++c) enc[c] = refs[c] < 0 ? (0x8000u | (uint32_t) ~refs[c]) : (uint32_t) refs[c];
        memcpy(blob.data() + 64 * n + 48, enc, 8);
    }
    if (bvh.root_is_leaf && bvh.root_count) t[4 * ((size_t) bvh.root_first + bvh.root_count - 1) + 3] |= 1;
    P.lds.blob = nullptr; P.lds.blob_bytes = (uint32_t) blob.size(); P.lds.nodes_off = 0; P.lds.verts_off = (uint32_t) nodes_b; P.lds.tris_off = (uint32_t) (nodes_b + verts_b);
    P.lds.stack_off = (uint32_t) blob.size(); P.lds.total_bytes = (uint32_t) lay.total();
}

static void referenced_bounds(const lrt_scene_desc &d, const std::vector<DSphere> &spheres, float lo[3], float hi[3]) {
    for (int a = 0; a < 3; ++a) { lo[a] = INFINITY; hi[a] = -INFINITY; }
    for (uint32_t f = 0; f < 3 * d.n_faces; ++f) for (int a = 0; a < 3; ++a) { float v = d.positions[3 * (size_t) d.faces[f] + a]; lo[a] = std::min(lo[a], v); hi[a] = std::max(hi[a], v); }
    for (const DSphere &o : spheres) for (int a = 0; a < 3; ++a) { lo[a] = std::min(lo[a], o.center[a] - o.radius); hi[a] = std::max(hi[a], o.center[a] + o.radius); }
}
static void vertex_bounds(const lrt_scene_desc &d, const std::vector<DSphere> &spheres, float lo[3], float hi[3]) {
    for (int a = 0; a < 3; ++a) { lo[a] = INFINITY; hi[a] = -INFINITY; }
    for (uint32_t i = 0; i < d.n_vertices; ++i) for (int a = 0; a < 3; ++a) { lo[a] = fminf(lo[a], d.positions[3 * i + a]); hi[a] = fmaxf(hi[a], d.positions[3 * i + a]); }
    for (const DSphere &o : spheres) for (int a = 0; a < 3; ++a) { lo[a] = fminf(lo[a], o.center[a] - o.radius); hi[a] = fmaxf(hi[a], o.center[a] + o.radius); }
}

void prepare_geometry(const lrt_scene_desc &d, const PrepOptions &opt, PreparedScene &P) {
    DScene &sc = P.sc;
    memset(&sc, 0, sizeof(sc));
    std::vector<DSphere> &spheres = P.spheres;
    for (uint32_t i = 0; i < d.n_shapes; ++i) {
        const lrt_shape_desc &s = d.shapes[i];
        if (s.kind != LRT_SHAPE_SPHERE) continue;
        DSphere o; memset(&o, 0, sizeof(o));
        const float *m = s.to_world;
        for (int a = 0; a < 3; ++a) o.center[a] = m[4 * a + 3];
        o.radius = sqrtf(fmaf(m[8], m[8], fmaf(m[4], m[4], m[0] * m[0])));
        for (int a = 0; a < 3; ++a) for (int b = 0; b < 3; ++b) o.to_world[3 * a + b] = m[4 * a + b];
        double md[16]; for (int k = 0; k < 16; ++k) md[k] = m[k];
        const double c00 = md[5] * md[10] - md[6] * md[9], c01 = md[6] * md[8] - md[4] * md[10], c02 = md[4] * md[9] - md[5] * md[8];
        const double id = 1.0 / (md[0] * c00 + md[1] * c01 + md[2] * c02);
        double inv[12] = { c00 * id, (md[2] * md[9] - md[1] * md[10]) * id, (md[1] * md[6] - md[2] * md[5]) * id, 0,
                           c01 * id, (md[0] * md[10] - md[2] * md[8]) * id, (md[2] * md[4] - md[0] * md[6]) * id, 0,
                           c02 * id, (md[1] * md[8] - md[0] * md[9]) * id, (md[0] * md[5] - md[1] * md[4]) * id, 0 };
        for (int a = 0; a < 3; ++a) inv[4 * a + 3] = -(inv[4 * a] * md[3] + inv[4 * a + 1] * md[7] + inv[4 * a + 2] * md[11]);
        for (int k = 0; k < 12; ++k) o.to_object[k] = (float) inv[k];
        o.shape = i; o.flip_normals = s.flip_normals;
        if (!(o.radius > 0.f) || !std::isfinite(o.radius)) throw std::runtime_error("sphere with a zero or invalid radius");
        spheres.push_back(o);
    }
    sc.n_spheres = (uint32_t) spheres.size();
    for (uint32_t i = 0; i < d.n_emitters; ++i) {
        const lrt_emitter_desc &e = d.emitters[i];
        if (e.type == LRT_EMITTER_POINT || (e.type == LRT_EMITTER_AREA && e.shape >= 0 && (uint32_t) e.shape < d.n_shapes && d.shapes[e.shape].kind == LRT_SHAPE_MESH)) P.ext = true;
    }
    if (!spheres.empty()) P.ext = true;
    HostBVH &bvh = P.bvh;
    {
        const int forced = opt.bvh_leaf;
        int chosen = forced ? forced : 4;
        bool done = false;
        if (!forced && lds_possible(d, opt)) {
            for (int leaf : { 2, 3, 4, 6, 8, 12, 16 }) {
                HostBVH b2; build_bvh(d.positions, d.faces, d.n_faces, b2, leaf);
                if (lds_image_fits(d, b2, opt)) { bvh = std::move(b2); chosen = leaf; done = true; break; }
            }
        }
        if (!done) build_bvh(d.positions, d.faces, d.n_faces, bvh, chosen);
        P.bvh_leaf = chosen;
    }
    sc.root_is_leaf = bvh.root_is_leaf; sc.root_leaf_first = bvh.root_first; sc.root_leaf_count = bvh.root_count;
    sc.n_faces = d.n_faces; sc.n_emitters = d.n_emitters; sc.one_shape = d.n_shapes == 1;
    if (lds_image_fits(d, bvh, opt)) { build_lds_image(d, bvh, P); P.use_lds = true; }
    sc.grid = DDistGrid{};
    if (d.n_media > 0 && (d.n_faces > 0 || !spheres.empty()) && d.n_faces <= (1u << 17) && !opt.no_dist_grid) {
        float lo[3], hi[3]; referenced_bounds(d, spheres, lo, hi);
        const float ext = std::max(hi[0] - lo[0], std::max(hi[1] - lo[1], hi[2] - lo[2]));
        const int res = opt.dist_grid_res ? opt.dist_grid_res : (d.n_faces <= (1u << 14) ? 192 : 64);
        if (ext > 0.f && std::isfinite(ext)) {
            DDistGrid g{};
            g.cell = ext / (float) res; g.inv_cell = 1.f / g.cell;
            for (int a = 0; a < 3; ++a) { g.lo[a] = lo[a]; g.n[a] = std::max(1, std::min(res, (int) std::ceil((hi[a] - lo[a]) / g.cell))); }
            float diag = std::sqrt((hi[0] - lo[0]) * (hi[0] - lo[0]) + (hi[1] - lo[1]) * (hi[1] - lo[1]) + (hi[2] - lo[2]) * (hi[2] - lo[2]));
            float amax = 0.f; for (int a = 0; a < 3; ++a) amax = std::max(amax, std::max(std::fabs(lo[a]), std::fabs(hi[a])));
            P.grid_abs_margin = 1e-4f * diag + 1e-5f * amax;
            g.enabled = 1; sc.grid = g;
        }
    }
}

void prepare_shading(const lrt_scene_desc &d, const PrepOptions &opt, PreparedScene &P) {
    DScene &sc = P.sc; const std::vector<DSphere> &spheres = P.spheres;
    {
        P.vattr.assign(8 * (size_t) d.n_vertices, 0.f); std::vector<float> &va = P.vattr;
        for (size_t v = 0; v < d.n_vertices; ++v) {
            if (d.normals) for (int a = 0; a < 3; ++a) va[8 * v + a] = d.normals[3 * v + a];
            if (d.texcoords) for (int a = 0; a < 2; ++a) va[8 * v + 4 + a] = d.texcoords[2 * v + a];
        }
    }
    std::vector<DShape> &shapes = P.shapes; shapes.resize(d.n_shapes);
    for (uint32_t i = 0; i < d.n_shapes; ++i) { const lrt_shape_desc &s = d.shapes[i]; shapes[i] = { s.bsdf, s.emitter, s.interior_medium, s.exterior_medium, s.has_normals, s.has_texcoords, s.flip_normals, s.kind }; }
    std::vector<DTexture> &tex = P.textures; tex.resize(d.n_textures); std::vector<float> &tex_data = P.tex_data;
    for (uint32_t i = 0; i < d.n_textures; ++i) {
        const lrt_texture_desc &T = d.textures[i]; DTexture &o = tex[i]; memset(&o, 0, sizeof(o));
        o.type = T.type; o.width = T.width; o.height = T.height; o.channels = T.channels;
        for (int k = 0; k < 3; ++k) { o.color0[k] = T.color0[k]; o.color1[k] = T.color1[k]; }
        for (int k = 0; k < 6; ++k) o.to_uv[k] = T.to_uv[k];
        if (T.type == LRT_TEX_BITMAP) {
            o.data_offset = (uint32_t) tex_data.size();
            size_t np = (size_t) T.width * T.height;
            for (size_t p = 0; p < np; ++p) {
                const float *px = T.data + p * T.channels;
                tex_data.push_back(T.channels == 1 ? px[0] : px[0] * 0.212671f + px[1] * 0.715160f + px[2] * 0.072169f);
            }
        }
    }
    std::vector<DBsdf> &bsdfs = P.bsdfs; bsdfs.resize(d.n_bsdfs); sc.has_null_bsdf = 0;
    auto leaf_flags = [](int type) { return type == LRT_BSDF_DIFFUSE ? PREP_F_SMOOTH : type == LRT_BSDF_DIELECTRIC ? PREP_F_DELTA : PREP_F_NULL; };
    for (uint32_t i = 0; i < d.n_bsdfs; ++i) {
        const lrt_bsdf_desc &B = d.bsdfs[i];
        bsdfs[i] = { B.type, B.reflectance, B.nested, B.texture, B.eta, B.scale, 0, 0 };
        if (B.type == LRT_BSDF_BUMPMAP) {
            if (B.nested < 0 || (uint32_t) B.nested >= d.n_bsdfs || d.bsdfs[B.nested].type == LRT_BSDF_BUMPMAP) throw std::runtime_error("bumpmap: invalid nested BSDF");
            bsdfs[i].flags = leaf_flags(d.bsdfs[B.nested].type);
        } else bsdfs[i].flags = leaf_flags(B.type);
        if (B.type == LRT_BSDF_DIFFUSE && (B.reflectance < 0 || (uint32_t) B.reflectance >= d.n_textures || d.textures[B.reflectance].type == LRT_TEX_BITMAP))
            throw std::runtime_error("unsupported: a bitmap texture as diffuse reflectance (bitmaps are supported as bump-map heights only)");
        if (B.type == LRT_BSDF_NULL) sc.has_null_bsdf = 1;
    }
    DEnv &E = sc.env; memset(&E, 0, sizeof(E)); E.type = -1; E.emitter = -1;
    {
        float lo[3], hi[3]; vertex_bounds(d, spheres, lo, hi);
        const float ray_eps = 5.9604644775390625e-8f * 1500.f;
        if (d.n_vertices || !spheres.empty()) {
            float c[3], dd[3]; for (int a = 0; a < 3; ++a) { c[a] = (hi[a] + lo[a]) * 0.5f; dd[a] = c[a] - hi[a]; E.bsphere_c[a] = c[a]; }
            float r = sqrtf(fmaf(dd[2], dd[2], fmaf(dd[1], dd[1], dd[0] * dd[0])));
            E.bsphere_r = fmaxf(ray_eps, r * (1.f + ray_eps));
        } else { E.bsphere_c[0] = E.bsphere_c[1] = E.bsphere_c[2] = 0.f; E.bsphere_r = ray_eps; }
    }
    if (d.n_media > 64) throw std::runtime_error("at most 64 media are supported");
    for (uint32_t i = 0; i < d.n_media; ++i) {
        const lrt_medium_desc &M = d.media[i];
        if (M.type == LRT_MEDIUM_HOMOGENEOUS || M.type == LRT_MEDIUM_HETEROGENEOUS) P.has_non_bio = true;
        if (M.type != LRT_MEDIUM_HETEROGENEOUS) continue;
        if (!M.grid_data || M.grid_res[0] < 1 || M.grid_res[1] < 1 || M.grid_res[2] < 1 || !(M.grid_max > 0.f)) throw std::runtime_error("heterogeneous medium without a valid grid");
        P.has_het = true;
    }
    for (uint32_t i = 0; i < d.n_shapes; ++i) for (int m : { d.shapes[i].interior_medium, d.shapes[i].exterior_medium })
        if (m >= 0 && d.media[m].type == LRT_MEDIUM_HETEROGENEOUS) P.prb_null = true;
    std::vector<DEmitter> &em = P.emitters; em.resize(d.n_emitters); std::vector<float> &env_rgbx = P.env_data, &hier = P.env_hier; bool &env_interior_positive = P.env_interior_positive;
    std::vector<DMeshEmitter> &mesh_em = P.mesh_emitters; mesh_em.resize(d.n_emitters); std::vector<float> &mesh_tab = P.mesh_emitter_tab;
    for (uint32_t i = 0; i < d.n_emitters; ++i) {
        const lrt_emitter_desc &S = d.emitters[i]; DEmitter &o = em[i]; memset(&o, 0, sizeof(o));
        o.type = S.type; o.shape = S.shape; o.scale = S.scale; for (int k = 0; k < 3; ++k) o.radiance[k] = S.radiance[k];
        if (S.type == LRT_EMITTER_AREA) {
            P.has_area_emitter = true;
            const lrt_shape_desc &sd = d.shapes[S.shape];
            if (sd.kind == LRT_SHAPE_SPHERE) throw std::runtime_error("unsupported: an area emitter on a sphere (area emitters are supported on rectangles and triangle meshes)");
            if (sd.kind == LRT_SHAPE_MESH) {
                MeshEmitterTable T; mesh_emitter_table(d.positions, d.faces, sd.first_face, sd.n_faces, "shapes[" + std::to_string(S.shape) + "]", T);
                DMeshEmitter &M = mesh_em[i];
                M.first_face = sd.first_face; M.n_faces = sd.n_faces; M.sum = T.sum; M.normalization = T.normalization;
                M.has_normals = sd.has_normals; M.flip_normals = sd.flip_normals; M.mesh = 1;
                M.pmf_offset = (uint32_t) mesh_tab.size(); mesh_tab.insert(mesh_tab.end(), T.pmf.begin(), T.pmf.end());
                M.cdf_offset = (uint32_t) mesh_tab.size(); mesh_tab.insert(mesh_tab.end(), T.cdf.begin(), T.cdf.end());
                continue;
            }
            memcpy(o.to_world, sd.to_world, sizeof(float) * 12);
            auto xv = [&](float x, float y, float z, float *r) { const float *m = sd.to_world; for (int a = 0; a < 3; ++a) r[a] = fmaf(m[4 * a + 2], z, fmaf(m[4 * a + 1], y, m[4 * a] * x)); };
            float du[3], dv[3]; xv(2.f, 0.f, 0.f, du); xv(0.f, 2.f, 0.f, dv);
            float cx = fmaf(du[1], dv[2], -(du[2] * dv[1])), cy = fmaf(du[2], dv[0], -(du[0] * dv[2])), cz = fmaf(du[0], dv[1], -(du[1] * dv[0]));
            o.inv_area = 1.f / sqrtf(fmaf(cz, cz, fmaf(cy, cy, cx * cx)));
            uint32_t v0 = d.faces[3 * sd.first_face];
            for (int a = 0; a < 3; ++a) o.n[a] = sd.flip_normals ? -d.normals[3 * v0 + a] : d.normals[3 * v0 + a];
        } else if (S.type == LRT_EMITTER_POINT) {
            memcpy(o.to_world, S.to_world, sizeof(float) * 12);
        } else {
            E.type = S.type; E.emitter = (int) i; E.scale = S.scale; for (int k = 0; k < 3; ++k) E.radiance[k] = S.radiance[k];
            if (S.type == LRT_EMITTER_ENVMAP) {
                uint32_t w = (uint32_t) S.width, h = (uint32_t) S.height; E.w = w + 1; E.h = h;
                env_rgbx.assign((size_t) E.w * h * 4, 0.f); std::vector<float> lum((size_t) E.w * h);
                float theta_scale = 1.f / (float) (h - 1) * 3.14159265358979323846f;
                const float *in = S.data;
                for (uint32_t y = 0; y < h; ++y) {
                    float sin_theta = (float) sin((double) ((float) y * theta_scale));
                    for (uint32_t x = 0; x < w; ++x) {
                        float l = fmaxf((in[0] * 0.212671f + in[1] * 0.715160f + in[2] * 0.072169f) - 0.f, 0.f);
                        lum[(size_t) y * E.w + x] = l * sin_theta;
                        float *o4 = &env_rgbx[((size_t) y * E.w + x) * 4]; o4[0] = in[0]; o4[1] = in[1]; o4[2] = in[2];
                        in += 3;
                    }
                    lum[(size_t) y * E.w + w] = lum[(size_t) y * E.w];
                    for (int k = 0; k < 3; ++k) env_rgbx[((size_t) y * E.w + w) * 4 + k] = env_rgbx[((size_t) y * E.w) * 4 + k];
                }
                build_hierarchy(lum, E.w, h, E, hier);
                env_interior_positive = true;
                for (uint32_t y = 1; y + 1 < h && env_interior_positive; ++y)
                    for (uint32_t x = 0; x < E.w; ++x) if (!(lum[(size_t) y * E.w + x] > 0.f)) { env_interior_positive = false; break; }
                for (int a = 0; a < 3; ++a) for (int b = 0; b < 3; ++b) E.to_world[3 * a + b] = S.to_world[4 * a + b];
                inverse3(S.to_world, E.to_local);
            }
        }
    }
    sc.nee_fast_reject = (d.n_emitters == 1 && !sc.has_null_bsdf && !P.has_het && !opt.no_nee_reject &&
                          (E.type == LRT_EMITTER_CONSTANT || (E.type == LRT_EMITTER_ENVMAP && env_interior_positive))) ? 1 : 0;
    build_camera(d, sc.cam, sc.film);
}

PreparedScene prepare_scene(const lrt_scene_desc &d, const PrepOptions &opt) {
    PreparedScene P; prepare_geometry(d, opt, P); prepare_shading(d, opt, P);
    return P;
}

void prepare_media(const lrt_scene_desc &d, float bsphere_r, std::vector<DMedium> &media, std::vector<DBioMedium> &bio, std::vector<DHetMedium> &het) {
    bio.assign(std::max<uint32_t>(d.n_media, 1), DBioMedium{});
    for (uint32_t i = 0; i < d.n_media; ++i) {
        const lrt_medium_desc &M = d.media[i]; DBioMedium &o = bio[i];
        o.type = M.type; o.has_spectral_extinction = M.has_spectral_extinction;
        for (int l = 0; l < 4; ++l) { o.layer_limit[l] = M.layer_limit[l]; for (int k = 0; k < 3; ++k) { o.collagen[l][k] = M.sigma_collagen[l][k]; o.elastin[l][k] = M.sigma_elastin[l][k]; } }
        for (int k = 0; k < 3; ++k) { o.blood[k] = M.sigma_blood[k]; o.bile[k] = M.sigma_bile[k]; o.lipid_water[k] = M.sigma_lipid_water[k]; }
        o.hepatocity = M.sigma_hepatocity; o.log10_hep = 0.f;
        if (M.type == LRT_MEDIUM_PARENCHYMA) { o.sigmat[0] = 77.2f / 255; o.sigmat[1] = 105.0f / 255; o.sigmat[2] = 149.0f / 255; }
        else for (int k = 0; k < 3; ++k) o.sigmat[k] = medium_sigma_t(M, k);
    }
    media.resize(std::max<uint32_t>(d.n_media, 1));
    for (uint32_t i = 0; i < d.n_media; ++i) {
        const lrt_medium_desc &M = d.media[i]; DMedium &o = media[i];
        for (int k = 0; k < 3; ++k) { o.sigma_t[k] = medium_sigma_t(M, k); o.albedo[k] = M.albedo[k]; }
        o.has_spectral_extinction = M.has_spectral_extinction; o.sample_emitters = M.sample_emitters; o.phase = M.phase; o.g = M.g;
        o.scale = M.scale; o.het = M.type == LRT_MEDIUM_HETEROGENEOUS ? 1 : 0;
        const float bound = (2.f * bsphere_r) * 0.998f - 1e-3f;
        for (int k = 0; k < 3; ++k) {
            const double x = (double) o.sigma_t[k] * (double) bound;
            double v = (x > 0.05 && std::isfinite(x)) ? std::exp(-x * (1.0 - 1e-4)) * (1.0 + 1e-4) : 2.0;
            float vf = (float) v; if ((double) vf < v) vf = std::nextafter(vf, 3.f);
            o.nee_vmin[k] = vf;
        }
    }
    het.assign(std::max<uint32_t>(d.n_media, 1), DHetMedium{});
    for (uint32_t i = 0; i < d.n_media; ++i) {
        const lrt_medium_desc &M = d.media[i]; DHetMedium &o = het[i];
        if (M.type != LRT_MEDIUM_HETEROGENEOUS) continue;
        for (int k = 0; k < 3; ++k) { o.res[k] = M.grid_res[k]; o.bbox_min[k] = M.grid_bbox_min[k]; o.bbox_max[k] = M.grid_bbox_max[k]; }
        for (int k = 0; k < 12; ++k) o.to_local[k] = M.grid_to_local[k];
        o.scale = M.scale; o.max_density = M.scale * M.grid_max;
    }
}

ResolvedOpts resolve(const lrt_scene_desc &d, const lrt_render_opts *o) {
    ResolvedOpts r;
    if (o && o->integrator > LRT_INTEGRATOR_VOLPATHMIS) throw std::invalid_argument("lrt_render_opts.integrator " + std::to_string(o->integrator) + " is not an integrator (LRT_INTEGRATOR_PATH .. LRT_INTEGRATOR_VOLPATHMIS, or -1 for the scene's own)");
// ... 74 lines not shown
```

liverrenderer_amd/csrc/scene_prep.h:

```cpp
#pragma once
#include "device_types.h"
#include "bvh.h"
#include "host_scene.h"
#include <utility>

namespace lrt {

struct PrepOptions {
    int bvh_leaf = 0;
    bool no_lds_bvh = false;
    bool no_dist_grid = false;
    int dist_grid_res = 0;
    bool no_nee_reject = false;
    size_t lds_limit = 0;
    int n_cus = 256;
    static PrepOptions from_env();
};

enum { PREP_F_DELTA = 1, PREP_F_SMOOTH = 2, PREP_F_NULL = 4 };

struct PreparedScene {
    std::vector<DSphere> spheres;
    HostBVH bvh;
    std::vector<unsigned char> lds_blob; DLdsInfo lds{};
    std::vector<float> vattr;
    std::vector<DShape> shapes;
    std::vector<DTexture> textures; std::vector<float> tex_data;
    std::vector<DBsdf> bsdfs;
    std::vector<DEmitter> emitters;
    std::vector<DMeshEmitter> mesh_emitters; std::vector<float> mesh_emitter_tab;
    std::vector<float> env_data, env_hier;
    DScene sc{};
    float grid_abs_margin = 0.f;
    bool env_interior_positive = false;
    bool ext = false, has_area_emitter = false, has_het = false, has_non_bio = false, prb_null = false, use_lds = false;
    int bvh_leaf = 4;
};
void prepare_geometry(const lrt_scene_desc &d, const PrepOptions &opt, PreparedScene &P);
void prepare_shading(const lrt_scene_desc &d, const PrepOptions &opt, PreparedScene &P);
PreparedScene prepare_scene(const lrt_scene_desc &d, const PrepOptions &opt);

size_t lds_image_bytes(const HostBVH &b, uint32_t n_vertices);
bool lds_image_fits(const lrt_scene_desc &d, const HostBVH &b, const PrepOptions &opt);

inline float medium_sigma_t(const lrt_medium_desc &M, int k) { return M.sigma_t[k] * M.scale; }
void prepare_media(const lrt_scene_desc &d, float bsphere_r, std::vector<DMedium> &media, std::vector<DBioMedium> &bio, std::vector<DHetMedium> &het);

struct ResolvedOpts { int integrator, max_depth, rr_depth, hide_emitters; uint32_t spp, seed, tile_rank, tile_count; uint32_t spp_total = 0, n_passes = 1, pass = 0; };
ResolvedOpts resolve(const lrt_scene_desc &d, const lrt_render_opts *o);

struct TilePixels { std::vector<uint32_t> list, slot; };
TilePixels tile_pixel_list(const DFilm &film, uint32_t rank, uint32_t count);
std::vector<uint32_t> halo_pixel_list(const DFilm &film, uint32_t rank, uint32_t count, uint32_t halo);

bool closed_records(const lrt_scene_desc &d, int sensor_medium);

}
```

Measured before the change: 6107 Msamples/s.

## Precompute per-face shading frames, skip zero-radiance film adds, cheaper texture wrap

Adds a host-built per-face table holding the geometric normal and dp_du/dp_dv, which the default compute_si reads in place of recomputing cross products, normalization and the UV Jacobian per hit. The PRB paths opt out and keep the on-the-fly computation. The film accumulation gains a wave-level skip of RGB atomics when no lane carries radiance. Texture wrapping uses one modulo plus a compare instead of two modulos, and the free-flight grid emptiness check is skipped for rays leaving a surface. These trade ALU work for extra memory traffic from 48-byte face table reads, and the ideas are bundled together.

Measured after the change: 6436 Msamples/s (median of 6 runs). 5.4% higher.

```diff
diff --git a/liverrenderer_amd/csrc/device.hip b/liverrenderer_amd/csrc/device.hip
--- a/liverrenderer_amd/csrc/device.hip
+++ b/liverrenderer_amd/csrc/device.hip
@@ -261,6 +261,7 @@
     D->has_area_emitter = P.has_area_emitter; D->has_het = P.has_het; D->has_non_bio = P.has_non_bio; D->prb_null = P.prb_null;
     sc.positions = D->track(dev_upload(d.positions, 3 * (size_t) d.n_vertices, st));
     sc.vattr = (const float4 *) up(P.vattr);
+    sc.face_consts = (const float4 *) up(P.face_consts);
     sc.faces = D->track(dev_upload(d.faces, 3 * (size_t) d.n_faces, st));
     sc.face_shape = D->track(dev_upload(d.face_shape, d.n_faces, st));
     sc.shapes = up(P.shapes);
@@ -356,6 +357,7 @@
     rp.integrator = O.integrator; rp.max_depth = O.max_depth; rp.rr_depth = O.rr_depth; rp.hide_emitters = O.hide_emitters;
     rp.spp = O.spp; rp.log2_spp = ((O.spp & (O.spp - 1)) == 0) ? (uint32_t) __builtin_ctz(O.spp) : 0xffffffffu;
     rp.profile = getenv("LRT_DEBUG_LAUNCH") ? 1u : 0u;
+    if (getenv("LRT_FILM_NO_ZERO_SKIP")) rp.profile |= 0x80000000u;
 #ifdef LRT_EXPERIMENT
     if (getenv("LRT_EXP")) rp.profile |= (uint32_t) atoi(getenv("LRT_EXP"));
     if (getenv("LRT_PRB_DEBUG_LANE")) rp.pad1 = (uint32_t) atoi(getenv("LRT_PRB_DEBUG_LANE")) + 1u;
diff --git a/liverrenderer_amd/csrc/device_types.h b/liverrenderer_amd/csrc/device_types.h
--- a/liverrenderer_amd/csrc/device_types.h
+++ b/liverrenderer_amd/csrc/device_types.h
@@ -133,6 +133,7 @@
     uint32_t n_spheres, pad_sph;
     const DMeshEmitter *mesh_emitters;
     const float *mesh_emitter_tab;
+    const float4 *face_consts;
 };
 
 #define LRT_CONST __attribute__((address_space(4)))
diff --git a/liverrenderer_amd/csrc/dshade.h b/liverrenderer_amd/csrc/dshade.h
--- a/liverrenderer_amd/csrc/dshade.h
+++ b/liverrenderer_amd/csrc/dshade.h
@@ -1,6 +1,7 @@
 #pragma once
 #include "device_types.h"
 #include "dmath.h"
+#include "tex_wrap.h"
 #include "../../include/liverrt.h"
 
 namespace lrt {
@@ -247,6 +248,7 @@
 #endif
 }
 
+template <bool TABLE = true>
 DEV SI compute_si(SceneRef sc, const Ray &r, const Hit &h, const LdsScene *L = nullptr) {
     const bool valid = h.prim != 0xffffffffu;
     float t = kInf; V3 p(0.f), n(0.f), shn(0.f), shs(0.f), sht(0.f), dp_du(0.f), dp_dv(0.f), wi = -r.d;
@@ -269,21 +271,29 @@
         float b1 = h.u, b2 = h.v, b0 = 1.f - b1 - b2;
         t = h.t;
         p = V3(fma_(p0.x, b0, fma_(p1.x, b1, p2.x * b2)), fma_(p0.y, b0, fma_(p1.y, b1, p2.y * b2)), fma_(p0.z, b0, fma_(p1.z, b1, p2.z * b2)));
-        V3 dp0 = p1 - p0, dp1 = p2 - p0;
-        n = normalize(cross(dp0, dp1));
+        if constexpr (TABLE) {
+            const float4 fc0 = sc.face_consts[3 * (size_t) f], fc1 = sc.face_consts[3 * (size_t) f + 1], fc2 = sc.face_consts[3 * (size_t) f + 2];
+            n = V3(fc0.x, fc0.y, fc0.z); dp_du = V3(fc1.x, fc1.y, fc1.z); dp_dv = V3(fc2.x, fc2.y, fc2.z);
+        } else {
+            const V3 dp0 = p1 - p0, dp1 = p2 - p0;
+            n = normalize(cross(dp0, dp1));
+            const Basis bs = coordinate_system(n);
+            dp_du = bs.s; dp_dv = bs.t;
+        }
         uv = { b1, b2 };
-        Basis bs = coordinate_system(n);
-        dp_du = bs.s; dp_dv = bs.t;
         if (sd.has_texcoords) {
             const float2 t0 = *reinterpret_cast<const float2 *>(sc.vattr + 2 * (size_t) i0 + 1), t1 = *reinterpret_cast<const float2 *>(sc.vattr + 2 * (size_t) i1 + 1),
                          t2 = *reinterpret_cast<const float2 *>(sc.vattr + 2 * (size_t) i2 + 1);
             V2 uv0 = { t0.x, t0.y }, uv1 = { t1.x, t1.y }, uv2 = { t2.x, t2.y };
             uv = { fma_(uv2.x, b2, fma_(uv1.x, b1, uv0.x * b0)), fma_(uv2.y, b2, fma_(uv1.y, b1, uv0.y * b0)) };
-            V2 duv0 = { uv1.x - uv0.x, uv1.y - uv0.y }, duv1 = { uv2.x - uv0.x, uv2.y - uv0.y };
-            float det = fma_(duv0.x, duv1.y, -(duv0.y * duv1.x)), inv_det = rcp(det);
-            if (det != 0.f) {
-                dp_du = V3(fma_(duv1.y, dp0.x, -(duv0.y * dp1.x)), fma_(duv1.y, dp0.y, -(duv0.y * dp1.y)), fma_(duv1.y, dp0.z, -(duv0.y * dp1.z))) * inv_det;
-                dp_dv = V3(fma_(-duv1.x, dp0.x, duv0.x * dp1.x), fma_(-duv1.x, dp0.y, duv0.x * dp1.y), fma_(-duv1.x, dp0.z, duv0.x * dp1.z)) * inv_det;
+            if constexpr (!TABLE) {
+                const V3 dp0 = p1 - p0, dp1 = p2 - p0;
+                V2 duv0 = { uv1.x - uv0.x, uv1.y - uv0.y }, duv1 = { uv2.x - uv0.x, uv2.y - uv0.y };
+                float det = fma_(duv0.x, duv1.y, -(duv0.y * duv1.x)), inv_det = rcp(det);
+                if (det != 0.f) {
+                    dp_du = V3(fma_(duv1.y, dp0.x, -(duv0.y * dp1.x)), fma_(duv1.y, dp0.y, -(duv0.y * dp1.y)), fma_(duv1.y, dp0.z, -(duv0.y * dp1.z))) * inv_det;
+                    dp_dv = V3(fma_(-duv1.x, dp0.x, duv0.x * dp1.x), fma_(-duv1.x, dp0.y, duv0.x * dp1.y), fma_(-duv1.x, dp0.z, duv0.x * dp1.z)) * inv_det;
+                }
             }
         }
         if (sd.has_normals) {
@@ -476,6 +486,7 @@
     return V3(0.f);
 }
 
+template <bool WRAP4 = false>
 DEV V2 tex_eval_1_grad(SceneRef sc, int tex, const SI &si) {
     const DTexture &T = sc.textures[tex];
     if (T.type != LRT_TEX_BITMAP) return { 0.f, 0.f };
@@ -485,8 +496,11 @@
     float fx = fma_(u, (float) w, -0.5f), fy = fma_(v, (float) h, -0.5f);
     int ix = (int) __builtin_floorf(fx), iy = (int) __builtin_floorf(fy);
     float w1x = fx - (float) ix, w1y = fy - (float) iy, w0x = 1.f - w1x, w0y = 1.f - w1y;
-    int x0 = ix % w; if (x0 < 0) x0 += w; int x1 = (ix + 1) % w; if (x1 < 0) x1 += w;
-    int y0 = iy % h; if (y0 < 0) y0 += h; int y1 = (iy + 1) % h; if (y1 < 0) y1 += h;
+    int x0, x1, y0, y1;
+    if constexpr (WRAP4) {
+        x0 = ix % w; if (x0 < 0) x0 += w; x1 = (ix + 1) % w; if (x1 < 0) x1 += w;
+        y0 = iy % h; if (y0 < 0) y0 += h; y1 = (iy + 1) % h; if (y1 < 0) y1 += h;
+    } else { x0 = tex_wrap(ix, w); x1 = tex_wrap_next(x0, w); y0 = tex_wrap(iy, h); y1 = tex_wrap_next(y0, h); }
     const float *d = sc.tex_data + T.data_offset;
     float f00 = d[y0 * w + x0], f10 = d[y0 * w + x1], f01 = d[y1 * w + x0], f11 = d[y1 * w + x1];
     float dx = fma_(w0y, f10 - f00, w1y * (f11 - f01)), dy = fma_(w0x, f01 - f00, w1x * (f11 - f10));
@@ -512,8 +526,9 @@
     *r = rr; *cos_theta_t = mulsign_neg(ctt, cos_theta_i);
 }
 
+template <bool WRAP4 = false>
 DEV Frame bump_frame(SceneRef sc, const DBsdf &B, const SI &si) {
-    V2 g = tex_eval_1_grad(sc, B.texture, si);
+    V2 g = tex_eval_1_grad<WRAP4>(sc, B.texture, si);
     float gx = B.scale * g.x, gy = B.scale * g.y;
     V3 dp_du = fma3(si.sh.n, gx - dot(si.sh.n, si.dp_du), si.dp_du);
     V3 dp_dv = fma3(si.sh.n, gy - dot(si.sh.n, si.dp_dv), si.dp_dv);
@@ -572,11 +587,11 @@
     return 0.f;
 }
 
-template <bool DIELECTRIC = false>
+template <bool DIELECTRIC = false, bool WRAP4 = false>
 DEV BSDFSample bsdf_sample(SceneRef sc, int b, const SI &si, float s1, float s2x, float s2y) {
     const DBsdf B = tab(sc.bsdfs, b, sc.one_shape);
     if (B.type == LRT_BSDF_BUMPMAP) {
-        Frame pf = bump_frame(sc, B, si);
+        Frame pf = bump_frame<WRAP4>(sc, B, si);
         V3 pwi = pf.to_local(si.wi);
         BSDFSample bs = leaf_sample<DIELECTRIC>(sc, tab(sc.bsdfs, B.nested, sc.one_shape), si, pwi, s1, s2x, s2y);
         bool active = any_nonzero(bs.weight);
@@ -589,20 +604,22 @@
     }
     return leaf_sample<DIELECTRIC>(sc, B, si, si.wi, s1, s2x, s2y);
 }
+template <bool WRAP4 = false>
 DEV V3 bsdf_eval(SceneRef sc, int b, const SI &si, V3 wo) {
     const DBsdf B = tab(sc.bsdfs, b, sc.one_shape);
     if (B.type == LRT_BSDF_BUMPMAP) {
-        Frame pf = bump_frame(sc, B, si);
+        Frame pf = bump_frame<WRAP4>(sc, B, si);
         V3 pwi = pf.to_local(si.wi), pwo = pf.to_local(wo);
         if (!(wo.z * pwo.z > 0.f)) return V3(0.f);
         return leaf_eval(sc, tab(sc.bsdfs, B.nested, sc.one_shape), si, pwi, pwo) * shadow_terminator(pf.n, wo);
     }
     return leaf_eval(sc, B, si, si.wi, wo);
 }
+template <bool WRAP4 = false>
 DEV float bsdf_pdf(SceneRef sc, int b, const SI &si, V3 wo) {
     const DBsdf B = tab(sc.bsdfs, b, sc.one_shape);
     if (B.type == LRT_BSDF_BUMPMAP) {
-        Frame pf = bump_frame(sc, B, si);
+        Frame pf = bump_frame<WRAP4>(sc, B, si);
         V3 pwi = pf.to_local(si.wi), pwo = pf.to_local(wo);
         if (!(wo.z * pwo.z > 0.f)) return 0.f;
         return leaf_pdf(tab(sc.bsdfs, B.nested, sc.one_shape), pwi, pwo);
diff --git a/liverrenderer_amd/csrc/film.h b/liverrenderer_amd/csrc/film.h
--- a/liverrenderer_amd/csrc/film.h
+++ b/liverrenderer_amd/csrc/film.h
@@ -78,6 +78,7 @@
     return r;
 }
 
+template <bool ZERO_SKIP = true>
 DEV void finish_paths_wave(SceneRef sc, RpRef rp, float *__restrict__ film, float *__restrict__ sample_out,
                            uint64_t sample_base, bool finishing, uint32_t lane, V3 L, bool valid) {
     FilmRef F = sc.film;
@@ -90,6 +91,17 @@
     if (finishing) { int px, py; lane_to_pixel(sc, rp, lane, &px, &py); pixel = (uint32_t) (py - F.crop_offset_y) * (uint32_t) F.width + (uint32_t) (px - F.crop_offset_x); }
     if (__ballot(finishing) == 0ull) return;
     const uint32_t prev = wave_prev(pixel, 0xfffffffeu), next = wave_next(pixel, 0xfffffffeu);
+    bool rgb = true;
+    if constexpr (ZERO_SKIP) rgb = __ballot(finishing && (L.x != 0.f || L.y != 0.f || L.z != 0.f)) != 0ull || (rp.profile & 0x80000000u);
+    if (ZERO_SKIP && !rgb) {
+        float v[2] = { finishing ? 1.f : 0.f, (finishing && valid) ? 1.f : 0.f };
+        wave_segmented_sums(v, pixel != prev || !finishing);
+        if (finishing && pixel != next) {
+            float *p = film + (size_t) pixel * F.channels;
+            if (F.has_alpha) { atomicAdd(p + 3, v[1]); atomicAdd(p + 4, v[0]); } else atomicAdd(p + 3, v[0]);
+        }
+        return;
+    }
     float v[5] = { finishing ? L.x : 0.f, finishing ? L.y : 0.f, finishing ? L.z : 0.f, finishing ? 1.f : 0.f, (finishing && valid) ? 1.f : 0.f };
     wave_segmented_sums(v, pixel != prev || !finishing);
     if (finishing && pixel != next) {
diff --git a/liverrenderer_amd/csrc/kernels.h b/liverrenderer_amd/csrc/kernels.h
--- a/liverrenderer_amd/csrc/kernels.h
+++ b/liverrenderer_amd/csrc/kernels.h
@@ -230,15 +230,15 @@
     };
     uint32_t nohit = 0;
     float cache_t = u2f(0x7fc00000u);
-    auto free_flight_stage = [&]() {
+    auto free_flight_stage = [&](bool on_surface) {
         if (medium < 0) return;
         const DMedium M = tab(sc.media, medium);
         cache_t = medium_sampled_t(M, rng.next(), channel);
-        if (sc.grid.enabled) { const MI m2 = medium_interaction_at(M, ray, cache_t); if (m2.valid() && segment_free_of_surfaces(sc.grid, ray.o, ray.d, m2.t)) nohit = PF_NOHIT; }
+        if (sc.grid.enabled && !on_surface) { const MI m2 = medium_interaction_at(M, ray, cache_t); if (m2.valid() && segment_free_of_surfaces(sc.grid, ray.o, ray.d, m2.t)) nohit = PF_NOHIT; }
     };
     bool active = true;
     if (!PRE) active = termination_stage();
-    else if (fresh) { active = termination_stage(); if (active) { free_flight_stage(); ff_t = cache_t; proven_empty = nohit != 0; nohit = 0; cache_t = u2f(0x7fc00000u); } }
+    else if (fresh) { active = termination_stage(); if (active) { free_flight_stage(false); ff_t = cache_t; proven_empty = nohit != 0; nohit = 0; cache_t = u2f(0x7fc00000u); } }
     if (!active) { commit(); return false; }
 
     bool active_medium = medium >= 0, active_surface = !active_medium;
@@ -403,7 +403,7 @@
     active = active && (active_surface || active_medium);
     if (clk) clk->at(3);
     if (PRE) {
-        if (active) { if (!termination_stage()) { active = false; n_extra++; } else free_flight_stage(); }
+        if (active) { if (!termination_stage()) { active = false; n_extra++; } else free_flight_stage(active_surface); }
         if (clk) clk->at(4);
     } else if (active) {
         SMP pk = rng;
diff --git a/liverrenderer_amd/csrc/kernels_prb.h b/liverrenderer_amd/csrc/kernels_prb.h
--- a/liverrenderer_amd/csrc/kernels_prb.h
+++ b/liverrenderer_amd/csrc/kernels_prb.h
@@ -4,6 +4,9 @@
 namespace lrt {
 
 struct PrbGrads { float sigma_t[3], albedo[3], g; };
+
+DEV SI prb_surface(const GlobalTracer &, SceneRef sc, const Ray &r, const Hit &h) { return compute_si<false>(sc, r, h); }
+template <int STRIDE> DEV SI prb_surface(const LdsTracer<STRIDE> &tr, SceneRef sc, const Ray &r, const Hit &h) { return compute_si<false>(sc, r, h, &tr.L); }
 
 DEV float hg_dlog_dg(float g, float c) {
     float temp = 1.f + sqr(g) + 2.f * g * c;
@@ -32,7 +35,7 @@
         ray.maxt = remaining_dist;
         active = active && remaining_dist > 0.f;
         needs_intersection = needs_intersection && active;
-        if (needs_intersection) { n_shadow++; Hit h = tr.closest(ray); si = tr.surface(sc, ray, h); }
+        if (needs_intersection) { n_shadow++; Hit h = tr.closest(ray); si = prb_surface(tr, sc, ray, h); }
         needs_intersection = false;
         bool active_medium = active && medium >= 0, active_surface = active && !active_medium;
         V3 tr_multiplier(1.f);
@@ -126,8 +129,8 @@
         het = HET && M.het;
         mei = het ? het_sample_interaction(M, tab(sc.het, medium), ray, rng.next()) : medium_sample_interaction(M, ray, rng.next(), channel);
         if (mei.valid() && !het) ray.maxt = mei.t;
-        if (!needs_intersection) si = compute_si(sc, ray, hkeep);
-        else if (!proven_empty) { hkeep = tr.closest(ray); si = tr.surface(sc, ray, hkeep); }
+        if (!needs_intersection) si = compute_si<false>(sc, ray, hkeep);
+        else if (!proven_empty) { hkeep = tr.closest(ray); si = prb_surface(tr, sc, ray, hkeep); }
         if (si.t < mei.t) mei.t = kInf;
         seg_t = fmin_(mei.t, si.t) - mei.mint;
         V3 tr(m_exp(-seg_t * mei.combined.x), m_exp(-seg_t * mei.combined.y), m_exp(-seg_t * mei.combined.z));
@@ -187,16 +190,16 @@
     }
     active_surface = active_surface || escaped_medium;
     bool intersect = active_surface && !escaped_medium;
-    if (intersect) { Hit h = tr.closest(ray); si = tr.surface(sc, ray, h); }
+    if (intersect) { Hit h = tr.closest(ray); si = prb_surface(tr, sc, ray, h); }
     if (rp.hide_emitters && intersect && depth == 0 && si.valid && tab(sc.shapes, si.shape, sc.one_shape).emitter >= 0) {
         Ray r2 = spawn_ray(si.p, si.n, ray.d);
         bool a = true; Hit h; h.prim = 0xffffffffu; h.t = kInf; h.u = h.v = 0.f;
         while (a) {
             h = tr.closest(r2);
             a = h.prim != 0xffffffffu && tab(sc.shapes, sc.face_shape[h.prim], sc.one_shape).emitter >= 0;
-            if (a) { SI s2 = compute_si(sc, r2, h); r2 = spawn_ray(s2.p, s2.n, r2.d); }
-        }
-        si = compute_si(sc, r2, h);
+            if (a) { SI s2 = compute_si<false>(sc, r2, h); r2 = spawn_ray(s2.p, s2.n, r2.d); }
+        }
+        si = compute_si<false>(sc, r2, h);
     }
     if (active_surface) {
         bool count_direct = (depth == 0) || specular_chain;
@@ -225,7 +228,7 @@
         SMP rng_march = rng;
         V3 emitted = prb_sample_emitter<HET>(sc, rng, rp_, rn, active_e_surface, active_e_surface ? si.shape : 0u, si.n, medium, channel, &ds, tr, n_shadow, &seg_sum, gm);
         V3 nee_weight; float nee_pdf;
-        if (active_e_surface) { V3 wo = si.sh.to_local(ds.d); nee_weight = bsdf_eval(sc, b, si, wo); nee_pdf = bsdf_pdf(sc, b, si, wo); }
+        if (active_e_surface) { V3 wo = si.sh.to_local(ds.d); nee_weight = bsdf_eval<true>(sc, b, si, wo); nee_pdf = bsdf_pdf<true>(sc, b, si, wo); }
         else { float pv = phase_eval(tab(sc.media, medium), mei.wi, ds.d); nee_weight = V3(pv); nee_pdf = pv; }
         V3 contrib = throughput * nee_weight * mis_weight(ds.pdf, ds.delta ? 0.f : nee_pdf) * emitted;
         L = ADJOINT ? L - contrib : L + contrib;
@@ -268,7 +271,7 @@
     if (active_surface) {
         const DShape sd = tab(sc.shapes, si.shape, sc.one_shape);
         float s1 = rng.next(), s2x, s2y; rng.next2(s2x, s2y);
-        const BSDFSample bs = bsdf_sample(sc, b, si, s1, s2x, s2y);
+        const BSDFSample bs = bsdf_sample<false, true>(sc, b, si, s1, s2x, s2y);
         active_surface = bs.pdf > 0.f;
         if (active_surface) {
             throughput = throughput * bs.weight;
diff --git a/liverrenderer_amd/csrc/kernels_prb_body.h b/liverrenderer_amd/csrc/kernels_prb_body.h
--- a/liverrenderer_amd/csrc/kernels_prb_body.h
+++ b/liverrenderer_amd/csrc/kernels_prb_body.h
@@ -78,7 +78,7 @@
             }
             if (!ADJOINT) {
                 if (L_buf) { if (had_path && !alive) L_buf[f2u(dl.w)] = make_float4(s.res.x, s.res.y, s.res.z, (s.flags & PF_VALID) ? 1.f : 0.f); }
-                else finish_paths_wave(sc, rp, A.film, A.sample_out, A.sample_base, had_path && !alive, s.lane, s.res, (s.flags & PF_VALID) != 0);
+                else finish_paths_wave<false>(sc, rp, A.film, A.sample_out, A.sample_base, had_path && !alive, s.lane, s.res, (s.flags & PF_VALID) != 0);
             } else {
                 float g[7] = { G.sigma_t[0], G.sigma_t[1], G.sigma_t[2], G.albedo[0], G.albedo[1], G.albedo[2], G.g };
 #pragma unroll
diff --git a/liverrenderer_amd/csrc/scene_prep.cpp b/liverrenderer_amd/csrc/scene_prep.cpp
--- a/liverrenderer_amd/csrc/scene_prep.cpp
+++ b/liverrenderer_amd/csrc/scene_prep.cpp
@@ -155,6 +155,46 @@
     for (const DSphere &o : spheres) for (int a = 0; a < 3; ++a) { lo[a] = fminf(lo[a], o.center[a] - o.radius); hi[a] = fmaxf(hi[a], o.center[a] + o.radius); }
 }
 
+namespace {
+struct H3 { float x, y, z; };
+inline uint32_t h_bits(float f) { uint32_t u; memcpy(&u, &f, 4); return u; }
+inline float h_float(uint32_t u) { float f; memcpy(&f, &u, 4); return f; }
+inline H3 h_sub(H3 a, H3 b) { return { a.x - b.x, a.y - b.y, a.z - b.z }; }
+inline H3 h_scale(H3 a, float s) { return { a.x * s, a.y * s, a.z * s }; }
+inline float h_dot(H3 a, H3 b) { return fmaf(a.z, b.z, fmaf(a.y, b.y, a.x * b.x)); }
+inline H3 h_cross(H3 a, H3 b) { return { fmaf(a.y, b.z, -(a.z * b.y)), fmaf(a.z, b.x, -(a.x * b.z)), fmaf(a.x, b.y, -(a.y * b.x)) }; }
+inline H3 h_normalize(H3 a) { return h_scale(a, 1.f / sqrtf(h_dot(a, a))); }
+inline float h_mulsign(float a, float s) { return h_float(h_bits(a) ^ (h_bits(s) & 0x80000000u)); }
+inline float h_mulsign_neg(float a, float s) { return h_float(h_bits(a) ^ (~h_bits(s) & 0x80000000u)); }
+inline void h_coordinate_system(H3 n, H3 &s, H3 &t) {
+    const float sign = h_float(0x3f800000u | (h_bits(n.z) & 0x80000000u)), a = -(1.f / (sign + n.z)), b = n.x * n.y * a;
+    s = { h_mulsign((n.x * n.x) * a, n.z) + 1.f, h_mulsign(b, n.z), h_mulsign_neg(n.x, n.z) };
+    t = { b, fmaf(n.y, n.y * a, sign), -n.y };
+}
+}
+void build_face_table(const lrt_scene_desc &d, const std::vector<float> &vattr, std::vector<float> &out) {
+    out.assign(12 * (size_t) d.n_faces, 0.f);
+    for (uint32_t f = 0; f < d.n_faces; ++f) {
+        const uint32_t shp = d.n_shapes == 1 ? 0u : d.face_shape[f];
+        const uint32_t i0 = d.faces[3 * (size_t) f], i1 = d.faces[3 * (size_t) f + 1], i2 = d.faces[3 * (size_t) f + 2];
+        auto pos = [&](uint32_t i) { return H3{ d.positions[3 * (size_t) i], d.positions[3 * (size_t) i + 1], d.positions[3 * (size_t) i + 2] }; };
+        const H3 p0 = pos(i0), dp0 = h_sub(pos(i1), p0), dp1 = h_sub(pos(i2), p0);
+        const H3 n = h_normalize(h_cross(dp0, dp1));
+        H3 dp_du, dp_dv; h_coordinate_system(n, dp_du, dp_dv);
+        if (shp < d.n_shapes && d.shapes[shp].has_texcoords) {
+            const float *t0 = &vattr[8 * (size_t) i0 + 4], *t1 = &vattr[8 * (size_t) i1 + 4], *t2 = &vattr[8 * (size_t) i2 + 4];
+            const float d0x = t1[0] - t0[0], d0y = t1[1] - t0[1], d1x = t2[0] - t0[0], d1y = t2[1] - t0[1];
+            const float det = fmaf(d0x, d1y, -(d0y * d1x)), inv_det = 1.f / det;
+            if (det != 0.f) {
+                dp_du = h_scale(H3{ fmaf(d1y, dp0.x, -(d0y * dp1.x)), fmaf(d1y, dp0.y, -(d0y * dp1.y)), fmaf(d1y, dp0.z, -(d0y * dp1.z)) }, inv_det);
+                dp_dv = h_scale(H3{ fmaf(-d1x, dp0.x, d0x * dp1.x), fmaf(-d1x, dp0.y, d0x * dp1.y), fmaf(-d1x, dp0.z, d0x * dp1.z) }, inv_det);
+            }
+        }
+        float *o = &out[12 * (size_t) f];
+        o[0] = n.x; o[1] = n.y; o[2] = n.z; o[4] = dp_du.x; o[5] = dp_du.y; o[6] = dp_du.z; o[8] = dp_dv.x; o[9] = dp_dv.y; o[10] = dp_dv.z;
+    }
+}
+
 void prepare_geometry(const lrt_scene_desc &d, const PrepOptions &opt, PreparedScene &P) {
     DScene &sc = P.sc;
     memset(&sc, 0, sizeof(sc));
@@ -227,6 +267,7 @@
             if (d.normals) for (int a = 0; a < 3; ++a) va[8 * v + a] = d.normals[3 * v + a];
             if (d.texcoords) for (int a = 0; a < 2; ++a) va[8 * v + 4 + a] = d.texcoords[2 * v + a];
         }
+        build_face_table(d, va, P.face_consts);
     }
     std::vector<DShape> &shapes = P.shapes; shapes.resize(d.n_shapes);
     for (uint32_t i = 0; i < d.n_shapes; ++i) { const lrt_shape_desc &s = d.shapes[i]; shapes[i] = { s.bsdf, s.emitter, s.interior_medium, s.exterior_medium, s.has_normals, s.has_texcoords, s.flip_normals, s.kind }; }
diff --git a/liverrenderer_amd/csrc/scene_prep.h b/liverrenderer_amd/csrc/scene_prep.h
--- a/liverrenderer_amd/csrc/scene_prep.h
+++ b/liverrenderer_amd/csrc/scene_prep.h
@@ -24,6 +24,7 @@
     HostBVH bvh;
     std::vector<unsigned char> lds_blob; DLdsInfo lds{};
     std::vector<float> vattr;
+    std::vector<float> face_consts;
     std::vector<DShape> shapes;
     std::vector<DTexture> textures; std::vector<float> tex_data;
     std::vector<DBsdf> bsdfs;
@@ -39,6 +40,8 @@
 void prepare_geometry(const lrt_scene_desc &d, const PrepOptions &opt, PreparedScene &P);
 void prepare_shading(const lrt_scene_desc &d, const PrepOptions &opt, PreparedScene &P);
 PreparedScene prepare_scene(const lrt_scene_desc &d, const PrepOptions &opt);
+
+void build_face_table(const lrt_scene_desc &d, const std::vector<float> &vattr, std::vector<float> &out);
 
 size_t lds_image_bytes(const HostBVH &b, uint32_t n_vertices);
 bool lds_image_fits(const lrt_scene_desc &d, const HostBVH &b, const PrepOptions &opt);
diff --git a/liverrenderer_amd/csrc/tex_wrap.h b/liverrenderer_amd/csrc/tex_wrap.h
--- /dev/null
+++ b/liverrenderer_amd/csrc/tex_wrap.h
@@ -0,0 +1,14 @@
+#pragma once
+
+namespace lrt {
+
+#if defined(__HIPCC__)
+#define LRT_HD __host__ __device__ __forceinline__
+#else
+#define LRT_HD inline
+#endif
+
+LRT_HD int tex_wrap(int i, int n) { int r = i % n; if (r < 0) r += n; return r; }
+LRT_HD int tex_wrap_next(int x0, int n) { return x0 + 1 == n ? 0 : x0 + 1; }
+
+}
```
